# jjalcaraz-upct/network-slicing

Hardware: AMD Instinct MI355X
Metric: env-steps/sec (batched RanSlice.step, scenario_0) (higher is better)
Workload: dtype f64

## Files before the change

include/ranslice.h:

```cpp
#ifndef RANSLICE_H
#define RANSLICE_H

#include <stdint.h>

#ifdef __cplusplus
extern "C" {
#endif

#define RS_OK 0
#define RS_EINVAL (-1)
#define RS_EOVERFLOW (-2)
#define RS_EHIP (-3)
#define RS_ESTATE (-4)

#define RS_N_EMBB_VARS 10
#define RS_N_MMTC_VARS 3
#define RS_MAX_MCS 32
#define RS_MAX_SET 8
#define RS_N_TRACES 3

typedef struct rs_config {
    int32_t n_envs;
    int32_t n_prbs;
    int32_t n_embb;
    int32_t n_mmtc;
    int32_t slots_per_step;
    int32_t max_ue;
    int32_t max_bursts;
    int32_t max_mtc_queue;
    double slot_length;
    double penalty;
    double cbr_lambda, cbr_t_mean, cbr_bit_rate;
    double vbr_lambda, vbr_t_mean, vbr_p_size, vbr_b_size, vbr_b_rate;
    double sla_embb[6];
    double norm_embb[RS_N_EMBB_VARS];
    int32_t mtc_n_devices;
    int32_t mtc_n_rep, mtc_n_period;
    int32_t mtc_rep_set[RS_MAX_SET];
    int32_t mtc_period_set[RS_MAX_SET];
    double sla_mtc_delay;
    double norm_mmtc[RS_N_MMTC_VARS];
    double prop_A, prop_B;
    int32_t pf_granularity, pf_window, sym_per_prb;
    int32_t n_mcs;
    double mcs_rate[RS_MAX_MCS];
    double mcs_snr[RS_MAX_MCS];
    int32_t mcs_order[RS_MAX_MCS];
    int32_t mcs_mod[RS_MAX_MCS];
    double mi_x0[3], mi_k[3];
    int32_t l1_multiplex;
    int32_t reserved_;
} rs_config;

typedef struct rs_handle rs_handle;

typedef struct rs_alloc_rec {
    int32_t serial;
    int32_t type;
    int32_t e_snr;
    int32_t prbs;
    int64_t bits;
    double queue;
    double th;
    double p;
} rs_alloc_rec;

int rs_create(const rs_config* cfg, int device, rs_handle** out);

int rs_load_fading(rs_handle* h, int trace_id, const double* data, int rows, int cols);

int rs_reset(rs_handle* h, const uint64_t* seeds, float* obs);

int rs_step(rs_handle* h, const int32_t* actions, float* obs, double* reward, int32_t* labels,
            int32_t* violations);

int rs_step_resident(rs_handle* h);

int rs_random_actions(rs_handle* h, uint64_t seed, uint64_t step_index);

int rs_fetch(rs_handle* h, int32_t* actions, float* obs, double* reward, int32_t* labels,
             int32_t* violations);

int rs_get_info(rs_handle* h, double* info);

int rs_run_random(rs_handle* h, uint64_t seed, uint64_t step_index0, int n_steps, int use_graph);

int rs_set_alloc_trace(rs_handle* h, int enable);
int rs_get_alloc_trace(rs_handle* h, rs_alloc_rec* out);

int rs_get_counters(rs_handle* h, uint64_t counters[4]);

int rs_get_rx_stats(rs_handle* h, uint64_t out[3]);

int rs_kernel_time_ms(rs_handle* h, double* avg_ms, int64_t* launches);
int rs_kernel_time_stats_ms(rs_handle* h, double out[3], int64_t* launches);
int rs_set_kernel_timing(rs_handle* h, int enable);

int rs_set_group_size(rs_handle* h, int lanes);

int rs_set_schedule_hint(rs_handle* h, int mode);

int rs_get_section_profile(rs_handle* h, uint64_t out[16]);
int rs_get_task_profile(rs_handle* h, uint64_t* out);

int rs_synchronize(rs_handle* h);
int rs_device_count(void);
int rs_device_mem_info(int device, uint64_t* free_bytes, uint64_t* total_bytes);
int rs_n_vars(const rs_handle* h);
int rs_state_bytes(rs_handle* h, uint64_t* bytes);
int rs_save_state(rs_handle* h, void* blob, uint64_t bytes);
int rs_load_state(rs_handle* h, const void* blob, uint64_t bytes);
int rs_fork(rs_handle* dst, rs_handle* src, const int32_t* src_index);
int rs_set_lookahead(rs_handle* h, int max_branches);
int rs_step_clairvoyant(rs_handle* h, int32_t* actions_out, float* obs, double* reward, int32_t* labels,
                        int32_t* violations);
int rs_set_clairvoyant_fallback(rs_handle* h, int mode);
int rs_n_slices(const rs_handle* h);
#define RS_ACT_PRBS   0
#define RS_ACT_SHARES 1
#define RS_ACT_INDEX  2

typedef struct rs_device_view {
    int32_t device, n_envs, n_slices, n_vars;
    void*    stream;
    int32_t* in_prbs;  float* in_shares;  int64_t* in_index;
    int32_t* actions;  int32_t* resources;
    float*   obs;       float* obs_norm;
    double*  reward;    int32_t* labels;  int32_t* violations;  int32_t* total_violations;
    int64_t* rejected;
} rs_device_view;

int rs_get_device_view(rs_handle* h, rs_device_view* out);
int rs_step_device(rs_handle* h, int kind, const void* actions_device, void* caller_stream);
int rs_stream_join(rs_handle* h, void* caller_stream);
int rs_set_action_table(rs_handle* h, const int32_t* table , int32_t n_actions);
int rs_report_begin(rs_handle* h, int32_t steps);
int rs_report_extend(rs_handle* h, int32_t eval_steps);
int rs_report_fetch(rs_handle* h, int16_t* violation, double* reward, int16_t* resources, int32_t* n_recorded);
int rs_device_copy(rs_handle* h, void* dst, const void* src, uint64_t bytes, int to_device);
const char* rs_last_error(const rs_handle* h);
void rs_destroy(rs_handle* h);


#define KB_MAX_SLICES 8
#define KB_CAPACITY_MAX 65536

typedef struct kb_config {
    int32_t n_envs;
    int32_t n_slices;
    int32_t n_prbs;
    int32_t capacity;
    int32_t dims[KB_MAX_SLICES];
    double alfa;
    double acc_lo, acc_hi;
    double gamma, eta;
    int32_t shared_dictionary;
    int32_t first_env;
    int64_t pool_bytes;
} kb_config;

typedef struct kb_handle kb_handle;

int kb_create(const kb_config* cfg, int device, kb_handle** out);
void kb_destroy(kb_handle* k);
const char* kb_last_error(const kb_handle* k);
int kb_reset(kb_handle* k, const int32_t* initial_action, const int32_t* security_factor, const uint64_t* seeds);
int kb_update_control(kb_handle* k, const float* state, const int32_t* action, const int32_t* labels, int32_t* hits);
int kb_select_action(kb_handle* k, const float* state, int32_t* action, int32_t* adjusted);
int kb_step_resident(kb_handle* k, rs_handle* env);
int kb_run_resident(kb_handle* k, rs_handle* env, int n_steps, int use_graph);
int kb_predict(kb_handle* k, int e, int s, const double* x, int32_t* y_pred, double* f);
int kb_update(kb_handle* k, int e, int s, const double* x, int32_t y, int32_t* branch, double* delta);
int kb_get_kernel_row(kb_handle* k, int e, int s, int32_t* m, double* row);
int kb_get_learner(kb_handle* k, int e, int s, int32_t* m, double* landmarks, double* coeff, double* kinv);
int kb_get_control(kb_handle* k, int32_t* margins, int32_t* security, int32_t* action, int32_t* adjusted,
                   double* accuracies);
int kb_set_adjusted(kb_handle* k, const int32_t* adjusted);
#define KB_PROP_WIDTH 18
int kb_shared_scan(kb_handle* k, const float* state, const int32_t* action, const int32_t* labels, int32_t round,
                   int32_t budget, int32_t* hits, int32_t* counts, double* props);
// ... 100 lines not shown
```

network-slicing_amd/csrc/kb_api.hip:

```cpp
#pragma once
#include "kb_kbrl.hip"

struct kb_prune_state;
struct kb_ref_state;
struct kb_rebuild_state;
struct kb_bridge_state;
struct kb_fit_state;

struct kb_handle {
    kb_config cfg;
    int device = 0;
    hipStream_t stream = nullptr;
    hipEvent_t ev_order = nullptr;
    hipEvent_t ev_join = nullptr;
    hipStream_t side = nullptr;
    hipEvent_t ev_sfork = nullptr, ev_sjoin = nullptr;
    kb::KbDev D;
    kb::KbState K;
    std::vector<void*> allocs;
    std::vector<GuardedAlloc> guarded;
    std::vector<std::pair<void*, size_t>> regions;
    float* d_state = nullptr;
    float* d_prev_state = nullptr;
    int32_t* d_action = nullptr;
// ... 652 lines not shown
                hipLaunchKernelGGL(kb::select_bin_big_kernel, dim3(KB_BINBIG_GRID), dim3(64 * KB_BINBIG_WAVES), 0, k->stream, a);
                hipLaunchKernelGGL(kb::select_bin_kernel, dim3((unsigned)k->T), dim3(64), 0, k->stream, a, (int)KB_BIG_MAX);
            } else {
                hipLaunchKernelGGL(kb::select_bin_all_kernel, dim3(KB_BINBIG_GRID + (unsigned)((k->T + KB_BINBIG_WAVES - 1) / KB_BINBIG_WAVES)),
                                   dim3(64 * KB_BINBIG_WAVES), 0, k->stream, a);
            }
            hipLaunchKernelGGL(kb::big_list_kernel, dim3((unsigned)((k->T + 255) / 256)), dim3(256), 0, k->stream, k->D, k->K, a.big_par);
        } else {
            hipLaunchKernelGGL(kb::select_bin_kernel, dim3(slots), dim3(64), 0, k->stream, a, 0);
        }
        if (eb) HIPCHK(k, hipEventRecord(eb, k->stream));
        HIPCHK(k, k->spans.begin(k->stream, 6, &eg));
        hipLaunchKernelGGL(kb::select_gemm_kernel, dim3((slots + KB_SEL_WAVES - 1) / KB_SEL_WAVES), dim3(256), 0, k->stream, a);
        if (eg) HIPCHK(k, hipEventRecord(eg, k->stream));
    }
    if (e1) HIPCHK(k, hipEventRecord(e1, k->stream));
    hipLaunchKernelGGL(kb::adjust_kernel, dim3((unsigned)((k->cfg.n_envs + 255) / 256)), dim3(256), 0, k->stream, k->D,
                       k->K, d_action_out, a.big_par);
    if (a.big_par >= 0) k->big_par = 1 - k->big_par;
    return RS_OK;
}

static int kb_refuse_plus(kb_handle* k, const char* who) {
    if (k->alg != KB_ALG_PROJECTRON_PLUS || k->control_plus) return RS_OK;
    k->err = std::string(who) +
             ": the handle is in Projectron++ mode (kb_set_algorithm), which learns through kb_update / kb_fit only -- the control "
             "loop's update phase implements Projectron's rule (kb_set_algorithm(k, KB_ALG_PROJECTRON) switches back; "
             "kb_set_learning(k, 0) lets the resident loop select without learning)";
    return RS_ESTATE;
}

extern "C" int kb_update_control(kb_handle* k, const float* state, const int32_t* action, const int32_t* labels,
                                 int32_t* hits) {
    if (!k || !state || !action || !labels) return RS_EINVAL;
    if (!k->is_reset) {
        k->err = "kb_update_control: call kb_reset first";
        return RS_ESTATE;
    }
    if (int rc = kb_refuse_plus(k, "kb_update_control")) return rc;
    if (k->D.shared) {
        k->err = "kb_update_control: shared-dictionary handles learn through kb_shared_scan/apply/commit";
        return RS_ESTATE;
    }
    if (k->frozen) {
        k->err = "kb_update_control: an inference-only handle (kb_deploy) cannot learn: it holds no Kinv";
        return RS_ESTATE;
    }
    HIPCHK(k, hipSetDevice(k->device));
    const size_t T = (size_t)k->T, N = (size_t)k->cfg.n_envs;
    for (size_t i = 0; i < T; ++i)
        if (action[i] < 0 || action[i] > k->cfg.n_prbs || (labels[i] != 1 && labels[i] != -1)) {
            k->err = "kb_update_control: action out of [0, n_prbs] or label not +-1";
            return RS_EINVAL;
        }
    HIPCHK(k, hipMemcpyAsync(k->d_state, state, sizeof(float) * N * k->nv, hipMemcpyHostToDevice, k->stream));
    HIPCHK(k, hipMemcpyAsync(k->d_action, action, sizeof(int32_t) * T, hipMemcpyHostToDevice, k->stream));
    HIPCHK(k, hipMemcpyAsync(k->d_labels, labels, sizeof(int32_t) * T, hipMemcpyHostToDevice, k->stream));
    int rc = launch_update_control(k, k->d_state, k->d_action, k->d_labels);
    if (rc != RS_OK) return rc;
    HIPCHK(k, hipGetLastError());
    if (hits) HIPCHK(k, hipMemcpyAsync(hits, k->d_hits, sizeof(int32_t) * T, hipMemcpyDeviceToHost, k->stream));
    return kb_check(k);
}

extern "C" int kb_select_action(kb_handle* k, const float* state, int32_t* action, int32_t* adjusted) {
    if (!k || !state) return RS_EINVAL;
    if (!k->is_reset) {
        k->err = "kb_select_action: call kb_reset first";
        return RS_ESTATE;
    }
    HIPCHK(k, hipSetDevice(k->device));
    const size_t T = (size_t)k->T, N = (size_t)k->cfg.n_envs;
    HIPCHK(k, hipMemcpyAsync(k->d_state, state, sizeof(float) * N * k->nv, hipMemcpyHostToDevice, k->stream));
    int rc = launch_select(k, k->d_state, nullptr);
    if (rc != RS_OK) return rc;
    HIPCHK(k, hipGetLastError());
    if (action) HIPCHK(k, hipMemcpyAsync(action, k->K.action, sizeof(int32_t) * T, hipMemcpyDeviceToHost, k->stream));
    if (adjusted) HIPCHK(k, hipMemcpyAsync(adjusted, k->K.adjusted, sizeof(int32_t) * N, hipMemcpyDeviceToHost, k->stream));
    return kb_check(k);
}

extern "C" int kb_step_resident(kb_handle* k, rs_handle* env) {
    if (!k || !env) return RS_EINVAL;
    if (!k->is_reset || env->cfg.n_envs != k->cfg.n_envs || env->n_slices != k->cfg.n_slices || env->n_vars != k->nv ||
        env->device != k->device) {
        k->err = "kb_step_resident: agent and environment do not match (or kb_reset missing)";
        return RS_EINVAL;
    }
    if (k->D.shared) {
        k->err = "kb_step_resident: shared-dictionary handles step through kb_shared_step_resident";
        return RS_ESTATE;
    }
    if (k->learning)
        if (int rc = kb_refuse_plus(k, "kb_step_resident")) return rc;
    HIPCHK(k, hipSetDevice(k->device));
    if (env->hint_auto && !env->block_hint) {
        rs_set_schedule_hint(env, 1);
        env->hint_auto = true;
    }
    int rc = stream_after(k, &k->ev_order, env->stream, k->stream);
    if (rc != RS_OK) return rc;
    if (k->learning && (rc = launch_update_control(k, k->d_prev_state, env->d_actions, env->d_labels)) != RS_OK) return rc;
    rc = launch_select(k, env->d_obs, env->d_actions);
    if (rc != RS_OK) return rc;
    if (k->h_steps > 0) {
        kb::HistArgs ha;
        ha.D = k->D;
        ha.K = k->K;
        ha.reward = env->d_reward;
        ha.labels = env->d_labels;
        ha.violations = env->d_viol;
        ha.hits = k->d_hits;
        ha.h_reward = k->h_reward;
        ha.h_resources = k->h_resources;
        ha.h_hits = k->h_hits;
        ha.h_adjusted = k->h_adjusted;
        ha.h_sla = k->h_sla;
        ha.h_violation = k->h_violation;
        ha.cursor = k->h_cursor;
        ha.steps = k->h_steps;
        hipLaunchKernelGGL(kb::history_kernel, dim3((unsigned)((k->cfg.n_envs + 255) / 256)), dim3(256), 0, k->stream, ha);
        hipLaunchKernelGGL(kb::history_advance_kernel, dim3(1), dim3(1), 0, k->stream, k->h_cursor);
    }
    HIPCHK(k, hipMemcpyAsync(k->d_prev_state, env->d_obs, sizeof(float) * (size_t)k->cfg.n_envs * k->nv,
                             hipMemcpyDeviceToDevice, k->stream));
    if ((rc = stream_after(k, &k->ev_order, k->stream, env->stream)) != RS_OK) return rc;
    HIPCHK(k, hipGetLastError());
    return RS_OK;
}

static int enqueue_closed_step(kb_handle* k, rs_handle* env) {
    int rc = kb_step_resident(k, env);
    if (rc != RS_OK) return rc;
    rc = launch_step(env);
    if (rc != RS_OK) k->err = env->err;
    return rc;
}

extern "C" int kb_run_resident(kb_handle* k, rs_handle* env, int n_steps, int use_graph) {
    if (!k || !env || n_steps < 0) return RS_EINVAL;
    int done = 0, rc;
    if (k->learning && (rc = kb_refuse_plus(k, "kb_run_resident")) != RS_OK) return rc;
    static const bool no_graph = getenv("ROCP_TOOL_LIBRARIES") != nullptr &&
                                 !(dev_env("KBRL_GRAPH_UNDER_PROFILER") && atoi(dev_env("KBRL_GRAPH_UNDER_PROFILER")) != 0);
    if (no_graph) use_graph = 0;
    if (use_graph && !k->spans.on && !env->spans.on && !k->D.shared && n_steps >= 3) {
        if (!k->gexec || k->g_env != env || k->g_sig != env->launch_sig) {
            kb_drop_graph(k);
            if ((rc = enqueue_closed_step(k, env)) != RS_OK) return rc;
            done += 1;
        } else if (k->big_par != k->g_big_par || env->order_par != k->g_order_par) {
            if ((rc = enqueue_closed_step(k, env)) != RS_OK) return rc;
            done += 1;
            if (k->big_par != k->g_big_par || env->order_par != k->g_order_par) kb_drop_graph(k);
        }
        if (!k->gexec && n_steps - done >= 2) {
            const int32_t clock0 = env->clock;
            const uint64_t steps0 = env->steps;
            const bool ra = k->rounds_always, gf = k->gemm_fresh;
            k->g_big_par = k->big_par;
            k->g_order_par = env->order_par;
            k->rounds_always = true;
            HIPCHK(k, hipStreamBeginCapture(env->stream, hipStreamCaptureModeThreadLocal));
            const int rc1 = enqueue_closed_step(k, env);
            const int rc2 = rc1 == RS_OK ? enqueue_closed_step(k, env) : rc1;
            const hipError_t ec = hipStreamEndCapture(env->stream, &k->graph);
            env->clock = clock0;
            env->steps = steps0;
            env->order_par = k->g_order_par;
            k->big_par = k->g_big_par;
            k->rounds_always = ra;
            k->gemm_fresh = gf;
            if (rc2 != RS_OK || ec != hipSuccess) {
                kb_drop_graph(k);
                if (rc2 == RS_OK) k->err = std::string("hipStreamEndCapture: ") + hipGetErrorString(ec);
                return rc2 != RS_OK ? rc2 : RS_EHIP;
            }
            HIPCHK(k, hipGraphInstantiate(&k->gexec, k->graph, nullptr, nullptr, 0));
            k->g_env = env;
            k->g_sig = env->launch_sig;
        }
        bool launched = false;
        if (k->gexec && n_steps - done >= 2) {
            if ((rc = stream_after(k, &k->ev_order, k->stream, env->stream)) != RS_OK) return rc;
        }
        while (k->gexec && n_steps - done >= 2) {
            HIPCHK(k, hipGraphLaunch(k->gexec, env->stream));
            env->clock += 2 * env->cfg.slots_per_step;
            env->steps += 2;
            done += 2;
            launched = true;
        }
        if (launched) {
            if ((rc = stream_after(k, &k->ev_join, env->stream, k->stream)) != RS_OK) return rc;
        }
    }
    for (; done < n_steps; ++done)
        if ((rc = enqueue_closed_step(k, env)) != RS_OK) return rc;
    return RS_OK;
}

static int kb_one(kb_handle* k, int e, int s, const double* x, int y, bool update, double out[4]) {
    if (!k || !x || e < 0 || e >= k->cfg.n_envs || s < 0 || s >= k->cfg.n_slices) return RS_EINVAL;
    k->gemm_fresh = false;
    if (!k->is_reset) {
        k->err = "kb_predict/kb_update: call kb_reset first";
        return RS_ESTATE;
    }
    if (update && k->frozen) {
        k->err = "kb_update: an inference-only handle (kb_deploy) cannot learn: it holds no Kinv";
        return RS_ESTATE;
    }
    if (k->ref) {
        k->err = "kb_predict: a by-reference handle (kb_deploy_ref) shares read-only dictionaries: the cached kernel row would be written into a shared page";
        return RS_ESTATE;
    }
    HIPCHK(k, hipSetDevice(k->device));
    kb::OneArgs a;
    a.D = k->D;
    a.K = k->K;
    a.task = e * k->cfg.n_slices + s;
    a.y = y;
    memset(a.x, 0, sizeof a.x);
// ... 411 lines not shown
        k->gemm_fresh = false;
        launch_shared_scan(k, a);
        if (e1) local(hipEventRecord(e1, k->stream), "hipEventRecord");
        hipLaunchKernelGGL(kb::shared_collect_block_kernel, dim3((unsigned)S), dim3(KB_RANK_THREADS), 0, k->stream, k->D, d_state,
                           d_labels, k->d_cstar, (int)budget, k->d_block);
        if (rnd == 0 && hits_host) local(hipMemcpyAsync(hits_host, k->d_hits, sizeof(int32_t) * T, hipMemcpyDeviceToHost, k->stream), "copy of the hits");
        local(hipGetLastError(), "launch of the scan kernels");
        if (rnd == inject) local_err = "failure injected by KBRL_INJECT_FAIL_ROUND";
        if (!local_err.empty() && k->d_gather) {
            static const double mark[KB_MAX_SLICES] = {-1.0, -1.0, -1.0, -1.0, -1.0, -1.0, -1.0, -1.0};
            (void)hipMemcpyAsync(k->d_block, mark, sizeof(double) * S, hipMemcpyHostToDevice, k->stream);
        }
        if (!k->d_gather) {
            k->err = "kb_shared_step: " + local_err;
            if (k->comm) kb_comm_abort(k);
            return RS_EHIP;
        }
        if (k->comm) {
            const int nrc = rccl::AllGather(k->d_block, k->d_gather, blk, rccl::kDouble, k->comm, k->stream);
            if (nrc != 0) {
                k->err = std::string("ncclAllGather: ") + (rccl::GetErrorString ? rccl::GetErrorString(nrc) : "error");
                kb_comm_abort(k);
                return RS_EHIP;
            }
        } else {
            HIPCHK(k, hipMemcpyAsync(k->d_gather, k->d_block, sizeof(double) * blk, hipMemcpyDeviceToDevice, k->stream));
        }
        HIPCHK(k, hipMemsetAsync(k->d_total, 0, 2 * sizeof(int32_t), k->stream));
        hipLaunchKernelGGL(kb::shared_merge_kernel, dim3((unsigned)S), dim3(256), 0, k->stream, k->D, k->d_gather, W, me,
                           (int)budget, blk, k->d_mprops, k->d_mcounts, k->d_taken, k->d_total);
        launch_shared_apply(k, k->d_mprops, k->d_mcounts, (int)budget);
        hipLaunchKernelGGL(kb::shared_commit_kernel, dim3((unsigned)S), dim3(KB_RANK_THREADS), 0, k->stream, k->D, k->d_cstar, k->d_taken,
                           k->d_cursor);
        HIPCHK(k, hipGetLastError());
        if (rnd + 1 == max_rounds && !rounds_out && !k->comm && local_err.empty()) break;
        if (!k->h_total) HIPCHK(k, hipHostMalloc((void**)&k->h_total, 2 * sizeof(int32_t), hipHostMallocDefault));
        volatile int32_t* total = k->h_total;
        total[0] = total[1] = 0;
        HIPCHK(k, hipMemcpyAsync(k->h_total, k->d_total, 2 * sizeof(int32_t), hipMemcpyDeviceToHost, k->stream));
        const int wrc = shared_wait(k);
        if (wrc != RS_OK) return wrc;
        if (total[1] != 0 || !local_err.empty()) {
            k->err = !local_err.empty() ? "kb_shared_step: this rank failed in round " + std::to_string(rnd) + " (" + local_err +
                                              "); the other ranks were told through the exchange and leave the step with it"
                                        : "kb_shared_step: another rank of the shared-dictionary group reported a failure in round " +
                                              std::to_string(rnd) + "; all ranks leave the step together";
            return RS_EHIP;
        }
        if (total[0] == 0) break;
        rounds = rnd + 1;
    }
    if (rounds_out) *rounds_out = rounds;
    return RS_OK;
}

extern "C" int kb_shared_step(kb_handle* k, const float* state, const int32_t* action, const int32_t* labels,
                              int32_t budget, int32_t max_rounds, int32_t* hits, int32_t* rounds_out) {
    if (!k || !state || !action || !labels || budget <= 0 || max_rounds <= 0) return RS_EINVAL;
    if (!k->D.shared || !k->is_reset) {
        k->err = "kb_shared_step: handle is not a reset shared-dictionary agent";
        return RS_ESTATE;
    }
    if (budget > k->budget_cap) {
        k->err = "kb_shared_step: budget too large (<= 256)";
        return RS_EINVAL;
    }
    HIPCHK(k, hipSetDevice(k->device));
    const size_t T = (size_t)k->T, N = (size_t)k->cfg.n_envs;
    for (size_t i = 0; i < T; ++i)
        if (action[i] < 0 || action[i] > k->cfg.n_prbs || (labels[i] != 1 && labels[i] != -1)) {
            k->err = "kb_shared_step: action out of [0, n_prbs] or label not +-1";
            return RS_EINVAL;
        }
    HIPCHK(k, hipMemcpyAsync(k->d_state, state, sizeof(float) * N * k->nv, hipMemcpyHostToDevice, k->stream));
    HIPCHK(k, hipMemcpyAsync(k->d_action, action, sizeof(int32_t) * T, hipMemcpyHostToDevice, k->stream));
    HIPCHK(k, hipMemcpyAsync(k->d_labels, labels, sizeof(int32_t) * T, hipMemcpyHostToDevice, k->stream));
    int rc = shared_step_core(k, k->d_state, k->d_action, k->d_labels, budget, max_rounds, hits, rounds_out);
    if (rc != RS_OK) return rc;
    return kb_check(k);
}

extern "C" int kb_shared_step_resident(kb_handle* k, rs_handle* env, int32_t budget, int32_t max_rounds, int32_t* rounds_out) {
    if (!k || !env || budget <= 0 || max_rounds <= 0) return RS_EINVAL;
    if (!k->D.shared || !k->is_reset || env->cfg.n_envs != k->cfg.n_envs || env->n_slices != k->cfg.n_slices ||
        env->n_vars != k->nv || env->device != k->device || budget > k->budget_cap) {
        k->err = "kb_shared_step_resident: agent and environment do not match (or not a reset shared-dictionary agent, or budget > 256)";
        return RS_EINVAL;
    }
    HIPCHK(k, hipSetDevice(k->device));
    if (env->hint_auto && !env->block_hint) {
        rs_set_schedule_hint(env, 1);
        env->hint_auto = true;
    }
    int rc = stream_after(k, &k->ev_order, env->stream, k->stream);
    if (rc != RS_OK) return rc;
    rc = shared_step_core(k, k->d_prev_state, env->d_actions, env->d_labels, budget, max_rounds, nullptr, rounds_out);
    if (rc != RS_OK) return rc;
    rc = launch_select(k, env->d_obs, env->d_actions);
    if (rc != RS_OK) return rc;
    HIPCHK(k, hipMemcpyAsync(k->d_prev_state, env->d_obs, sizeof(float) * (size_t)k->cfg.n_envs * k->nv,
                             hipMemcpyDeviceToDevice, k->stream));
    if ((rc = stream_after(k, &k->ev_order, k->stream, env->stream)) != RS_OK) return rc;
    HIPCHK(k, hipGetLastError());
    k->gemm_fresh = true;
    return RS_OK;
}

extern "C" int kb_shared_merge(kb_handle* k, const double* gathered, int32_t world, int32_t me, int32_t budget, double* merged,
                               int32_t* counts, int32_t* taken, int32_t* total) {
    if (!k || !gathered || world < 1 || world > 64 || me < 0 || me >= world || budget <= 0 || budget > k->budget_cap)
        return RS_EINVAL;
    if (!k->D.shared) {
        k->err = "kb_shared_merge: handle is not a shared-dictionary agent";
        return RS_ESTATE;
    }
    HIPCHK(k, hipSetDevice(k->device));
    const size_t S = (size_t)k->cfg.n_slices, blk = S * (1 + (size_t)budget * KB_PROP_W);
    double* d_g = nullptr;
    HIPCHK(k, hipMalloc((void**)&d_g, sizeof(double) * blk * (size_t)world));
    int rc = RS_OK;
    hipError_t e = hipMemcpyAsync(d_g, gathered, sizeof(double) * blk * (size_t)world, hipMemcpyHostToDevice, k->stream);
    if (e == hipSuccess) e = hipMemsetAsync(k->d_total, 0, 2 * sizeof(int32_t), k->stream);
    if (e == hipSuccess) {
        hipLaunchKernelGGL(kb::shared_merge_kernel, dim3((unsigned)S), dim3(256), 0, k->stream, k->D, d_g, (int)world, (int)me,
                           (int)budget, blk, k->d_mprops, k->d_mcounts, k->d_taken, k->d_total);
        e = hipGetLastError();
    }
    if (e == hipSuccess && merged)
        e = hipMemcpyAsync(merged, k->d_mprops, sizeof(double) * S * budget * KB_PROP_W, hipMemcpyDeviceToHost, k->stream);
    if (e == hipSuccess && counts) e = hipMemcpyAsync(counts, k->d_mcounts, sizeof(int32_t) * S, hipMemcpyDeviceToHost, k->stream);
    if (e == hipSuccess && taken) e = hipMemcpyAsync(taken, k->d_taken, sizeof(int32_t) * S, hipMemcpyDeviceToHost, k->stream);
    if (e == hipSuccess && total) e = hipMemcpyAsync(total, k->d_total, sizeof(int32_t), hipMemcpyDeviceToHost, k->stream);
    if (e == hipSuccess) e = hipStreamSynchronize(k->stream);
    (void)hipFree(d_g);
    if (e != hipSuccess) {
        k->err = std::string("kb_shared_merge: ") + hipGetErrorString(e);
        rc = RS_EHIP;
    }
    return rc;
}

extern "C" int kb_history_begin(kb_handle* k, int32_t steps) {
    if (!k || steps <= 0) return RS_EINVAL;
    kb_drop_graph(k);
    HIPCHK(k, hipSetDevice(k->device));
    HIPCHK(k, hipStreamSynchronize(k->stream));
    kb_history_release(k);
    const size_t N = (size_t)k->cfg.n_envs, S = (size_t)k->cfg.n_slices, n = N * (size_t)steps;
    HIPCHK(k, hipMalloc((void**)&k->h_reward, sizeof(double) * n));
    HIPCHK(k, hipMalloc((void**)&k->h_resources, sizeof(int16_t) * n));
    HIPCHK(k, hipMalloc((void**)&k->h_hits, sizeof(int16_t) * n * S));
    HIPCHK(k, hipMalloc((void**)&k->h_adjusted, sizeof(int16_t) * n));
    HIPCHK(k, hipMalloc((void**)&k->h_sla, sizeof(int16_t) * n));
    HIPCHK(k, hipMalloc((void**)&k->h_violation, sizeof(int16_t) * n));
    HIPCHK(k, hipMalloc((void**)&k->h_cursor, sizeof(int32_t)));
    HIPCHK(k, hipMemsetAsync(k->h_reward, 0, sizeof(double) * n, k->stream));
    HIPCHK(k, hipMemsetAsync(k->h_resources, 0, sizeof(int16_t) * n, k->stream));
    HIPCHK(k, hipMemsetAsync(k->h_hits, 0, sizeof(int16_t) * n * S, k->stream));
    HIPCHK(k, hipMemsetAsync(k->h_adjusted, 0, sizeof(int16_t) * n, k->stream));
    HIPCHK(k, hipMemsetAsync(k->h_sla, 0, sizeof(int16_t) * n, k->stream));
    HIPCHK(k, hipMemsetAsync(k->h_violation, 0, sizeof(int16_t) * n, k->stream));
    HIPCHK(k, hipMemsetAsync(k->h_cursor, 0, sizeof(int32_t), k->stream));
    k->h_steps = steps;
    return RS_OK;
}

// ... 224 lines not shown
```

network-slicing_amd/csrc/rs_api.hip:

```cpp

#include <hip/hip_runtime.h>

#include <cmath>
#include <cstdio>
#include <cstdlib>
#include <cstring>
#include <string>
#include <vector>

#include "rs_host.h"

#ifdef RS_DEV
static inline const char* dev_env(const char* name) { return getenv(name); }
#else
static inline const char* dev_env(const char*) { return nullptr; }
#endif

#include "rs_embb.hip"
#include "rs_mmtc.hip"
#include "rs_order.hip"
#include "rs_mux.hip"

using namespace rs;

struct GuardedAlloc {
    void* base;
    size_t bytes;
};
static const size_t kGuard = 64 * 1024;
static bool guards_on() {
    static const bool on = dev_env("RANSLICE_GUARD") != nullptr;
    return on;
}
static hipError_t guarded_malloc(void** q, size_t bytes, std::vector<GuardedAlloc>* reg) {
    if (!guards_on()) return hipMalloc(q, bytes);
    void* b = nullptr;
    const size_t padded = (bytes + 255) / 256 * 256;
    hipError_t e = hipMalloc(&b, padded + 2 * kGuard);
    if (e != hipSuccess) return e;
    if (padded <= ((size_t)1 << 30)) {
        e = hipMemset(b, 0xA5, padded + 2 * kGuard);
    } else {
        e = hipMemset(b, 0xA5, kGuard);
        if (e == hipSuccess) e = hipMemset((char*)b + kGuard + padded, 0xA5, kGuard);
    }
    if (e != hipSuccess) return e;
    reg->push_back({b, padded});
    *q = (char*)b + kGuard;
    if (const char* v = dev_env("RANSLICE_GUARD"))
        if (v[0] == '2') fprintf(stderr, "RANSLICE_GUARD: buffer #%zu at %p, %zu bytes\n", reg->size() - 1, *q, bytes);
    return hipSuccess;
}
static void check_guards(const std::vector<GuardedAlloc>& reg, const char* who) {
    std::vector<unsigned char> buf(kGuard);
    for (size_t i = 0; i < reg.size(); ++i)
        for (int side = 0; side < 2; ++side) {
            const char* src = (const char*)reg[i].base + (side ? kGuard + reg[i].bytes : 0);
            if (hipMemcpy(buf.data(), src, kGuard, hipMemcpyDeviceToHost) != hipSuccess) continue;
            for (size_t k = 0; k < kGuard; ++k)
                if (buf[k] != 0xA5) {
                    fprintf(stderr, "RANSLICE_GUARD: %s buffer #%zu (%zu bytes): %s guard overwritten at offset %zu\n", who, i,
                            reg[i].bytes, side ? "upper" : "lower", k);
                    abort();
                }
        }
}

struct rs_handle {
    rs_config cfg;
    int device = 0;
    hipStream_t stream = nullptr;
    hipStream_t side = nullptr;
    hipEvent_t ev_fork = nullptr, ev_join = nullptr;
    int mixed = 0;
    int mixed_light = 256;
    int mixed_ue = 8;
    hipStream_t side2 = nullptr, side3 = nullptr;
    hipEvent_t ev_fork2 = nullptr, ev_join2 = nullptr, ev_join3 = nullptr;
    RsDev hdev;
    RsDev* ddev = nullptr;
    RsState st;
    RsState* d_st = nullptr;
    MtcState mst;
    std::vector<void*> allocs;
    std::vector<GuardedAlloc> guarded;
    std::vector<std::pair<void*, size_t>> regions;
    double* fad = nullptr;
    uint8_t* fad_valid = nullptr;
    double rx_band0 = 0.0;
    float* fad32 = nullptr;
    double* fps = nullptr;
    bool fad_loaded[RS_N_TRACES] = {false, false, false};
    std::vector<double> fad_host[RS_N_TRACES];
    std::vector<uint8_t> valid_host[RS_N_TRACES];
    int32_t* d_actions = nullptr;
    float* d_obs = nullptr;
    double* d_reward = nullptr;
    int32_t* d_labels = nullptr;
    int32_t* d_viol = nullptr;
    double* d_info = nullptr;
    uint64_t* d_counters = nullptr;
    uint64_t* d_counter_sum = nullptr;
    rs_alloc_rec* d_trace = nullptr;
    uint64_t* d_sections = nullptr;
    unsigned long long* d_pace = nullptr;
    int32_t* d_redo = nullptr;
    int32_t* d_order = nullptr;
    uint64_t* d_oslot = nullptr;
    int* d_ohist = nullptr;
    int order_par = 0;
    int order_mode = 6;
    int order_pair = 256;
    int block_hint = 0;
    int spread_mode = -1;
    int spread_max = 1024;
    int key_w[4] = {16, 16, 0, 0};
    int rot_mask = 0;
    int snake_mask = 0x2aaaaaaa;
    int snake = 1;
    bool hint_auto = true;
    int group = 16;
    bool trace_on = false;
    int n_slices = 0, n_vars = 0, n_tasks = 0;
    int n_ran = 0;
    bool mux = false;
    int64_t* d_run = nullptr;
    hipGraph_t graph = nullptr;
    hipGraphExec_t gexec = nullptr;
    int graph_par = 0, graph_sig = -1;
    uint64_t launch_sig = 0;
    int32_t clock = 0;
    uint64_t steps = 0;
    bool is_reset = false;
    uint64_t fad_hash = 0;
    bool tables_borrowed = false;
    int32_t* d_fork_idx = nullptr;
    int32_t* h_fork_idx = nullptr;
    hipEvent_t ev_fork_in = nullptr, ev_fork_out = nullptr;
    rs_handle* la = nullptr;
    int la_max = 0;
    int la_widest = 0;
    int32_t* d_la_err = nullptr;
    struct PolicyIo* pio = nullptr;
    EventSpans spans;
    std::string err;
};

static int auto_hint(const rs_handle* h);

static void drop_graph(rs_handle* h);

template <class T>
static int dalloc(rs_handle* h, T** p, size_t n) {
    void* q = nullptr;
    size_t bytes = sizeof(T) * (n ? n : 1);
    HIPCHK(h, guarded_malloc(&q, bytes, &h->guarded));
    HIPCHK(h, hipMemsetAsync(q, 0, bytes, h->stream));
    if (!guards_on()) h->allocs.push_back(q);
    h->regions.emplace_back(q, bytes);
    *p = (T*)q;
    return RS_OK;
}


static size_t mtc_mux_lds_bytes(int cap, int n_mmtc) {
    return ((size_t)2 * cap * n_mmtc + (size_t)n_mmtc * MTC_DEV_MAX) * sizeof(int32_t);
}

static int mtc_alloc(rs_handle* h, rs::MtcState* m, size_t n_tasks, const RsDev& d) {
    memset(m, 0, sizeof *m);
    m->n_tasks = n_tasks;
    m->cap = d.mtc_cap;
    if (n_tasks == 0) return RS_OK;
    if (d.mtc_n_dev > MTC_DEV_MAX || d.mtc_cap > MTC_CAP_MAX || d.mtc_n_rep <= 0 || d.mtc_n_rep > 8 ||
        d.mtc_n_period <= 0 || d.mtc_n_period > 8) {
        h->err = "rs_create: mMTC configuration out of range (<=1024 devices, queue capacity <=2048)";
        return RS_EINVAL;
    }
    if (d.mux) {
        const size_t lds = mtc_mux_lds_bytes(d.mtc_cap, d.n_mmtc);
        if (lds > 160 * 1024 - 4096) {
            h->err = "rs_create: l1_multiplex with this many mMTC RAN slices and this queue capacity needs more LDS than a CU has";
            return RS_EINVAL;
        }
        if (lds > 48 * 1024)
            HIPCHK(h, hipFuncSetAttribute((const void*)rs::mtc_mux_step_kernel, hipFuncAttributeMaxDynamicSharedMemorySize, (int)lds));
    }
    for (int i = 0; i < d.mtc_n_period; ++i)
        if (d.mtc_period_set[i] < d.slots) {
            h->err = "rs_create: mMTC periods shorter than one observation period are not supported";
            return RS_EINVAL;
        }
    int rc;
    if ((rc = dalloc(h, &m->n_users, n_tasks)) != RS_OK) return rc;
    if ((rc = dalloc(h, &m->s_start, n_tasks)) != RS_OK) return rc;
    if ((rc = dalloc(h, &m->s_rep, n_tasks)) != RS_OK) return rc;
    if ((rc = dalloc(h, &m->dev_next, n_tasks * MTC_DEV_MAX)) != RS_OK) return rc;
    if ((rc = dalloc(h, &m->dev_period, n_tasks * MTC_DEV_MAX)) != RS_OK) return rc;
    if ((rc = dalloc(h, &m->dev_rep, n_tasks * MTC_DEV_MAX)) != RS_OK) return rc;
    if ((rc = dalloc(h, &m->q_rep, n_tasks * (size_t)m->cap)) != RS_OK) return rc;
    if ((rc = dalloc(h, &m->q_start, n_tasks * (size_t)m->cap)) != RS_OK) return rc;
    return RS_OK;
}

static int mtc_reset(rs_handle* h, rs::MtcState* m) {
    if (m->n_tasks == 0) return RS_OK;
    hipLaunchKernelGGL(rs::mtc_reset_kernel, dim3((unsigned)m->n_tasks), dim3(256), 0, h->stream, h->ddev, *m,
                       h->st.seeds);
    return RS_OK;
}

static int mtc_step(rs_handle* h, rs::MtcState* m, hipStream_t stream) {
    if (m->n_tasks == 0) return RS_OK;
    rs::MtcArgs a;
    a.D = h->ddev;
    a.M = *m;
    a.actions = h->d_actions;
    a.run = h->d_run;
    a.obs = h->d_obs;
    a.labels = h->d_labels;
    a.violations = h->d_viol;
    a.info = h->d_info;
    a.err = h->st.err;
    size_t lds = (size_t)4 * 2 * m->cap * sizeof(int32_t);
    hipLaunchKernelGGL(rs::mtc_step_kernel, dim3((unsigned)((m->n_tasks + 3) / 4)), dim3(256), lds, stream, a);
    return RS_OK;
}


namespace rs {

__global__ void reset_kernel(const RsDev* D, RsState S, const uint64_t* seeds_in) {
    int i = blockIdx.x * blockDim.x + threadIdx.x;
    int n_tasks = D->n_envs * D->n_embb;
    if (i < n_tasks) {
        S.t_n_ue[i] = 0;
        S.t_cbr_at[i] = 1;
        S.t_vbr_at[i] = 1;
        S.t_ctr[i] = 0;
        S.t_serial[i] = 1;
        S.t_cost[i] = 0;
    }
    if (i < D->n_envs) {
        S.seeds[i] = seeds_in[i];
        S.err[i] = 0;
    }
}

__global__ void finalize_kernel(const RsDev* D, const int32_t* actions, const int32_t* viol, double* reward,
                                int64_t* run) {
    int r = blockIdx.x * blockDim.x + threadIdx.x;
    if (r >= D->n_envs) return;
    if (r == 0) {
        run[0] += D->slots;
        run[1] += 1;
    }
    int S = D->n_act;
    long tv = 0, ta = 0;
    for (int s = 0; s < S; ++s) {
        tv += viol[r * S + s];
        ta += actions[r * S + s];
    }
    double rew;
    if (tv > 0)
        rew = -1 * D->penalty * (double)tv;
    else
        rew = (double)(D->n_prbs - ta > 0 ? D->n_prbs - ta : 0);
    reward[r] = rew;
}

__global__ __launch_bounds__(256) void random_actions_kernel(const RsDev* D, int32_t* actions, uint64_t seed,
                                                           uint64_t step, const int64_t* run) {
    if (run) {
        step = (uint64_t)run[1];
        seed = (uint64_t)run[2];
    }
    const int lane = threadIdx.x & 63;
    const int r = blockIdx.x * 4 + (threadIdx.x >> 6);
    if (r >= D->n_envs) return;
    const int S = D->n_act;
    int my_bin[8];
    int cnt = 0;
    for (int p = lane; p < D->n_prbs; p += 64) {
        uint32_t a, b;
        rs_philox4x32_10((uint32_t)p, (uint32_t)r, (uint32_t)step,
                         (uint32_t)(step >> 32) ^ (uint32_t)((uint64_t)r >> 32) ^ 0x5bd1e995u, (uint32_t)seed,
                         (uint32_t)(seed >> 32), &a, &b);
        my_bin[cnt++ & 7] = (int)(((uint64_t)a * (uint64_t)(S + 1)) >> 32);
    }
    for (int s = 0; s < S; ++s) {
        int c = 0;
        for (int k = 0; k < cnt; ++k) c += my_bin[k] == s ? 1 : 0;
        for (int d = 32; d >= 1; d >>= 1) c += __shfl_xor(c, d);
        if (lane == 0) actions[r * S + s] = c;
    }
}

__global__ void set_run_kernel(int64_t* run, uint64_t seed, uint64_t step) {
    run[1] = (int64_t)step;
    run[2] = (int64_t)seed;
}

__global__ void counter_sum_kernel(const uint64_t* per_task, int n_tasks, uint64_t* out) {
    __shared__ unsigned long long acc[4];
    if (threadIdx.x < 4) acc[threadIdx.x] = 0ull;
    __syncthreads();
    unsigned long long loc[4] = {0ull, 0ull, 0ull, 0ull};
    for (int i = blockIdx.x * blockDim.x + threadIdx.x; i < n_tasks; i += gridDim.x * blockDim.x)
        for (int k = 0; k < 4; ++k) loc[k] += per_task[(size_t)i * 4 + k];
    for (int k = 0; k < 4; ++k) atomicAdd(&acc[k], loc[k]);
    __syncthreads();
    if (threadIdx.x < 4) atomicAdd((unsigned long long*)&out[threadIdx.x], acc[threadIdx.x]);
}

}


static void mcs_factors(double* A, double* B) {
    double Delta = 0.1;
    double a = 1.0 / Delta;
    double s01 = rs_sigmoid(0.1, 0.0, 1.0), s09 = rs_sigmoid(0.9, 0.0, 1.0);
    a = a * (rs_log(1.0 / s01 - 1.0) - rs_log(1.0 / s09 - 1.0));
    *A = a;
    *B = -rs_log(1.0 / s09 - 1.0);
}

static void mcs_lookup(const rs_config* c, double A, double B, int e_snr, int* mcs_out, int* rate_out) {
    double rx_prob = 1.0 - 0.1;
    int mcs;
    for (mcs = 0; mcs < c->n_mcs; ++mcs) {
        double x = A * ((double)e_snr - c->mcs_snr[mcs]) - B;
        if (rs_sigmoid(x, 0.0, 1.0) < rx_prob) {
            *mcs_out = mcs - 1 > 0 ? mcs - 1 : 0;
            *rate_out = (int)((double)c->sym_per_prb * (c->mcs_rate[mcs] * (double)c->mcs_order[mcs]));
            return;
        }
    }
    mcs = c->n_mcs - 1;
    *mcs_out = mcs;
    *rate_out = (int)((double)c->sym_per_prb * (c->mcs_rate[mcs] * (double)c->mcs_order[mcs]));
}

static void rx_fast_setup(RsDev& d, double* band0) {
    const double A = d.mcsA;
    double kmax = 0.0, kmin = 1e300;
    bool ok = std::isfinite(A) && A > 0.0 && std::isfinite(d.mcsB);
    for (int m = 0; m < 3; ++m) {
        const double k = d.mi_k[m];
        ok = ok && std::isfinite(k) && k > 0.0 && std::isfinite(d.mi_x0[m]);
        kmax = k > kmax ? k : kmax;
        kmin = k < kmin ? k : kmin;
        d.rx_c1[m] = (float)(-k * RS_INV_LN2);
    }
    ok = ok && A / kmax >= 1.0 && A / kmin <= 1.0e4;
    d.rx_invA = ok ? (float)(1.0 / A) : 0.0f;
    d.rx_B = (float)d.mcsB;
    d.rx_band = 0.0;
    *band0 = ok ? 6.0e-6 + 6.0e-6 * (kmax / A) : 0.0;
    d.rx_band1 = ok ? 4.0e-5 / A + 1.0e-6 : 0.0;
    if (dev_env("RANSLICE_RX_EXACT")) *band0 = 0.0;
    if (const char* e = dev_env("RANSLICE_RX_BAND_SCALE")) {
        const double f = atof(e);
// ... 117 lines not shown
        }
        d.slot_rc = rc;
        d.pf_div_fast = (same && !dev_env("RANSLICE_EXACT_DIV")) ? 1 : 0;
    }
    for (int m = 0; m < cfg->n_mcs; ++m) {
        d.mcs_ref[m] = cfg->mcs_snr[m];
        if (cfg->mcs_mod[m] < 0 || cfg->mcs_mod[m] > 2) {
            h->err = "rs_create: modulation index out of range";
            return RS_EINVAL;
        }
        d.mcs_mod[m] = cfg->mcs_mod[m];
    }
    for (int m = 0; m < 3; ++m) {
        d.mi_x0[m] = cfg->mi_x0[m];
        d.mi_k[m] = cfg->mi_k[m];
    }
    rx_fast_setup(d, &h->rx_band0);
    d.mtc_n_dev = cfg->mtc_n_devices;
    d.mtc_cap = cfg->max_mtc_queue > 0 ? cfg->max_mtc_queue : 1024;
    d.mtc_n_rep = cfg->mtc_n_rep;
    d.mtc_n_period = cfg->mtc_n_period;
    for (int i = 0; i < 8; ++i) {
        d.mtc_rep_set[i] = cfg->mtc_rep_set[i];
        d.mtc_period_set[i] = cfg->mtc_period_set[i];
    }
    d.sla_mtc_delay = cfg->sla_mtc_delay;
    for (int i = 0; i < 3; ++i) d.norm_mmtc[i] = cfg->norm_mmtc[i];

    int rc;
    const size_t T = (size_t)h->n_tasks, N = (size_t)cfg->n_envs;
    const size_t U = T * RS_GROUP;
    RsState& s = h->st;
#define DA(p, n)                                   \
    if ((rc = dalloc(h, &(p), (n))) != RS_OK) return rc
    DA(h->ddev, 1);
    DA(s.t_n_ue, T); DA(s.t_cbr_at, T); DA(s.t_vbr_at, T); DA(s.t_ctr, T); DA(s.t_serial, T); DA(s.t_cost, T);
    DA(s.u_queue, U); DA(s.u_th, U); DA(s.u_nominal, U);
    DA(s.u_hold_at, U); DA(s.u_e_snr, U); DA(s.u_findex, U); DA(s.u_bits, U); DA(s.u_prbs, U);
    DA(s.u_vbr_at, U); DA(s.u_ctr, U); DA(s.u_serial, U); DA(s.u_flags, U);
    DA(s.u_burst, U * RS_BURSTS);
    DA(s.seeds, N); DA(s.err, N);
    DA(h->d_actions, N * h->n_slices);
    DA(h->d_obs, N * h->n_vars);
    DA(h->d_reward, N);
    DA(h->d_labels, N * h->n_slices);
    DA(h->d_viol, N * h->n_slices);
    DA(h->d_info, N * h->n_ran * 10);
    DA(h->d_counters, (T ? T : 1) * 4);
    DA(h->d_counter_sum, 4);
    DA(h->d_sections, 16 + 4 * (T ? T : 1) + 16);
    DA(h->d_redo, T ? T : 1);
    DA(h->d_order, T ? T : 1);
    DA(h->d_oslot, T ? T : 1);
    DA(h->d_ohist, 2 * RS_ORDER_BINS);
    HIPCHK(h, hipMemset(h->d_ohist, 0, sizeof(int) * 2 * RS_ORDER_BINS));
    if (const char* e = dev_env("RANSLICE_ORDER")) h->order_mode = atoi(e);
    {
        int cus = 256;
        if (hipDeviceGetAttribute(&cus, hipDeviceAttributeMultiprocessorCount, h->device) != hipSuccess) cus = 256;
        (void)hipGetLastError();
        const long long resident_waves = (long long)cus * 4 * RS_OCC;
        h->order_pair = (long long)h->n_tasks / 4 > resident_waves + resident_waves / 4 ? 0 : 256;
    }
    if (const char* e = dev_env("RANSLICE_PAIR")) h->order_pair = atoi(e);
    h->group = h->n_tasks <= 6144 ? 32 : 16;
    if (const char* e = dev_env("RANSLICE_GROUP")) {
        const int g = atoi(e);
        if (g == 8 || g == 16 || g == 32) h->group = g;
    }
    {
        int cus = 0;
        if (hipDeviceGetAttribute(&cus, hipDeviceAttributeMultiprocessorCount, h->device) == hipSuccess && cus > 0) h->spread_max = cus * 4;
        (void)hipGetLastError();
        if (const char* e = dev_env("RANSLICE_SPREAD")) h->spread_mode = atoi(e);
        if (const char* e = dev_env("RANSLICE_SNAKE")) h->snake = atoi(e);
        if (const char* e = dev_env("RANSLICE_KEY_W")) (void)sscanf(e, "%d,%d,%d,%d", &h->key_w[0], &h->key_w[1], &h->key_w[2], &h->key_w[3]);
        if (const char* e = dev_env("RANSLICE_SNAKE_MASK")) h->snake_mask = (int)strtol(e, nullptr, 0);
        if (const char* e = dev_env("RANSLICE_SNAKE_ROT")) h->rot_mask = (int)strtol(e, nullptr, 0);
    }
    if (h->group == 16 && h->n_tasks >= 49152) h->mixed_light = 224;
    if (const char* e = dev_env("RANSLICE_MIXED")) h->mixed = atoi(e);
    if (const char* e = dev_env("RANSLICE_MIXED_UE")) h->mixed_ue = atoi(e);
    if (const char* e = dev_env("RANSLICE_MIXED_LIGHT")) h->mixed_light = atoi(e);
    if (h->mixed > 0 || h->mixed_light < 256) {
        HIPCHK(h, hipStreamCreateWithFlags(&h->side2, hipStreamNonBlocking));
        HIPCHK(h, hipEventCreateWithFlags(&h->ev_fork2, hipEventDisableTiming));
        HIPCHK(h, hipEventCreateWithFlags(&h->ev_join2, hipEventDisableTiming));
        HIPCHK(h, hipStreamCreateWithFlags(&h->side3, hipStreamNonBlocking));
        HIPCHK(h, hipEventCreateWithFlags(&h->ev_join3, hipEventDisableTiming));
    }
    h->block_hint = auto_hint(h);
    if (const char* e = dev_env("RANSLICE_HINT")) {
        h->hint_auto = atoi(e) < 0;
        if (!h->hint_auto) h->block_hint = atoi(e) ? 1 : 0;
    }
    DA(h->d_st, 1);
    DA(h->d_run, 4);
    DA(h->d_pace, 4);
    if ((rc = mtc_alloc(h, &h->mst, N * (size_t)cfg->n_mmtc, d)) != RS_OK) return rc;
#undef DA
    HIPCHK(h, hipMemcpyAsync(h->d_st, &h->st, sizeof(RsState), hipMemcpyHostToDevice, h->stream));
    HIPCHK(h, hipStreamSynchronize(h->stream));
    return RS_OK;
}

static void fork_release(rs_handle* h);
static void policy_io_release(rs_handle* h);
static int policy_io_on_reset(rs_handle* h);

extern "C" void rs_destroy(rs_handle* h) {
    if (!h) return;
    if (h->stream) (void)hipStreamSynchronize(h->stream);
    drop_graph(h);
    fork_release(h);
    policy_io_release(h);
    if (guards_on()) check_guards(h->guarded, "rs");
    for (auto& g : h->guarded) (void)hipFree(g.base);
    for (void* p : h->allocs) (void)hipFree(p);
    if (!h->tables_borrowed) {
        if (h->fad) (void)hipFree(h->fad);
        if (h->fad_valid) (void)hipFree(h->fad_valid);
        if (h->fad32) (void)hipFree(h->fad32);
        if (h->fps) (void)hipFree(h->fps);
    }
    if (h->d_trace) (void)hipFree(h->d_trace);
    h->spans.release();
    if (h->side) (void)hipStreamDestroy(h->side);
    if (h->side2) (void)hipStreamDestroy(h->side2);
    if (h->side3) (void)hipStreamDestroy(h->side3);
    if (h->ev_join3) (void)hipEventDestroy(h->ev_join3);
    if (h->ev_fork2) (void)hipEventDestroy(h->ev_fork2);
    if (h->ev_join2) (void)hipEventDestroy(h->ev_join2);
    if (h->ev_fork) (void)hipEventDestroy(h->ev_fork);
    if (h->ev_join) (void)hipEventDestroy(h->ev_join);
    if (h->stream) (void)hipStreamDestroy(h->stream);
    delete h;
}

extern "C" const char* rs_last_error(const rs_handle* h) { return h ? h->err.c_str() : "null handle"; }
extern "C" int rs_n_vars(const rs_handle* h) { return h ? h->n_vars : RS_EINVAL; }
extern "C" int rs_n_slices(const rs_handle* h) { return h ? h->n_slices : RS_EINVAL; }
extern "C" int rs_device_count(void) {
    int n = 0;
    return hipGetDeviceCount(&n) == hipSuccess ? n : RS_EHIP;
}

extern "C" int rs_device_mem_info(int device, uint64_t* free_bytes, uint64_t* total_bytes) {
    if (!free_bytes || !total_bytes) return RS_EINVAL;
    size_t f = 0, t = 0;
    if (hipSetDevice(device) != hipSuccess || hipMemGetInfo(&f, &t) != hipSuccess) return RS_EHIP;
    *free_bytes = (uint64_t)f;
    *total_bytes = (uint64_t)t;
    return RS_OK;
}


static uint64_t fading_hash(const rs_handle* h) {
    uint64_t x = kFnvOffsetBasis;
    auto mix = [&x](const void* p, size_t n) { x = fnv1a(p, n, x); };
    mix(&h->hdev.P, sizeof h->hdev.P);
    for (int f = 0; f < RS_N_TRACES; ++f) {
        mix(&h->hdev.T[f], sizeof h->hdev.T[f]);
        mix(h->fad_host[f].data(), sizeof(double) * h->fad_host[f].size());
        mix(h->valid_host[f].data(), h->valid_host[f].size());
    }
    return x;
}

static int upload_fading(rs_handle* h) {
    RsDev& d = h->hdev;
    size_t elems = 0, vbytes = 0;
    d.has_nan = 0;
    for (int f = 0; f < RS_N_TRACES; ++f) {
        d.fad_off[f] = (int64_t)elems;
        d.valid_off[f] = (int64_t)vbytes;
        elems += h->fad_host[f].size();
        vbytes += h->valid_host[f].size();
        bool any_valid = false;
        for (uint8_t v : h->valid_host[f]) {
            if (!v) d.has_nan = 1;
            any_valid = any_valid || v;
        }
        if (!any_valid) {
            h->err = "rs_load_fading: a trace has no NaN-free column";
            return RS_EINVAL;
        }
    }
    if (elems + (size_t)RS_MAX_PRBS >= (size_t)1 << 31) {
        h->err = "rs_load_fading: tables exceed 2^31 samples";
        return RS_EINVAL;
    }
    if (h->fad) (void)hipFree(h->fad);
    if (h->fad_valid) (void)hipFree(h->fad_valid);
    if (h->fad32) (void)hipFree(h->fad32);
    if (h->fps) (void)hipFree(h->fps);
    h->fad32 = nullptr;
    h->fps = nullptr;
    HIPCHK(h, hipMalloc((void**)&h->fad, sizeof(double) * (elems + 16)));
    HIPCHK(h, hipMalloc((void**)&h->fad_valid, vbytes + 16));
    if (const char* v = dev_env("RANSLICE_GUARD"))
        if (v[0] == '2') fprintf(stderr, "RANSLICE_GUARD: fading table at %p, %zu bytes\n", (void*)h->fad, sizeof(double) * (elems + 16));
    for (int f = 0; f < RS_N_TRACES; ++f) {
        HIPCHK(h, hipMemcpyAsync(h->fad + d.fad_off[f], h->fad_host[f].data(), sizeof(double) * h->fad_host[f].size(),
                                 hipMemcpyHostToDevice, h->stream));
        HIPCHK(h, hipMemcpyAsync(h->fad_valid + d.valid_off[f], h->valid_host[f].data(), h->valid_host[f].size(),
                                 hipMemcpyHostToDevice, h->stream));
    }
    {
        const int P = d.P;
        std::vector<float> t32(elems + 64, 0.0f);
        std::vector<double> ps((elems / (size_t)P) * (size_t)(P + 1) + 16, 0.0);
        double smax = 0.0;
        bool finite = true;
        for (int f = 0; f < RS_N_TRACES; ++f) {
            const std::vector<double>& tab = h->fad_host[f];
            const size_t cols = tab.size() / (size_t)P, c0 = (size_t)d.fad_off[f] / (size_t)P;
            d.col_off[f] = (int32_t)c0;
            for (size_t t = 0; t < cols; ++t) {
                long double acc = 0.0L;
                double* row = &ps[(c0 + t) * (size_t)(P + 1)];
                row[0] = 0.0;
                const bool ok = h->valid_host[f][t] != 0;
                for (int p = 0; p < P; ++p) {
                    const double v = tab[t * (size_t)P + p];
                    t32[(size_t)d.fad_off[f] + t * (size_t)P + p] = (float)v;
                    acc += (long double)v;
                    row[p + 1] = (double)acc;
                    if (ok) {
                        finite = finite && std::isfinite(v);
                        smax = std::fabs(v) > smax ? std::fabs(v) : smax;
                    }
                }
            }
        }
        const bool small = finite && smax <= 1.0e3;
        const bool ps_fits = ps.size() + (size_t)RS_MAX_PRBS < ((size_t)1 << 31);
        d.est_band = (small && ps_fits && !dev_env("RANSLICE_EST_EXACT")) ? 1.0e-9 : 0.0;
        double kmax = 0.0;
        for (int m = 0; m < 3; ++m) kmax = d.mi_k[m] > kmax ? d.mi_k[m] : kmax;
        d.rx_band = (small && h->rx_band0 > 0.0) ? h->rx_band0 + 0.5 * kmax * 5.97e-8 * smax : 0.0;
        if (const char* e = dev_env("RANSLICE_RX_BAND_SCALE")) {
            const double fsc = atof(e);
            if (fsc >= 1.0) d.rx_band *= fsc;
        }
        if (const char* e = dev_env("RANSLICE_EST_BAND")) {
            const double b = atof(e);
            if (d.est_band > 0.0 && b > 0.0 && b < 0.5) d.est_band = b;
        }
        HIPCHK(h, hipMalloc((void**)&h->fad32, sizeof(float) * t32.size()));
        HIPCHK(h, hipMalloc((void**)&h->fps, sizeof(double) * ps.size()));
        HIPCHK(h, hipMemcpy(h->fad32, t32.data(), sizeof(float) * t32.size(), hipMemcpyHostToDevice));
        HIPCHK(h, hipMemcpy(h->fps, ps.data(), sizeof(double) * ps.size(), hipMemcpyHostToDevice));
    }
    HIPCHK(h, hipMemcpyAsync(h->ddev, &d, sizeof d, hipMemcpyHostToDevice, h->stream));
    HIPCHK(h, hipStreamSynchronize(h->stream));
    h->fad_hash = fading_hash(h);
    for (int f = 0; f < RS_N_TRACES; ++f) {
        std::vector<double>().swap(h->fad_host[f]);
        std::vector<uint8_t>().swap(h->valid_host[f]);
    }
    return RS_OK;
}

extern "C" int rs_load_fading(rs_handle* h, int trace_id, const double* data, int rows, int cols) {
    if (!h) return RS_EINVAL;
    if (trace_id < 0 || trace_id >= RS_N_TRACES || !data || rows <= 0 || cols <= 0 || h->cfg.n_prbs > 2 * rows) {
        h->err = "rs_load_fading: bad arguments";
        return RS_EINVAL;
    }
    HIPCHK(h, hipSetDevice(h->device));
    drop_graph(h);
    if (h->tables_borrowed) {
        h->err = "rs_load_fading: a lookahead branch handle shares its tables";
        return RS_ESTATE;
    }
    if (h->la) {
        HIPCHK(h, hipStreamSynchronize(h->stream));
        rs_destroy(h->la);
        h->la = nullptr;
    }
    h->fad_hash = 0;
    const int P = h->cfg.n_prbs > rows ? h->cfg.n_prbs : rows;
    if (h->hdev.P != 0 && h->hdev.P != P) {
        h->err = "rs_load_fading: all traces must have the same number of rows";
        return RS_EINVAL;
    }
    h->hdev.P = P;
    h->hdev.T[trace_id] = cols;
    std::vector<double>& tab = h->fad_host[trace_id];
    std::vector<uint8_t>& val = h->valid_host[trace_id];
    tab.assign((size_t)P * cols, 0.0);
    val.assign((size_t)cols, 1);
    for (int t = 0; t < cols; ++t) {
        bool bad = false;
        for (int p = 0; p < P; ++p) {
            double v = data[(size_t)(p % rows) * cols + t];
            tab[(size_t)t * P + p] = v;
            bad = bad || (v != v);
        }
        val[t] = bad ? 0 : 1;
    }
    h->fad_loaded[trace_id] = true;
    if (h->fad_loaded[0] && h->fad_loaded[1] && h->fad_loaded[2]) return upload_fading(h);
    return RS_OK;
}


static bool fading_ready(const rs_handle* h) {
    return h->cfg.n_embb == 0 || (h->fad != nullptr && h->fad_loaded[0] && h->fad_loaded[1] && h->fad_loaded[2]);
}

extern "C" int rs_reset(rs_handle* h, const uint64_t* seeds, float* obs) {
    if (!h || !seeds) return RS_EINVAL;
    HIPCHK(h, hipSetDevice(h->device));
    if (!fading_ready(h)) {
        h->err = "rs_reset: fading traces not loaded";
        return RS_ESTATE;
    }
    const int N = h->cfg.n_envs;
    if (h->cfg.n_embb == 0) HIPCHK(h, hipMemcpyAsync(h->ddev, &h->hdev, sizeof(RsDev), hipMemcpyHostToDevice, h->stream));
    uint64_t* tmp = nullptr;
    HIPCHK(h, hipMalloc((void**)&tmp, sizeof(uint64_t) * N));
    HIPCHK(h, hipMemcpyAsync(tmp, seeds, sizeof(uint64_t) * N, hipMemcpyHostToDevice, h->stream));
    int n = h->n_tasks > N ? h->n_tasks : N;
    hipLaunchKernelGGL(reset_kernel, dim3((n + 255) / 256), dim3(256), 0, h->stream, h->ddev, h->st, tmp);
    if (h->cfg.n_mmtc > 0) mtc_reset(h, &h->mst);
    HIPCHK(h, hipMemsetAsync(h->d_counters, 0, sizeof(uint64_t) * 4 * (h->n_tasks ? h->n_tasks : 1), h->stream));
    HIPCHK(h, hipMemsetAsync(h->d_obs, 0, sizeof(float) * N * h->n_vars, h->stream));
    HIPCHK(h, hipMemsetAsync(h->d_run, 0, sizeof(int64_t) * 4, h->stream));
    if (policy_io_on_reset(h) != RS_OK) return RS_EHIP;
    HIPCHK(h, hipGetLastError());
    HIPCHK(h, hipStreamSynchronize(h->stream));
    (void)hipFree(tmp);
    h->clock = 0;
    h->steps = 0;
    h->is_reset = true;
    if (obs) memset(obs, 0, sizeof(float) * (size_t)N * h->n_vars);
    return RS_OK;
}

static StepArgs step_args(const rs_handle* h) {
    StepArgs a;
    memset(&a, 0, sizeof a);
    a.D = h->ddev;
    a.S = h->d_st;
    a.fad = h->fad;
    a.fad32 = h->fad32;
    a.fps = h->fps;
    a.fad_valid = h->fad_valid;
    a.actions = h->d_actions;
    a.run = h->d_run;
    a.obs = h->d_obs;
    a.labels = h->d_labels;
    a.violations = h->d_viol;
    a.info = h->d_info;
    a.counters = h->d_counters;
    a.trace = h->d_trace;
    return a;
}

static int launch_step(rs_handle* h) {
    if (!h->is_reset) {
        h->err = "rs_step: call rs_reset first";
        return RS_ESTATE;
    }
    if (h->clock > 2000000000 - h->cfg.slots_per_step) {
        h->err = "rs_step: slot clock would overflow; reset the environment";
        return RS_ESTATE;
    }
    if (h->mux) {
        if (h->n_tasks > 0) {
            StepArgs a = step_args(h);
            hipEvent_t e1;
            HIPCHK(h, h->spans.begin(h->stream, 0, &e1));
            if (h->trace_on) hipLaunchKernelGGL((embb_mux_step_kernel<true>), dim3((unsigned)h->cfg.n_envs), dim3(64), 0, h->stream, a);
            else hipLaunchKernelGGL((embb_mux_step_kernel<false>), dim3((unsigned)h->cfg.n_envs), dim3(64), 0, h->stream, a);
            if (e1) HIPCHK(h, hipEventRecord(e1, h->stream));
        }
        if (h->cfg.n_mmtc > 0) {
            rs::MtcArgs ma;
            ma.D = h->ddev;
            ma.M = h->mst;
            ma.actions = h->d_actions;
            ma.run = h->d_run;
            ma.obs = h->d_obs;
            ma.labels = h->d_labels;
            ma.violations = h->d_viol;
            ma.info = h->d_info;
            ma.err = h->st.err;
            const size_t lds = mtc_mux_lds_bytes(h->mst.cap, h->cfg.n_mmtc);
            hipLaunchKernelGGL(rs::mtc_mux_step_kernel, dim3((unsigned)h->cfg.n_envs), dim3(64), lds, h->stream, ma);
        }
        hipLaunchKernelGGL(finalize_kernel, dim3((h->cfg.n_envs + 255) / 256), dim3(256), 0, h->stream, h->ddev,
                           h->d_actions, h->d_viol, h->d_reward, h->d_run);
        HIPCHK(h, hipGetLastError());
        h->clock += h->cfg.slots_per_step;
        h->steps += 1;
        return RS_OK;
    }
    const bool forked = h->side && h->cfg.n_mmtc > 0 && h->n_tasks > 0 && h->mst.n_tasks > 0;
    if (forked) {
        HIPCHK(h, hipEventRecord(h->ev_fork, h->stream));
        HIPCHK(h, hipStreamWaitEvent(h->side, h->ev_fork, 0));
        mtc_step(h, &h->mst, h->side);
        HIPCHK(h, hipEventRecord(h->ev_join, h->side));
    }
    if (h->n_tasks > 0) {
        StepArgs a = step_args(h);
        a.sections = h->d_sections;
        a.redo = h->d_redo;
        a.pace = h->d_pace;
        a.order_cnt = -1;
        hipStream_t lstream = h->stream;
        auto launch = [&](int g) {
            if (a.order_cnt < 0) a.spread = (h->spread_mode == 1 || (h->spread_mode < 0 && h->n_tasks <= h->spread_max)) ? 1 : 0;
            const int per_block = a.spread ? 4 : 256 / g;
            const int n_mine = a.order_cnt >= 0 ? a.order_cnt : h->n_tasks;
            dim3 grid((n_mine + per_block - 1) / per_block), block(256);
            const bool tr = h->trace_on;
#define RS_LAUNCH_STEP(G_, TR_, BL_)                                                                              \
    do {                                                                                                          \
        if (h->hdev.pf_div_fast)                                                                                  \
            hipLaunchKernelGGL((embb_step_kernel<G_, TR_, BL_, true>), grid, block, 0, lstream, a);             \
        else                                                                                                      \
            hipLaunchKernelGGL((embb_step_kernel<G_, TR_, BL_, false>), grid, block, 0, lstream, a);            \
    } while (0)
            if (g == 8) {
                if (tr) RS_LAUNCH_STEP(8, true, true);
                else if (h->block_hint) RS_LAUNCH_STEP(8, false, true);
                else RS_LAUNCH_STEP(8, false, false);
            } else if (g == 16) {
                if (tr) RS_LAUNCH_STEP(16, true, true);
                else if (h->block_hint) RS_LAUNCH_STEP(16, false, true);
                else RS_LAUNCH_STEP(16, false, false);
            } else {
                if (tr) RS_LAUNCH_STEP(32, true, true);
                else RS_LAUNCH_STEP(32, false, true);
            }
#undef RS_LAUNCH_STEP
        };
        int seg_head = 0, seg_light = 0;
        if (h->order_mode > 0) {
            const int par = h->order_par;
            h->order_par ^= 1;
            const unsigned nb = (unsigned)((h->n_tasks + 255) / 256);
            const bool split = h->side2 != nullptr && (h->mixed > 0 || h->mixed_light < 256) && !h->trace_on && h->group == 16 && h->n_tasks >= 4096;
            if (split) {
                seg_head = h->mixed > 0 ? (h->n_tasks / h->mixed) & ~3 : 0;
                seg_light = h->mixed_light >= 256 ? h->n_tasks - seg_head : ((int)(((long long)h->n_tasks * h->mixed_light) >> 8)) & ~7;
                if (((h->n_tasks - seg_head - seg_light) & 3) != 0) seg_light += (h->n_tasks - seg_head - seg_light) & 3;
            }
            const int seg_mid = h->n_tasks - seg_head - seg_light;
            hipLaunchKernelGGL(order_key_kernel, dim3(nb), dim3(256), 0, h->stream, h->ddev, h->d_st, h->d_actions,
                               h->order_mode, h->d_ohist + par * RS_ORDER_BINS, h->d_oslot, make_int4(h->key_w[0], h->key_w[1], h->key_w[2], h->key_w[3]),
                               split ? h->mixed_ue : 0);
            hipLaunchKernelGGL(order_scatter_kernel, dim3(nb), dim3(256), 0, h->stream, h->ddev,
                               h->d_ohist + par * RS_ORDER_BINS, h->d_ohist + (1 - par) * RS_ORDER_BINS, h->d_oslot,
                               h->d_order, h->order_mode > 3 ? h->order_pair : 0, 64 / h->group,
                               h->snake == 1 ? h->spread_max : h->snake, h->snake_mask, h->rot_mask, seg_head, seg_head + seg_mid);
            a.order = h->d_order;
        }
        hipEvent_t e1;
        HIPCHK(h, h->spans.begin(h->stream, 0, &e1));
        if (a.order && seg_head + seg_light > 0) {
            const int seg_mid = h->n_tasks - seg_head - seg_light;
            HIPCHK(h, hipEventRecord(h->ev_fork2, h->stream));
            if (seg_head > 0) {
                HIPCHK(h, hipStreamWaitEvent(h->side2, h->ev_fork2, 0));
                lstream = h->side2;
                a.order_off = 0;
                a.order_cnt = seg_head;
                a.spread = 1;
                launch(16);
                HIPCHK(h, hipEventRecord(h->ev_join2, h->side2));
            }
            if (seg_mid > 0 && seg_light > 0) {
                HIPCHK(h, hipStreamWaitEvent(h->side3, h->ev_fork2, 0));
                lstream = h->side3;
                a.order_off = seg_head + seg_mid;
                a.order_cnt = seg_light;
                a.spread = 0;
                launch(8);
                HIPCHK(h, hipEventRecord(h->ev_join3, h->side3));
            }
            lstream = h->stream;
            a.spread = 0;
            if (seg_mid > 0) {
                a.order_off = seg_head;
                a.order_cnt = seg_mid;
                launch(16);
            } else {
                a.order_off = seg_head;
                a.order_cnt = seg_light;
                launch(8);
            }
            if (seg_head > 0) HIPCHK(h, hipStreamWaitEvent(h->stream, h->ev_join2, 0));
            if (seg_mid > 0 && seg_light > 0) HIPCHK(h, hipStreamWaitEvent(h->stream, h->ev_join3, 0));
            a.order_off = 0;
            a.order_cnt = -1;
        } else {
            launch(h->group);
        }
        if (e1) HIPCHK(h, hipEventRecord(e1, h->stream));
        a.order = nullptr;
        if (h->group < 32) {
            a.replay = 1;
            launch(32);
        }
    }
    if (forked) HIPCHK(h, hipStreamWaitEvent(h->stream, h->ev_join, 0));
    else if (h->cfg.n_mmtc > 0) mtc_step(h, &h->mst, h->stream);
    hipLaunchKernelGGL(finalize_kernel, dim3((h->cfg.n_envs + 255) / 256), dim3(256), 0, h->stream, h->ddev,
                       h->d_actions, h->d_viol, h->d_reward, h->d_run);
    HIPCHK(h, hipGetLastError());
    h->clock += h->cfg.slots_per_step;
    h->steps += 1;
    return RS_OK;
}

static int auto_hint(const rs_handle* h) {
    const int gran = h->cfg.pf_granularity > 0 ? h->cfg.pf_granularity : 1;
    return h->cfg.n_prbs / (h->n_slices + 1) >= RS_HINT_PAIRS * gran ? 1 : 0;
}

static int check_errors(rs_handle* h) {
    std::vector<int32_t> e((size_t)h->cfg.n_envs);
    HIPCHK(h, hipMemcpyAsync(e.data(), h->st.err, sizeof(int32_t) * e.size(), hipMemcpyDeviceToHost, h->stream));
    HIPCHK(h, hipStreamSynchronize(h->stream));
    for (size_t i = 0; i < e.size(); ++i)
        if (e[i]) {
            h->err = std::string("capacity exceeded in replica ") + std::to_string(i) + ":" +
                     ((e[i] & 1) ? " UEs per slice" : "") + ((e[i] & 2) ? " active VBR bursts per UE" : "") +
                     ((e[i] & 4) ? " backlogged mMTC devices" : "");
            return RS_EOVERFLOW;
        }
    return RS_OK;
}

extern "C" int rs_fetch(rs_handle* h, int32_t* actions, float* obs, double* reward, int32_t* labels,
                        int32_t* violations) {
    if (!h) return RS_EINVAL;
    HIPCHK(h, hipSetDevice(h->device));
    const size_t N = (size_t)h->cfg.n_envs, S = (size_t)h->n_slices;
    if (actions) HIPCHK(h, hipMemcpyAsync(actions, h->d_actions, sizeof(int32_t) * N * S, hipMemcpyDeviceToHost, h->stream));
    if (obs) HIPCHK(h, hipMemcpyAsync(obs, h->d_obs, sizeof(float) * N * h->n_vars, hipMemcpyDeviceToHost, h->stream));
    if (reward) HIPCHK(h, hipMemcpyAsync(reward, h->d_reward, sizeof(double) * N, hipMemcpyDeviceToHost, h->stream));
    if (labels) HIPCHK(h, hipMemcpyAsync(labels, h->d_labels, sizeof(int32_t) * N * S, hipMemcpyDeviceToHost, h->stream));
    if (violations) HIPCHK(h, hipMemcpyAsync(violations, h->d_viol, sizeof(int32_t) * N * S, hipMemcpyDeviceToHost, h->stream));
    return check_errors(h);
}

extern "C" int rs_step(rs_handle* h, const int32_t* actions, float* obs, double* reward, int32_t* labels,
                       int32_t* violations) {
    if (!h || !actions) return RS_EINVAL;
    HIPCHK(h, hipSetDevice(h->device));
    const size_t N = (size_t)h->cfg.n_envs, S = (size_t)h->n_slices;
    size_t wide = 0;
    const int wide_prbs = RS_HINT_PAIRS * (h->cfg.pf_granularity > 0 ? h->cfg.pf_granularity : 1);
    for (size_t r = 0; r < N; ++r) {
        long tot = 0;
        for (size_t s = 0; s < S; ++s) {
            if (actions[r * S + s] < 0) {
                h->err = "rs_step: negative action";
                return RS_EINVAL;
            }
            tot += actions[r * S + s];
            wide += actions[r * S + s] >= wide_prbs;
        }
        if (tot > h->cfg.n_prbs) {
            h->err = "rs_step: sum(action) > n_prbs in replica " + std::to_string(r);
            return RS_EINVAL;
        }
    }
    if (h->hint_auto) {
        const int want = wide * 16 >= N ? 1 : 0;
        if (want != h->block_hint) {
            h->block_hint = want;
            drop_graph(h);
        }
    }
    HIPCHK(h, hipMemcpyAsync(h->d_actions, actions, sizeof(int32_t) * N * S, hipMemcpyHostToDevice, h->stream));
    int rc = launch_step(h);
    if (rc != RS_OK) return rc;
    return rs_fetch(h, nullptr, obs, reward, labels, violations);
}

extern "C" int rs_step_resident(rs_handle* h) {
    if (!h) return RS_EINVAL;
    HIPCHK(h, hipSetDevice(h->device));
    return launch_step(h);
}

extern "C" int rs_random_actions(rs_handle* h, uint64_t seed, uint64_t step_index) {
    if (!h) return RS_EINVAL;
    HIPCHK(h, hipSetDevice(h->device));
    if (h->n_slices > 8) {
        h->err = "rs_random_actions: at most 8 slices";
        return RS_EINVAL;
    }
    if (h->cfg.n_prbs > 512) return RS_EINVAL;
    hipLaunchKernelGGL(random_actions_kernel, dim3((h->cfg.n_envs + 3) / 4), dim3(256), 0, h->stream, h->ddev,
                       h->d_actions, seed, step_index, (const int64_t*)nullptr);
    HIPCHK(h, hipGetLastError());
    return RS_OK;
}

static void drop_graph(rs_handle* h) {
    h->launch_sig += 1;
    if (h->gexec) (void)hipGraphExecDestroy(h->gexec);
    if (h->graph) (void)hipGraphDestroy(h->graph);
    h->gexec = nullptr;
    h->graph = nullptr;
}

static int enqueue_scripted_step(rs_handle* h) {
    hipLaunchKernelGGL(random_actions_kernel, dim3((h->cfg.n_envs + 3) / 4), dim3(256), 0, h->stream, h->ddev,
                       h->d_actions, (uint64_t)0, (uint64_t)0, (const int64_t*)h->d_run);
    return launch_step(h);
}

extern "C" int rs_run_random(rs_handle* h, uint64_t seed, uint64_t step_index0, int n_steps, int use_graph) {
    if (!h || n_steps < 0) return RS_EINVAL;
    HIPCHK(h, hipSetDevice(h->device));
    if (h->n_slices > 8 || h->cfg.n_prbs > 512) {
        h->err = "rs_run_random: at most 8 slices and 512 PRBs";
        return RS_EINVAL;
    }
    if (!h->is_reset) {
        h->err = "rs_run_random: call rs_reset first";
        return RS_ESTATE;
    }
    if ((int64_t)h->clock + (int64_t)n_steps * h->cfg.slots_per_step > 2000000000) {
        h->err = "rs_run_random: slot clock would overflow; reset the environment";
        return RS_ESTATE;
    }
    hipLaunchKernelGGL(set_run_kernel, dim3(1), dim3(1), 0, h->stream, h->d_run, seed, step_index0);
    int done = 0, rc;
    if (use_graph && !h->spans.on && n_steps >= 2) {
        if (h->gexec && h->graph_par != h->order_par) {
            if ((rc = enqueue_scripted_step(h)) != RS_OK) return rc;
            done += 1;
        }
        if (!h->gexec) {
            const int32_t clock0 = h->clock;
            const uint64_t steps0 = h->steps;
            h->graph_par = h->order_par;
            HIPCHK(h, hipStreamBeginCapture(h->stream, hipStreamCaptureModeThreadLocal));
            const int rc1 = enqueue_scripted_step(h);
            const int rc2 = rc1 == RS_OK ? enqueue_scripted_step(h) : rc1;
            const hipError_t ec = hipStreamEndCapture(h->stream, &h->graph);
            h->clock = clock0;
            h->steps = steps0;
            h->order_par = h->graph_par;
            if (rc2 != RS_OK || ec != hipSuccess) {
                drop_graph(h);
                if (rc2 == RS_OK) h->err = std::string("hipStreamEndCapture: ") + hipGetErrorString(ec);
                return rc2 != RS_OK ? rc2 : RS_EHIP;
            }
            HIPCHK(h, hipGraphInstantiate(&h->gexec, h->graph, nullptr, nullptr, 0));
        }
        while (n_steps - done >= 2) {
            HIPCHK(h, hipGraphLaunch(h->gexec, h->stream));
            h->clock += 2 * h->cfg.slots_per_step;
            h->steps += 2;
            done += 2;
        }
    }
    for (; done < n_steps; ++done)
        if ((rc = enqueue_scripted_step(h)) != RS_OK) return rc;
    return RS_OK;
}

extern "C" int rs_get_info(rs_handle* h, double* info) {
    if (!h || !info) return RS_EINVAL;
    HIPCHK(h, hipSetDevice(h->device));
    HIPCHK(h, hipMemcpyAsync(info, h->d_info, sizeof(double) * (size_t)h->cfg.n_envs * h->n_ran * 10,
                             hipMemcpyDeviceToHost, h->stream));
    HIPCHK(h, hipStreamSynchronize(h->stream));
    return RS_OK;
}

extern "C" int rs_set_alloc_trace(rs_handle* h, int enable) {
    if (!h) return RS_EINVAL;
    HIPCHK(h, hipSetDevice(h->device));
    if (enable && !h->d_trace) {
        size_t n = (size_t)h->n_tasks * h->cfg.slots_per_step * RS_GROUP;
        if (h->mux) n = (size_t)h->cfg.n_envs * h->cfg.slots_per_step * RS_MUX_UE;
        HIPCHK(h, hipMalloc((void**)&h->d_trace, sizeof(rs_alloc_rec) * (n ? n : 1)));
    }
    h->trace_on = enable != 0;
    drop_graph(h);
    return RS_OK;
}

extern "C" int rs_get_alloc_trace(rs_handle* h, rs_alloc_rec* out) {
    if (!h || !out || !h->d_trace) return RS_EINVAL;
    HIPCHK(h, hipSetDevice(h->device));
    size_t n = (size_t)h->n_tasks * h->cfg.slots_per_step * RS_GROUP;
    if (h->mux) n = (size_t)h->cfg.n_envs * h->cfg.slots_per_step * RS_MUX_UE;
    HIPCHK(h, hipMemcpyAsync(out, h->d_trace, sizeof(rs_alloc_rec) * n, hipMemcpyDeviceToHost, h->stream));
    HIPCHK(h, hipStreamSynchronize(h->stream));
    return RS_OK;
}

extern "C" int rs_get_counters(rs_handle* h, uint64_t counters[4]) {
    if (!h || !counters) return RS_EINVAL;
    HIPCHK(h, hipSetDevice(h->device));
    HIPCHK(h, hipMemsetAsync(h->d_counter_sum, 0, sizeof(uint64_t) * 4, h->stream));
    if (h->n_tasks > 0)
        hipLaunchKernelGGL(counter_sum_kernel, dim3(64), dim3(256), 0, h->stream, h->d_counters, h->n_tasks,
                           h->d_counter_sum);
    HIPCHK(h, hipMemcpyAsync(counters, h->d_counter_sum, sizeof(uint64_t) * 4, hipMemcpyDeviceToHost, h->stream));
    HIPCHK(h, hipStreamSynchronize(h->stream));
    counters[1] = h->steps * (uint64_t)h->cfg.n_envs;
    return RS_OK;
}

extern "C" int rs_get_rx_stats(rs_handle* h, uint64_t out[3]) {
    if (!h || !out) return RS_EINVAL;
    uint64_t c[4];
    const int rc = rs_get_counters(h, c);
    if (rc != RS_OK) return rc;
    HIPCHK(h, hipMemcpyAsync(c, h->d_counter_sum, sizeof(uint64_t) * 4, hipMemcpyDeviceToHost, h->stream));
    HIPCHK(h, hipStreamSynchronize(h->stream));
    out[0] = c[1] >> 32;
    out[1] = c[1] & 0xffffffffull;
    out[2] = h->hdev.rx_band > 0.0 ? 1u : 0u;
    return RS_OK;
}

extern "C" int rs_set_schedule_hint(rs_handle* h, int mode) {
    if (!h) return RS_EINVAL;
    h->hint_auto = mode < 0;
    h->block_hint = mode < 0 ? auto_hint(h) : (mode ? 1 : 0);
    drop_graph(h);
    return RS_OK;
}

extern "C" int rs_set_group_size(rs_handle* h, int lanes) {
    if (!h || (lanes != 8 && lanes != 16 && lanes != 32)) return RS_EINVAL;
    h->group = lanes;
    drop_graph(h);
    return RS_OK;
}

extern "C" int rs_get_section_profile(rs_handle* h, uint64_t out[16]) {
    if (!h || !out) return RS_EINVAL;
    HIPCHK(h, hipSetDevice(h->device));
    HIPCHK(h, hipMemcpyAsync(out, h->d_sections, sizeof(uint64_t) * 16, hipMemcpyDeviceToHost, h->stream));
    HIPCHK(h, hipStreamSynchronize(h->stream));
    return RS_OK;
}

extern "C" int rs_get_task_profile(rs_handle* h, uint64_t* out) {
    if (!h || !out) return RS_EINVAL;
    HIPCHK(h, hipSetDevice(h->device));
    HIPCHK(h, hipMemcpyAsync(out, h->d_sections + 16, sizeof(uint64_t) * (4 * (size_t)h->n_tasks + 16),
                             hipMemcpyDeviceToHost, h->stream));
    HIPCHK(h, hipStreamSynchronize(h->stream));
    return RS_OK;
}

extern "C" int rs_set_kernel_timing(rs_handle* h, int enable) {
    if (!h) return RS_EINVAL;
    h->spans.on = enable != 0;
    h->spans.reset();
    return RS_OK;
}

extern "C" int rs_kernel_time_stats_ms(rs_handle* h, double out[3], int64_t* launches) {
    if (!h || !out) return RS_EINVAL;
    HIPCHK(h, hipSetDevice(h->device));
    HIPCHK(h, hipStreamSynchronize(h->stream));
    double tot = 0.0, mn = 0.0, mx = 0.0;
    int64_t n = 0;
    HIPCHK(h, h->spans.drain([&](int, double ms) {
        tot += ms;
        mn = (n == 0 || ms < mn) ? ms : mn;
        mx = ms > mx ? ms : mx;
        n += 1;
    }));
    out[0] = n ? tot / (double)n : 0.0;
    out[1] = mn;
    out[2] = mx;
    if (launches) *launches = n;
    return RS_OK;
}

extern "C" int rs_kernel_time_ms(rs_handle* h, double* avg_ms, int64_t* launches) {
    if (!h || !avg_ms) return RS_EINVAL;
    double st[3];
    const int rc = rs_kernel_time_stats_ms(h, st, launches);
    if (rc == RS_OK) *avg_ms = st[0];
    return rc;
}

extern "C" int rs_synchronize(rs_handle* h) {
    if (!h) return RS_EINVAL;
    HIPCHK(h, hipSetDevice(h->device));
    HIPCHK(h, hipStreamSynchronize(h->stream));
    return RS_OK;
}

struct rs_state_header {
    uint64_t magic, n_regions, total_bytes, cfg_hash;
    int64_t clock, steps;
    int32_t order_par, graph_par, block_hint, hint_auto, is_reset, pad;
};
static int sync_streams(rs_handle* h) {
    HIPCHK(h, hipStreamSynchronize(h->stream));
    for (hipStream_t s : {h->side, h->side2, h->side3})
        if (s) HIPCHK(h, hipStreamSynchronize(s));
    return RS_OK;
}
static const uint64_t kRsStateMagic = 0x52534c4943453034ull;
static uint64_t rs_cfg_hash(const rs_handle* h) {
    uint64_t x = fnv1a(&h->cfg, sizeof h->cfg);
    for (auto& r : h->regions) x = fnv1a_step(x, (uint64_t)r.second);
    return x;
}
extern "C" int rs_state_bytes(rs_handle* h, uint64_t* bytes) {
    if (!h || !bytes) return RS_EINVAL;
    uint64_t t = sizeof(rs_state_header);
    for (auto& r : h->regions) t += r.second;
    *bytes = t;
    return RS_OK;
}
extern "C" int rs_save_state(rs_handle* h, void* blob, uint64_t bytes) {
    uint64_t need = 0;
    if (!h || !blob || rs_state_bytes(h, &need) != RS_OK) return RS_EINVAL;
    if (bytes < need) {
        h->err = "rs_save_state: buffer smaller than rs_state_bytes";
        return RS_EINVAL;
    }
    HIPCHK(h, hipSetDevice(h->device));
    if (sync_streams(h) != RS_OK) return RS_EHIP;
    rs_state_header hd = {kRsStateMagic, (uint64_t)h->regions.size(), need, rs_cfg_hash(h), (int64_t)h->clock, (int64_t)h->steps,
                          h->order_par, h->graph_par, h->block_hint, h->hint_auto ? 1 : 0, h->is_reset ? 1 : 0, 0};
    memcpy(blob, &hd, sizeof hd);
    char* o = (char*)blob + sizeof hd;
    for (auto& r : h->regions) {
        HIPCHK(h, hipMemcpy(o, r.first, r.second, hipMemcpyDeviceToHost));
        o += r.second;
    }
    return RS_OK;
}
extern "C" int rs_load_state(rs_handle* h, const void* blob, uint64_t bytes) {
    uint64_t need = 0;
    if (!h || !blob || rs_state_bytes(h, &need) != RS_OK) return RS_EINVAL;
    rs_state_header hd;
    if (bytes < sizeof hd) return RS_EINVAL;
    memcpy(&hd, blob, sizeof hd);
    if (hd.magic != kRsStateMagic || hd.n_regions != h->regions.size() || hd.total_bytes != need || bytes < need ||
        hd.cfg_hash != rs_cfg_hash(h)) {
        h->err = "rs_load_state: the blob was not saved by a handle of this configuration";
        return RS_EINVAL;
    }
    HIPCHK(h, hipSetDevice(h->device));
    if (sync_streams(h) != RS_OK) return RS_EHIP;
    drop_graph(h);
    const char* o = (const char*)blob + sizeof hd;
    for (auto& r : h->regions) {
        if (r.first != (void*)h->ddev && r.first != (void*)h->d_st)
            HIPCHK(h, hipMemcpy(r.first, o, r.second, hipMemcpyHostToDevice));
        o += r.second;
    }
    h->clock = (int32_t)hd.clock;
    h->steps = (uint64_t)hd.steps;
    h->order_par = hd.order_par;
    h->graph_par = hd.graph_par;
    h->graph_sig = -1;
    h->block_hint = hd.block_hint;
    h->hint_auto = hd.hint_auto != 0;
    h->is_reset = hd.is_reset != 0;
    return RS_OK;
}
#include "rs_fork.hip"
#include "rs_policy_io.hip"
#include "kb_api.hip"
#include "kb_fork.hip"
#include "kb_prune.hip"
#include "kb_shared_prune.hip"
#include "kb_ref.hip"
#include "kb_agents.hip"
#include "kb_rebuild.hip"
#include "kb_bridge.hip"
#include "kb_fit.hip"
#include "kb_fit_wide.hip"
#include "kb_fit_steps.hip"
#include "kb_control_plus.hip"
#include "kb_control_plus_batch.hip"
#include "kb_control_plus_wide.hip"
#include "kb_fit_steps_batch.hip"
#include "kb_shared_plus.hip"
#include "kb_shared_plus_batch.hip"
#ifdef RS_DEV
#include "rs_probe.hip"
#include "kb_probe.hip"
#endif
```

network-slicing_amd/csrc/rs_fork.hip:

```cpp

#define RS_FORK_MAX 48

namespace rs {

struct ForkTable {
    const char* src[RS_FORK_MAX];
    char* dst[RS_FORK_MAX];
    uint32_t bpr[RS_FORK_MAX];
    int32_t n;
};

struct ForkArgs {
    ForkTable T;
    const int32_t* index;
    int32_t n_dst;
    const int64_t* run_src;
    int64_t* run_dst;
    int32_t C, c0, cnt, s, n_act, n_prbs;
    const int32_t* acts_src;
    int32_t* acts_dst;
};

__global__ __launch_bounds__(256) void fork_gather_kernel(ForkArgs a) {
    const int lane = threadIdx.x & 63;
// ... 92 lines not shown
        {a.u_bits, b.u_bits, 4 * U}, {a.u_prbs, b.u_prbs, 4 * U}, {a.u_vbr_at, b.u_vbr_at, 4 * U},
        {a.u_ctr, b.u_ctr, 4 * U}, {a.u_serial, b.u_serial, 4 * U}, {a.u_flags, b.u_flags, 4 * U},
        {a.u_burst, b.u_burst, 2 * U * RS_BURSTS},
        {a.seeds, b.seeds, 8}, {a.err, b.err, 4},
        {ma.n_users, mb.n_users, 4 * M}, {ma.s_start, mb.s_start, 8 * M}, {ma.s_rep, mb.s_rep, 8 * M},
        {ma.dev_next, mb.dev_next, 4 * MD}, {ma.dev_period, mb.dev_period, 4 * MD}, {ma.dev_rep, mb.dev_rep, 4 * MD},
        {ma.q_rep, mb.q_rep, 4 * MQ}, {ma.q_start, mb.q_start, 4 * MQ},
        {src->d_obs, dst->d_obs, 4 * (size_t)src->n_vars}, {src->d_reward, dst->d_reward, 8},
        {src->d_labels, dst->d_labels, 4 * (size_t)src->n_slices}, {src->d_viol, dst->d_viol, 4 * (size_t)src->n_slices},
        {src->d_info, dst->d_info, 80 * (size_t)src->n_ran},
        {src->d_actions, dst->d_actions, with_actions ? 4 * (size_t)src->n_slices : 0},
    };
    const void* skipped[] = {a.t_cost, src->d_counters, src->ddev, src->d_st, src->d_run, src->d_counter_sum, src->d_sections,
                             src->d_redo, src->d_order, src->d_oslot, src->d_ohist, src->d_pace};
    const size_t n_src = (size_t)src->cfg.n_envs, n_dst = (size_t)dst->cfg.n_envs;
    auto region_bytes = [](const rs_handle* h, const void* p) -> size_t {
        for (auto& r : h->regions)
            if (r.first == p) return r.second;
        return 0;
    };
    for (auto& r : src->regions) {
        bool known = false;
        for (const Ent& e : copied) known = known || e.s == r.first;
        for (const void* p : skipped) known = known || p == r.first;
        if (!known) {
            src->err = "rs_fork: a state region of the handle is not classified for forking";
            return RS_ESTATE;
        }
    }
    T->n = 0;
    for (const Ent& e : copied) {
        if (e.bpr == 0 || !e.s) continue;
        if (T->n == RS_FORK_MAX || (e.bpr & 3) != 0 || e.bpr > 0xffffffffull || region_bytes(src, e.s) < e.bpr * n_src ||
            region_bytes(dst, e.d) < e.bpr * n_dst) {
            src->err = "rs_fork: internal region layout mismatch";
            return RS_ESTATE;
        }
        T->src[T->n] = (const char*)e.s;
        T->dst[T->n] = (char*)e.d;
        T->bpr[T->n] = (uint32_t)e.bpr;
        T->n++;
    }
    return RS_OK;
}

static uint64_t fork_cfg_hash(const rs_handle* h) {
    rs_config c = h->cfg;
    c.n_envs = 0;
    return fnv1a(&c, sizeof c);
}

static int fork_check(rs_handle* dst, rs_handle* src, const char* who) {
    if (fork_cfg_hash(dst) != fork_cfg_hash(src)) {
        dst->err = std::string(who) + ": the handles' configurations differ (beyond n_envs)";
        return RS_EINVAL;
    }
    if (!src->is_reset) {
        dst->err = std::string(who) + ": the source was never reset";
        return RS_ESTATE;
    }
    if (dst->device != src->device) {
        dst->err = std::string(who) + ": the handles live on different devices";
        return RS_ESTATE;
    }
    if (!fading_ready(src) || !fading_ready(dst) || dst->fad_hash != src->fad_hash) {
        dst->err = std::string(who) + ": the handles' fading tables are not identical";
        return RS_ESTATE;
    }
    return RS_OK;
}

static int fork_adopt(rs_handle* dst, const rs_handle* src) {
    if (dst->cfg.n_embb == 0)
        HIPCHK(dst, hipMemcpyAsync(dst->ddev, &dst->hdev, sizeof(RsDev), hipMemcpyHostToDevice, dst->stream));
    HIPCHK(dst, hipMemsetAsync(dst->d_counters, 0, sizeof(uint64_t) * 4 * (dst->n_tasks ? dst->n_tasks : 1), dst->stream));
    dst->clock = src->clock;
    dst->steps = src->steps;
    dst->is_reset = true;
    return RS_OK;
}

extern "C" int rs_fork(rs_handle* dst, rs_handle* src, const int32_t* src_index) {
    if (!dst || !src || !src_index) return RS_EINVAL;
    if (dst == src) {
        dst->err = "rs_fork: source and destination must be different handles";
        return RS_EINVAL;
    }
    int rc = fork_check(dst, src, "rs_fork");
    if (rc != RS_OK) return rc;
    const int n_dst = dst->cfg.n_envs;
    for (int j = 0; j < n_dst; ++j)
        if (src_index[j] < 0 || src_index[j] >= src->cfg.n_envs) {
            dst->err = "rs_fork: source index " + std::to_string(src_index[j]) + " of destination replica " + std::to_string(j) +
                       " out of range";
            return RS_EINVAL;
        }
    rs::ForkArgs a;
    memset(&a, 0, sizeof a);
    if ((rc = fork_table(dst, src, true, &a.T)) != RS_OK) {
        dst->err = src->err;
        return rc;
    }
    HIPCHK(dst, hipSetDevice(dst->device));
    drop_graph(dst);
    if ((rc = ensure_event(dst, &dst->ev_fork_in)) != RS_OK || (rc = ensure_event(dst, &dst->ev_fork_out)) != RS_OK) return rc;
    if (!dst->d_fork_idx) HIPCHK(dst, hipMalloc((void**)&dst->d_fork_idx, sizeof(int32_t) * n_dst));
    if (!dst->h_fork_idx) HIPCHK(dst, hipHostMalloc((void**)&dst->h_fork_idx, sizeof(int32_t) * n_dst, hipHostMallocDefault));
    else HIPCHK(dst, hipEventSynchronize(dst->ev_fork_out));
    memcpy(dst->h_fork_idx, src_index, sizeof(int32_t) * n_dst);
    if ((rc = stream_after(dst, &dst->ev_fork_in, src->stream, dst->stream)) != RS_OK) return rc;
    HIPCHK(dst, hipMemcpyAsync(dst->d_fork_idx, dst->h_fork_idx, sizeof(int32_t) * n_dst, hipMemcpyHostToDevice,
                               dst->stream));
    a.index = dst->d_fork_idx;
    a.n_dst = n_dst;
    a.run_src = src->d_run;
    a.run_dst = dst->d_run;
    hipLaunchKernelGGL(rs::fork_gather_kernel, dim3((unsigned)((n_dst + 3) / 4)), dim3(256), 0, dst->stream, a);
    HIPCHK(dst, hipGetLastError());
    if ((rc = fork_adopt(dst, src)) != RS_OK) return rc;
    return stream_after(dst, &dst->ev_fork_out, dst->stream, src->stream);
}

static void fork_release(rs_handle* h) {
    if (h->la) {
        rs_destroy(h->la);
        h->la = nullptr;
    }
    if (h->d_la_err) (void)hipFree(h->d_la_err);
    if (h->d_fork_idx) (void)hipFree(h->d_fork_idx);
    if (h->h_fork_idx) (void)hipHostFree(h->h_fork_idx);
    h->h_fork_idx = nullptr;
    h->d_la_err = nullptr;
    h->d_fork_idx = nullptr;
    if (h->ev_fork_in) (void)hipEventDestroy(h->ev_fork_in);
    if (h->ev_fork_out) (void)hipEventDestroy(h->ev_fork_out);
    h->ev_fork_in = h->ev_fork_out = nullptr;
}


extern "C" int rs_set_lookahead(rs_handle* h, int max_branches) {
    if (!h) return RS_EINVAL;
    if (max_branches < 0 || (max_branches > 0 && max_branches < h->cfg.n_prbs + 1)) {
        h->err = "rs_set_lookahead: max_branches must be 0 or at least n_prbs + 1";
        return RS_EINVAL;
    }
    HIPCHK(h, hipSetDevice(h->device));
    if (h->la) {
        HIPCHK(h, hipStreamSynchronize(h->stream));
        rs_destroy(h->la);
        h->la = nullptr;
    }
    h->la_max = max_branches;
    return RS_OK;
}

extern "C" int rs_set_clairvoyant_fallback(rs_handle* h, int mode) {
    if (!h || mode < 0 || mode > 1) return RS_EINVAL;
    h->la_widest = mode;
    return RS_OK;
}

static int ensure_branches(rs_handle* h) {
    if (h->la) return RS_OK;
    const long long C = h->cfg.n_prbs + 1;
    long long reps = 0x7fffffffll;
    if (h->cfg.n_embb > 0) reps = std::min(reps, 0x7fffffffll / ((long long)RS_BURSTS * RS_GROUP * h->cfg.n_embb) - 1);
    if (h->cfg.n_mmtc > 0)
        reps = std::min(reps, 0x7fffffffll / ((long long)h->cfg.n_mmtc * std::max<long long>(MTC_DEV_MAX, h->mst.cap)) - 1);
    const long long chunk = std::min<long long>(std::min<long long>(h->la_max, reps) / C, h->cfg.n_envs);
    if (chunk < 1) {
        h->err = "rs_step_clairvoyant: one replica's candidates exceed the largest branch handle";
        return RS_EINVAL;
    }
    rs_config c = h->cfg;
    c.n_envs = (int32_t)(chunk * C);
    rs_handle* b = nullptr;
    int rc = rs_create(&c, h->device, &b);
    if (rc != RS_OK) {
        h->err = std::string("rs_step_clairvoyant: creating the branch handle: ") + (b ? b->err : "");
        rs_destroy(b);
        return rc;
    }
    b->fad = h->fad;
    b->fad_valid = h->fad_valid;
    b->fad32 = h->fad32;
    b->fps = h->fps;
    b->tables_borrowed = true;
    for (int f = 0; f < RS_N_TRACES; ++f) b->fad_loaded[f] = h->fad_loaded[f];
    b->fad_hash = h->fad_hash;
    b->hdev = h->hdev;
    b->hdev.n_envs = c.n_envs;
    b->hint_auto = false;
    b->block_hint = 1;
    if (hipMemcpyAsync(b->ddev, &b->hdev, sizeof(RsDev), hipMemcpyHostToDevice, b->stream) != hipSuccess ||
        hipStreamSynchronize(b->stream) != hipSuccess || ensure_event(b, &b->ev_fork_in) != RS_OK ||
        ensure_event(b, &b->ev_fork_out) != RS_OK) {
        h->err = "rs_step_clairvoyant: setting up the branch handle failed";
        rs_destroy(b);
        return RS_EHIP;
    }
    if (!h->d_la_err) HIPCHK(h, hipMalloc((void**)&h->d_la_err, sizeof(int32_t) * h->cfg.n_envs));
    h->la = b;
    return RS_OK;
}

extern "C" int rs_step_clairvoyant(rs_handle* h, int32_t* actions_out, float* obs, double* reward, int32_t* labels,
                                   int32_t* violations) {
    if (!h) return RS_EINVAL;
    HIPCHK(h, hipSetDevice(h->device));
    if (!h->is_reset) {
        h->err = "rs_step_clairvoyant: call rs_reset first";
        return RS_ESTATE;
    }
    if (h->la_max <= 0) {
        h->err = "rs_step_clairvoyant: no lookahead capacity (rs_set_lookahead)";
        return RS_ESTATE;
    }
    if (h->clock > 2000000000 - h->cfg.slots_per_step) {
        h->err = "rs_step_clairvoyant: slot clock would overflow; reset the environment";
        return RS_ESTATE;
    }
    int rc = ensure_branches(h);
    if (rc != RS_OK) return rc;
    rs_handle* B = h->la;
    rs::ForkArgs a;
    memset(&a, 0, sizeof a);
    if ((rc = fork_table(B, h, false, &a.T)) != RS_OK) return rc;
    const int N = h->cfg.n_envs, S = h->n_slices, C = h->cfg.n_prbs + 1;
    const int chunk = B->cfg.n_envs / C;
    a.index = nullptr;
    a.n_dst = B->cfg.n_envs;
    a.run_src = h->d_run;
    a.run_dst = B->d_run;
    a.C = C;
    a.n_act = S;
    a.n_prbs = h->cfg.n_prbs;
    a.acts_src = h->d_actions;
    a.acts_dst = B->d_actions;
    if ((rc = stream_after(h, &B->ev_fork_in, h->stream, B->stream)) != RS_OK) return rc;
    HIPCHK(h, hipMemsetAsync(h->d_la_err, 0, sizeof(int32_t) * N, B->stream));
    for (int s = 0; s < S; ++s)
        for (int c0 = 0; c0 < N; c0 += chunk) {
            a.c0 = c0;
            a.cnt = std::min(chunk, N - c0);
            a.s = s;
            hipLaunchKernelGGL(rs::fork_gather_kernel, dim3((unsigned)((a.n_dst + 3) / 4)), dim3(256), 0, B->stream, a);
            HIPCHK(h, hipGetLastError());
            B->clock = h->clock;
            B->steps = h->steps;
            B->is_reset = true;
            if ((rc = launch_step(B)) != RS_OK) {
                h->err = "rs_step_clairvoyant: branch step: " + B->err;
                return rc;
            }
            hipLaunchKernelGGL(rs::clairvoyant_select_kernel, dim3((unsigned)((a.cnt + 3) / 4)), dim3(256), 0, B->stream,
                               (const int32_t*)B->d_viol, (const int32_t*)B->st.err, C, c0, a.cnt, s, S, h->cfg.n_prbs,
                               h->la_widest, h->d_actions, h->d_la_err);
            HIPCHK(h, hipGetLastError());
        }
    if ((rc = stream_after(h, &B->ev_fork_out, B->stream, h->stream)) != RS_OK) return rc;
    if ((rc = launch_step(h)) != RS_OK) return rc;
    if ((rc = rs_fetch(h, actions_out, obs, reward, labels, violations)) != RS_OK) return rc;
    std::vector<int32_t> e((size_t)N);
    HIPCHK(h, hipMemcpyAsync(e.data(), h->d_la_err, sizeof(int32_t) * N, hipMemcpyDeviceToHost, h->stream));
    HIPCHK(h, hipStreamSynchronize(h->stream));
    for (int i = 0; i < N; ++i)
        if (e[i]) {
            h->err = "capacity exceeded in a lookahead branch of replica " + std::to_string(i) + ":" +
                     ((e[i] & 1) ? " UEs per slice" : "") + ((e[i] & 2) ? " active VBR bursts per UE" : "") +
                     ((e[i] & 4) ? " backlogged mMTC devices" : "");
            return RS_EOVERFLOW;
        }
    return RS_OK;
}
```

network-slicing_amd/csrc/rs_order.hip:

```cpp
#pragma once
#include <hip/hip_runtime.h>
#include <stdint.h>

#include "rs_device.h"

namespace rs {

#define RS_ORDER_BINS 2048

__device__ __forceinline__ int order_key(int mode, int n_ue, int n_prb, int cost) {
    int key;
    mode = mode > 3 ? mode - 3 : mode;
    if (mode == 4) key = ((n_ue * n_prb) >> 2) + 2 * cost;
    else if (mode == 5) key = cost;
    else if (mode == 2) key = n_ue * 64 + (n_prb >> 2);
    else if (mode == 3) key = n_ue * n_prb + cost;
    else key = n_ue * n_prb;
    key = key < 0 ? 0 : key;
    return key < RS_ORDER_BINS ? key : RS_ORDER_BINS - 1;
}

__global__ __launch_bounds__(256) void order_key_kernel(const RsDev* __restrict__ D, const RsState* __restrict__ Sp,
                                                        const int32_t* __restrict__ actions, int mode, int* hist,
                                                        uint64_t* slot, int4 kw, int split_ue) {
    __shared__ int cnt[RS_ORDER_BINS];
    for (int k = threadIdx.x; k < RS_ORDER_BINS; k += 256) cnt[k] = 0;
    __syncthreads();
    const int n_tasks = D->n_envs * D->n_embb;
    const int task = (int)(blockIdx.x * blockDim.x + threadIdx.x);
    int bin = 0, local = 0;
    if (task < n_tasks) {
        const int rep = task / D->n_embb, sl = task - rep * D->n_embb;
        const int n_prb = actions[rep * D->n_slices + sl];
        int key;
        if (kw.w > 0 || kw.x != 16 || kw.y != 16 || kw.z != 0) {
            const int n_ue = Sp->t_n_ue[task];
            int need_rb = 0;
            if (kw.w > 0) {
                for (int u = 0; u < n_ue && u < RS_GROUP; ++u) {
                    const double q = Sp->u_queue[(size_t)task * RS_GROUP + u];
                    int li = Sp->u_e_snr[(size_t)task * RS_GROUP + u] - D->lut_lo;
                    li = li < 0 ? 0 : (li >= D->lut_n ? D->lut_n - 1 : li);
                    const int rate = D->lut_rate[li] > 0 ? D->lut_rate[li] : 1;
                    const double rb = q / (double)rate;
                    need_rb += rb < 100000.0 ? (int)rb : 100000;
                }
            }
            int drain = n_prb > 0 ? need_rb / n_prb : 0;
            drain = drain < 50 ? drain : 50;
            key = (kw.x * (n_ue * n_prb) + kw.y * Sp->t_cost[task] + kw.z * n_ue + kw.w * drain * (n_ue + 1)) >> 4;
            key = key < 0 ? 0 : (key < RS_ORDER_BINS ? key : RS_ORDER_BINS - 1);
        } else {
            key = order_key(mode, Sp->t_n_ue[task], n_prb, Sp->t_cost[task]);
        }
        if (split_ue > 0) key = (Sp->t_n_ue[task] >= split_ue ? RS_ORDER_BINS / 2 : 0) + ((key >> 1) < RS_ORDER_BINS / 2 ? (key >> 1) : RS_ORDER_BINS / 2 - 1);
        bin = RS_ORDER_BINS - 1 - key;
        local = atomicAdd(&cnt[bin], 1);
    }
    __syncthreads();
    if (task < n_tasks && local == 0) cnt[bin] = atomicAdd(&hist[bin], cnt[bin]);
    __syncthreads();
    if (task < n_tasks) slot[task] = (uint64_t)bin | ((uint64_t)(cnt[bin] + local) << 11);
}

__global__ __launch_bounds__(256) void order_scatter_kernel(const RsDev* __restrict__ D, const int* __restrict__ hist,
                                                            int* hist_next, const uint64_t* __restrict__ slot,
                                                            int32_t* order, int pair, int tpw, int snake, int snake_mask, int rot_mask,
                                                            int seg_lo, int seg_hi) {
    __shared__ int start[RS_ORDER_BINS];
    __shared__ int part[256];
    constexpr int PER = RS_ORDER_BINS / 256;
    int loc[PER];
    int s = 0;
#pragma unroll
    for (int k = 0; k < PER; ++k) {
        loc[k] = s;
        s += hist[threadIdx.x * PER + k];
    }
    part[threadIdx.x] = s;
    __syncthreads();
    int incl = s;
    for (int d = 1; d < 256; d <<= 1) {
        const int o = (int)threadIdx.x >= d ? part[threadIdx.x - d] : 0;
        __syncthreads();
        incl += o;
        part[threadIdx.x] = incl;
        __syncthreads();
    }
    const int excl = incl - s;
#pragma unroll
    for (int k = 0; k < PER; ++k) start[threadIdx.x * PER + k] = excl + loc[k];
    __syncthreads();
    if (blockIdx.x == 0)
        for (int k = threadIdx.x; k < RS_ORDER_BINS; k += 256) hist_next[k] = 0;
    const int n_all = D->n_envs * D->n_embb;
    const int task = (int)(blockIdx.x * blockDim.x + threadIdx.x);
    if (task >= n_all) return;
    const uint64_t v = slot[task];
    int p = start[(int)(v & (RS_ORDER_BINS - 1))] + (int)(v >> 11);
    if (p < seg_lo || p >= seg_hi) {
        order[p] = task;
        return;
    }
    const int n_tasks = seg_hi - seg_lo;
    p -= seg_lo;
    if (pair > 0 && tpw > 1 && n_tasks % tpw == 0) {
        const int W = n_tasks / tpw;
        const int Hw = (int)(((long long)W * pair) >> 8);
        if (p < Hw) p = tpw * p;
        else if (p >= n_tasks - (tpw - 1) * Hw) {
            const int q = n_tasks - 1 - p;
            p = tpw * (q / (tpw - 1)) + 1 + q % (tpw - 1);
        } else {
            p = tpw * Hw + (p - Hw);
        }
    }
    if (snake > 0 && tpw > 0) {
        int Wv = p / tpw;
        const int in = p - Wv * tpw, k = Wv / snake;
        if (((snake_mask >> (k & 31)) & 1) != 0 && (k + 1) * snake <= n_tasks / tpw) Wv = k * snake + (snake - 1 - (Wv - k * snake));
        if (((rot_mask >> (k & 31)) & 1) != 0 && (k + 1) * snake <= n_tasks / tpw) Wv = k * snake + (Wv - k * snake + snake / 2) % snake;
        p = Wv * tpw + in;
    }
    order[seg_lo + p] = task;
}

}
```

network-slicing_amd/csrc/rs_policy_io.hip:

```cpp

namespace rs {

struct FrontArgs {
    const RsDev* D;
    int32_t kind;
    const void* in;
    const int32_t* table;
    int32_t n_table;
    int32_t* actions;
    int32_t* resources;
    unsigned long long* rejected;
    int32_t* cursor;
    int32_t hist_steps;
};

__global__ __launch_bounds__(256) void policy_front_kernel(FrontArgs a) {
    const int r = blockIdx.x * blockDim.x + threadIdx.x;
    const int N = a.D->n_envs, S = a.D->n_act, n_prbs = a.D->n_prbs;
    if (r == 0 && a.cursor && *a.cursor <= a.hist_steps) *a.cursor += 1;
    if (r >= N) return;
    int32_t row[8];
    bool ok = true;
    if (a.kind == RS_ACT_PRBS) {
        const int32_t* in = (const int32_t*)a.in + (size_t)r * S;
// ... 99 lines not shown
    int32_t* total_viol = nullptr;
    unsigned long long* rejected = nullptr;
    int32_t* cursor = nullptr;
    int32_t* table = nullptr;
    int32_t n_table = 0;
    int32_t hist_steps = 0;
    int16_t* h_viol = nullptr;
    double* h_reward = nullptr;
    int16_t* h_res = nullptr;
    hipEvent_t ev_in = nullptr, ev_out = nullptr;
    std::vector<void*> allocs;
};

template <class T>
static int pio_alloc(rs_handle* h, T** p, size_t n) {
    void* q = nullptr;
    const size_t bytes = sizeof(T) * (n ? n : 1);
    HIPCHK(h, guarded_malloc(&q, bytes, &h->guarded));
    HIPCHK(h, hipMemsetAsync(q, 0, bytes, h->stream));
    if (!guards_on()) h->pio->allocs.push_back(q);
    *p = (T*)q;
    return RS_OK;
}

static int pio_create(rs_handle* h) {
    PolicyIo* p = h->pio;
    const size_t N = (size_t)h->cfg.n_envs, S = (size_t)h->n_slices;
    int rc;
    if ((rc = pio_alloc(h, &p->in_prbs, N * S)) != RS_OK) return rc;
    if ((rc = pio_alloc(h, &p->in_shares, N * (S + 1))) != RS_OK) return rc;
    if ((rc = pio_alloc(h, &p->in_index, N)) != RS_OK) return rc;
    if ((rc = pio_alloc(h, &p->resources, N)) != RS_OK) return rc;
    if ((rc = pio_alloc(h, &p->obs_norm, N * h->n_vars)) != RS_OK) return rc;
    if ((rc = pio_alloc(h, &p->total_viol, N)) != RS_OK) return rc;
    if ((rc = pio_alloc(h, &p->rejected, 1)) != RS_OK) return rc;
    if ((rc = pio_alloc(h, &p->cursor, 1)) != RS_OK) return rc;
    HIPCHK(h, hipEventCreateWithFlags(&p->ev_in, hipEventDisableTiming));
    HIPCHK(h, hipEventCreateWithFlags(&p->ev_out, hipEventDisableTiming));
    return RS_OK;
}

static void policy_io_release(rs_handle* h);

static int pio_ensure(rs_handle* h) {
    if (h->pio) return RS_OK;
    HIPCHK(h, hipSetDevice(h->device));
    h->pio = new PolicyIo();
    const int rc = pio_create(h);
    if (rc != RS_OK) policy_io_release(h);
    return rc;
}

static void pio_free_history(PolicyIo* p) {
    if (p->h_viol) (void)hipFree(p->h_viol);
    if (p->h_reward) (void)hipFree(p->h_reward);
    if (p->h_res) (void)hipFree(p->h_res);
    p->h_viol = p->h_res = nullptr;
    p->h_reward = nullptr;
    p->hist_steps = 0;
}

static void policy_io_release(rs_handle* h) {
    PolicyIo* p = h->pio;
    if (!p) return;
    pio_free_history(p);
    if (p->table) (void)hipFree(p->table);
    for (void* q : p->allocs) (void)hipFree(q);
    if (p->ev_in) (void)hipEventDestroy(p->ev_in);
    if (p->ev_out) (void)hipEventDestroy(p->ev_out);
    delete p;
    h->pio = nullptr;
}

static int policy_io_on_reset(rs_handle* h) {
    PolicyIo* p = h->pio;
    if (!p) return RS_OK;
    HIPCHK(h, hipMemsetAsync(p->rejected, 0, sizeof(unsigned long long), h->stream));
    HIPCHK(h, hipMemsetAsync(p->cursor, 0, sizeof(int32_t), h->stream));
    return RS_OK;
}

extern "C" int rs_get_device_view(rs_handle* h, rs_device_view* out) {
    if (!h || !out) return RS_EINVAL;
    int rc = pio_ensure(h);
    if (rc != RS_OK) return rc;
    const PolicyIo* p = h->pio;
    memset(out, 0, sizeof *out);
    out->device = h->device;
    out->n_envs = h->cfg.n_envs;
    out->n_slices = h->n_slices;
    out->n_vars = h->n_vars;
    out->stream = (void*)h->stream;
    out->in_prbs = p->in_prbs;
    out->in_shares = p->in_shares;
    out->in_index = p->in_index;
    out->actions = h->d_actions;
    out->resources = p->resources;
    out->obs = h->d_obs;
    out->obs_norm = p->obs_norm;
    out->reward = h->d_reward;
    out->labels = h->d_labels;
    out->violations = h->d_viol;
    out->total_violations = p->total_viol;
    out->rejected = (int64_t*)p->rejected;
    return RS_OK;
}

extern "C" int rs_step_device(rs_handle* h, int kind, const void* actions_device, void* caller_stream) {
    if (!h || !actions_device) return RS_EINVAL;
    if (kind != RS_ACT_PRBS && kind != RS_ACT_SHARES && kind != RS_ACT_INDEX) {
        h->err = "rs_step_device: unknown action kind";
        return RS_EINVAL;
    }
    if (h->n_slices > 8) {
        h->err = "rs_step_device: at most 8 action entries per replica";
        return RS_EINVAL;
    }
    if (!h->is_reset) {
        h->err = "rs_step_device: call rs_reset first";
        return RS_ESTATE;
    }
    int rc = pio_ensure(h);
    if (rc != RS_OK) return rc;
    PolicyIo* p = h->pio;
    if (kind == RS_ACT_INDEX && !p->table) {
        h->err = "rs_step_device: RS_ACT_INDEX needs an action table (rs_set_action_table)";
        return RS_ESTATE;
    }
    HIPCHK(h, hipSetDevice(h->device));
    if (h->hint_auto) {
        const int want = auto_hint(h);
        if (want != h->block_hint) {
            h->block_hint = want;
            drop_graph(h);
        }
    }
    hipStream_t cs = (hipStream_t)caller_stream;
    const bool foreign = cs != h->stream;
    if (foreign && (rc = stream_after(h, &p->ev_in, cs, h->stream)) != RS_OK) return rc;
    const unsigned nb = (unsigned)((h->cfg.n_envs + 255) / 256);
    rs::FrontArgs f;
    f.D = h->ddev;
    f.kind = kind;
    f.in = actions_device;
    f.table = p->table;
    f.n_table = p->n_table;
    f.actions = h->d_actions;
    f.resources = p->resources;
    f.rejected = p->rejected;
    f.cursor = p->cursor;
    f.hist_steps = p->hist_steps;
    hipLaunchKernelGGL(rs::policy_front_kernel, dim3(nb), dim3(256), 0, h->stream, f);
    if ((rc = launch_step(h)) != RS_OK) return rc;
    rs::BackArgs b;
    b.D = h->ddev;
    b.obs = h->d_obs;
    b.obs_norm = p->obs_norm;
    b.viol = h->d_viol;
    b.reward = h->d_reward;
    b.resources = p->resources;
    b.total_viol = p->total_viol;
    b.cursor = p->cursor;
    b.hist_steps = p->hist_steps;
    b.h_viol = p->h_viol;
    b.h_reward = p->h_reward;
    b.h_res = p->h_res;
    const size_t quads = ((size_t)h->cfg.n_envs * h->n_vars + 3) / 4;
    size_t blocks = (quads + 255) / 256;
    if (blocks < nb) blocks = nb;
    if (blocks > 2048) blocks = 2048;
    hipLaunchKernelGGL(rs::policy_back_kernel, dim3((unsigned)blocks), dim3(256), 0, h->stream, b);
    HIPCHK(h, hipGetLastError());
    return foreign ? stream_after(h, &p->ev_out, h->stream, cs) : RS_OK;
}

extern "C" int rs_stream_join(rs_handle* h, void* caller_stream) {
    if (!h) return RS_EINVAL;
    hipStream_t cs = (hipStream_t)caller_stream;
    if (cs == h->stream) return RS_OK;
    int rc = pio_ensure(h);
    if (rc != RS_OK) return rc;
    HIPCHK(h, hipSetDevice(h->device));
    return stream_after(h, &h->pio->ev_out, h->stream, cs);
}

extern "C" int rs_set_action_table(rs_handle* h, const int32_t* table, int32_t n_actions) {
    if (!h || !table || n_actions <= 0) return RS_EINVAL;
    int rc = pio_ensure(h);
    if (rc != RS_OK) return rc;
    PolicyIo* p = h->pio;
    HIPCHK(h, hipSetDevice(h->device));
    HIPCHK(h, hipStreamSynchronize(h->stream));
    if (p->table) (void)hipFree(p->table);
    p->table = nullptr;
    p->n_table = 0;
    const size_t bytes = sizeof(int32_t) * (size_t)n_actions * h->n_slices;
    HIPCHK(h, hipMalloc((void**)&p->table, bytes));
    HIPCHK(h, hipMemcpy(p->table, table, bytes, hipMemcpyHostToDevice));
    p->n_table = n_actions;
    return RS_OK;
}

static int pio_new_history(rs_handle* h, int32_t steps, int16_t** v, double** rw, int16_t** rs_) {
    const size_t n = (size_t)h->cfg.n_envs * (size_t)steps;
    HIPCHK(h, hipMalloc((void**)v, sizeof(int16_t) * (n ? n : 1)));
    HIPCHK(h, hipMalloc((void**)rw, sizeof(double) * (n ? n : 1)));
    HIPCHK(h, hipMalloc((void**)rs_, sizeof(int16_t) * (n ? n : 1)));
    if (n) {
        HIPCHK(h, hipMemsetAsync(*v, 0, sizeof(int16_t) * n, h->stream));
        HIPCHK(h, hipMemsetAsync(*rw, 0, sizeof(double) * n, h->stream));
        HIPCHK(h, hipMemsetAsync(*rs_, 0, sizeof(int16_t) * n, h->stream));
    }
    return RS_OK;
}

extern "C" int rs_report_begin(rs_handle* h, int32_t steps) {
    if (!h || steps < 0) return RS_EINVAL;
    int rc = pio_ensure(h);
    if (rc != RS_OK) return rc;
    PolicyIo* p = h->pio;
    HIPCHK(h, hipSetDevice(h->device));
    HIPCHK(h, hipStreamSynchronize(h->stream));
    pio_free_history(p);
    if ((rc = pio_new_history(h, steps, &p->h_viol, &p->h_reward, &p->h_res)) != RS_OK) return rc;
    p->hist_steps = steps;
    HIPCHK(h, hipMemsetAsync(p->cursor, 0, sizeof(int32_t), h->stream));
    return RS_OK;
}

extern "C" int rs_report_extend(rs_handle* h, int32_t eval_steps) {
    if (!h || eval_steps < 0) return RS_EINVAL;
    PolicyIo* p = h->pio;
    if (!p || !p->h_viol) {
        h->err = "rs_report_extend: no report history (rs_report_begin)";
        return RS_ESTATE;
    }
    HIPCHK(h, hipSetDevice(h->device));
    const int32_t old = p->hist_steps, now = old + eval_steps;
    const size_t N = (size_t)h->cfg.n_envs;
    int16_t *v = nullptr, *r = nullptr;
    double* w = nullptr;
    int rc = pio_new_history(h, now, &v, &w, &r);
    if (rc != RS_OK) return rc;
    if (old > 0) {
        HIPCHK(h, hipMemcpy2DAsync(v, sizeof(int16_t) * now, p->h_viol, sizeof(int16_t) * old, sizeof(int16_t) * old, N, hipMemcpyDeviceToDevice, h->stream));
        HIPCHK(h, hipMemcpy2DAsync(w, sizeof(double) * now, p->h_reward, sizeof(double) * old, sizeof(double) * old, N, hipMemcpyDeviceToDevice, h->stream));
        HIPCHK(h, hipMemcpy2DAsync(r, sizeof(int16_t) * now, p->h_res, sizeof(int16_t) * old, sizeof(int16_t) * old, N, hipMemcpyDeviceToDevice, h->stream));
    }
    HIPCHK(h, hipMemcpyAsync(p->cursor, &old, sizeof(int32_t), hipMemcpyHostToDevice, h->stream));
    HIPCHK(h, hipStreamSynchronize(h->stream));
    pio_free_history(p);
    p->h_viol = v;
    p->h_reward = w;
    p->h_res = r;
    p->hist_steps = now;
    return RS_OK;
}

extern "C" int rs_report_fetch(rs_handle* h, int16_t* violation, double* reward, int16_t* resources, int32_t* n_recorded) {
    if (!h) return RS_EINVAL;
    PolicyIo* p = h->pio;
    if (!p || !p->h_viol) {
        h->err = "rs_report_fetch: no report history (rs_report_begin)";
        return RS_ESTATE;
    }
    HIPCHK(h, hipSetDevice(h->device));
    const size_t n = (size_t)h->cfg.n_envs * (size_t)p->hist_steps;
    int32_t cur = 0;
    if (violation && n) HIPCHK(h, hipMemcpyAsync(violation, p->h_viol, sizeof(int16_t) * n, hipMemcpyDeviceToHost, h->stream));
    if (reward && n) HIPCHK(h, hipMemcpyAsync(reward, p->h_reward, sizeof(double) * n, hipMemcpyDeviceToHost, h->stream));
    if (resources && n) HIPCHK(h, hipMemcpyAsync(resources, p->h_res, sizeof(int16_t) * n, hipMemcpyDeviceToHost, h->stream));
    HIPCHK(h, hipMemcpyAsync(&cur, p->cursor, sizeof(int32_t), hipMemcpyDeviceToHost, h->stream));
    HIPCHK(h, hipStreamSynchronize(h->stream));
    if (n_recorded) *n_recorded = cur < p->hist_steps ? cur : p->hist_steps;
    return RS_OK;
}

extern "C" int rs_device_copy(rs_handle* h, void* dst, const void* src, uint64_t bytes, int to_device) {
    if (!h || (bytes && (!dst || !src))) return RS_EINVAL;
    HIPCHK(h, hipSetDevice(h->device));
    if (bytes == 0) return RS_OK;
    HIPCHK(h, hipMemcpyAsync(dst, src, (size_t)bytes, to_device ? hipMemcpyHostToDevice : hipMemcpyDeviceToHost, h->stream));
    if (!to_device) HIPCHK(h, hipStreamSynchronize(h->stream));
    return RS_OK;
}
```

network-slicing_amd/ranslice/_lib.py:

```python
import ctypes as C
import os

from .config import RsConfig, KbConfig

_HERE = os.path.dirname(os.path.abspath(__file__))
LIB_PATH = os.environ.get('RANSLICE_LIB', os.path.join(os.path.dirname(_HERE), 'csrc', 'build', 'libranslice.so'))
DEV_LIB_PATH = os.path.join(os.path.dirname(LIB_PATH), 'libranslice_dev.so')

RS_OK, RS_EINVAL, RS_EOVERFLOW, RS_EHIP, RS_ESTATE = 0, -1, -2, -3, -4

KB_EXPORTS = (
    'kb_create', 'kb_destroy', 'kb_last_error', 'kb_reset', 'kb_update_control', 'kb_select_action',
    'kb_step_resident', 'kb_run_resident', 'kb_predict', 'kb_update', 'kb_get_learner', 'kb_get_control', 'kb_set_adjusted',
    'kb_comm_info', 'kb_get_stats', 'kb_get_sizes', 'kb_get_pool', 'kb_state_bytes', 'kb_save_state', 'kb_load_state', 'kb_get_flags', 'kb_get_repair_work', 'kb_get_kernel_row', 'kb_shared_scan', 'kb_shared_apply', 'kb_shared_commit', 'kb_comm_unique_id', 'kb_comm_init', 'kb_shared_step', 'kb_shared_step_resident', 'kb_shared_merge', 'kb_history_begin', 'kb_history_fetch', 'kb_kernel_time_ms', 'kb_phase_times_ms', 'kb_repair_times_ms', 'kb_kernel_times_ms', 'kb_set_kernel_timing', 'kb_synchronize',
    'kb_fork', 'kb_deploy', 'kb_set_learning',
    'kb_prune', 'kb_get_pruned', 'kb_prune_time_ms', 'kb_get_prune_work',
    'kb_shared_prune',
    'kb_deploy_ref',
    'kb_export_bytes', 'kb_export_agents', 'kb_agents_info', 'kb_import_agents', 'kb_agents_kernel_times',
    'kb_fork_rebuild', 'kb_get_rebuild', 'kb_rebuild_time_ms',
    'kb_unshare', 'kb_share', 'kb_bridge_time_ms',
    'kb_fit', 'kb_score', 'kb_fit_time_ms',
    'kb_set_algorithm', 'kb_get_algorithm',
    'kb_set_fit_wide', 'kb_get_fit_wide', 'kb_fit_wide_info',
    'kb_set_fit_wide_plus', 'kb_get_fit_wide_plus',
    'kb_fit_steps',
    'kb_set_control_plus', 'kb_get_control_plus',
    'kb_set_control_plus_batch', 'kb_get_control_plus_batch', 'kb_control_plus_batch_info',
    'kb_set_control_plus_wide', 'kb_get_control_plus_wide', 'kb_control_plus_wide_info',
    'kb_set_fit_steps_batch', 'kb_get_fit_steps_batch', 'kb_fit_steps_batch_info',
    'kb_set_shared_plus', 'kb_get_shared_plus',
    'kb_set_shared_plus_batch', 'kb_get_shared_plus_batch', 'kb_shared_plus_batch_info',
)

EXPORTS = (
    'rs_create', 'rs_load_fading', 'rs_reset', 'rs_step', 'rs_step_resident', 'rs_random_actions', 'rs_fetch',
    'rs_get_info', 'rs_set_alloc_trace', 'rs_get_alloc_trace', 'rs_get_counters', 'rs_get_rx_stats', 'rs_set_group_size', 'rs_set_schedule_hint', 'rs_get_section_profile', 'rs_get_task_profile', 'rs_run_random', 'rs_kernel_time_ms', 'rs_kernel_time_stats_ms',
    'rs_set_kernel_timing', 'rs_synchronize', 'rs_state_bytes', 'rs_save_state', 'rs_load_state', 'rs_device_count', 'rs_device_mem_info', 'rs_n_vars', 'rs_n_slices', 'rs_last_error', 'rs_destroy',
    'rs_fork', 'rs_set_lookahead', 'rs_step_clairvoyant', 'rs_set_clairvoyant_fallback',
    'rs_get_device_view', 'rs_step_device', 'rs_stream_join', 'rs_set_action_table', 'rs_report_begin', 'rs_report_extend',
    'rs_report_fetch', 'rs_device_copy',
) + KB_EXPORTS

RS_ACT_PRBS, RS_ACT_SHARES, RS_ACT_INDEX = 0, 1, 2


class RsDeviceView(C.Structure):
    _fields_ = [('device', C.c_int32), ('n_envs', C.c_int32), ('n_slices', C.c_int32), ('n_vars', C.c_int32),
                ('stream', C.c_void_p),
                ('in_prbs', C.c_void_p), ('in_shares', C.c_void_p), ('in_index', C.c_void_p),
                ('actions', C.c_void_p), ('resources', C.c_void_p),
                ('obs', C.c_void_p), ('obs_norm', C.c_void_p),
                ('reward', C.c_void_p), ('labels', C.c_void_p), ('violations', C.c_void_p), ('total_violations', C.c_void_p),
                ('rejected', C.c_void_p)]


class RanSliceError(RuntimeError):
    def __init__(self, code, msg):
        super().__init__('libranslice error %d: %s' % (code, msg))
        self.code = code


_libs = {}


def device_count():
    n = load().rs_device_count()
    if n < 0:
        raise RanSliceError(n, 'hipGetDeviceCount failed')
    return n


def device_mem_info(device=0):
    f, t = C.c_uint64(), C.c_uint64()
    rc = load().rs_device_mem_info(int(device), C.byref(f), C.byref(t))
    if rc < 0:
        raise RanSliceError(rc, 'hipMemGetInfo failed')
    return int(f.value), int(t.value)


def default_pool_bytes(device=0, headroom=24 << 30, floor=8 << 30):
    free, _ = device_mem_info(device)
    return max(int(floor), int(free) - int(headroom))


def load(dev=None):
    if dev is None:
        dev = os.environ.get('RANSLICE_DEV_BUILD') == '1'
    path = DEV_LIB_PATH if dev else LIB_PATH
    if path in _libs:
        return _libs[path]
    if not os.path.exists(path):
        raise ImportError('%s not found: build it with `make -C network-slicing_amd/csrc` '
                          '(hipcc, gfx950). There is no CPU fallback.' % path)
    os.environ.setdefault('GPU_MAX_HW_QUEUES', '24')
    L = C.CDLL(path)
    vp, ip, dp = C.c_void_p, C.POINTER(C.c_int32), C.POINTER(C.c_double)
    fp, up = C.POINTER(C.c_float), C.POINTER(C.c_uint64)
    L.rs_create.argtypes = [C.POINTER(RsConfig), C.c_int, C.POINTER(vp)]
    L.rs_load_fading.argtypes = [vp, C.c_int, dp, C.c_int, C.c_int]
    L.rs_reset.argtypes = [vp, up, fp]
    L.rs_step.argtypes = [vp, ip, fp, dp, ip, ip]
    L.rs_step_resident.argtypes = [vp]
    L.rs_random_actions.argtypes = [vp, C.c_uint64, C.c_uint64]
    L.rs_run_random.argtypes = [vp, C.c_uint64, C.c_uint64, C.c_int, C.c_int]
    L.rs_fetch.argtypes = [vp, ip, fp, dp, ip, ip]
    L.rs_get_info.argtypes = [vp, dp]
    L.rs_set_alloc_trace.argtypes = [vp, C.c_int]
    L.rs_get_alloc_trace.argtypes = [vp, vp]
    L.rs_get_counters.argtypes = [vp, up]
    L.rs_get_rx_stats.argtypes = [vp, up]
    L.rs_get_section_profile.argtypes = [vp, up]
    L.rs_get_task_profile.argtypes = [vp, up]
    L.rs_set_group_size.argtypes = [vp, C.c_int]
    L.rs_set_schedule_hint.argtypes = [vp, C.c_int]
    L.rs_kernel_time_ms.argtypes = [vp, dp, C.POINTER(C.c_int64)]
    L.rs_kernel_time_stats_ms.argtypes = [vp, dp, C.POINTER(C.c_int64)]
    L.rs_set_kernel_timing.argtypes = [vp, C.c_int]
    L.rs_synchronize.argtypes = [vp]
    L.rs_n_vars.argtypes = [vp]
    L.rs_n_slices.argtypes = [vp]
    L.rs_last_error.argtypes = [vp]
    L.rs_last_error.restype = C.c_char_p
    L.rs_destroy.argtypes = [vp]
    L.rs_destroy.restype = None
    L.rs_fork.argtypes = [vp, vp, ip]
    L.rs_set_lookahead.argtypes = [vp, C.c_int]
    L.rs_set_clairvoyant_fallback.argtypes = [vp, C.c_int]
    L.rs_step_clairvoyant.argtypes = [vp, ip, fp, dp, ip, ip]
    L.rs_get_device_view.argtypes = [vp, C.POINTER(RsDeviceView)]
    L.rs_step_device.argtypes = [vp, C.c_int, vp, vp]
    L.rs_stream_join.argtypes = [vp, vp]
    L.rs_set_action_table.argtypes = [vp, ip, C.c_int32]
    L.rs_report_begin.argtypes = [vp, C.c_int32]
    L.rs_report_extend.argtypes = [vp, C.c_int32]
    L.rs_report_fetch.argtypes = [vp, C.POINTER(C.c_int16), dp, C.POINTER(C.c_int16), ip]
    L.rs_device_copy.argtypes = [vp, vp, vp, C.c_uint64, C.c_int]
    i64p = C.POINTER(C.c_int64)
    L.kb_create.argtypes = [C.POINTER(KbConfig), C.c_int, C.POINTER(vp)]
    L.kb_destroy.argtypes = [vp]
    L.kb_destroy.restype = None
    L.kb_last_error.argtypes = [vp]
    L.kb_last_error.restype = C.c_char_p
    L.kb_reset.argtypes = [vp, ip, ip, up]
    L.kb_update_control.argtypes = [vp, fp, ip, ip, ip]
    L.kb_select_action.argtypes = [vp, fp, ip, ip]
    L.kb_step_resident.argtypes = [vp, vp]
    L.kb_run_resident.argtypes = [vp, vp, C.c_int, C.c_int]
    L.kb_predict.argtypes = [vp, C.c_int, C.c_int, dp, ip, dp]
    L.kb_update.argtypes = [vp, C.c_int, C.c_int, dp, C.c_int32, ip, dp]
    L.kb_get_learner.argtypes = [vp, C.c_int, C.c_int, ip, dp, dp, dp]
    L.kb_get_control.argtypes = [vp, ip, ip, ip, ip, dp]
    L.kb_set_adjusted.argtypes = [vp, ip]
    L.kb_get_stats.argtypes = [vp, up]
    L.kb_get_sizes.argtypes = [vp, ip]
    L.kb_get_pool.argtypes = [vp, up, up, ip, ip]
    L.kb_get_repair_work.argtypes = [vp, up]
    for _n in ('rs', 'kb'):
        getattr(L, _n + '_state_bytes').argtypes = [vp, up]
        getattr(L, _n + '_save_state').argtypes = [vp, vp, C.c_uint64]
        getattr(L, _n + '_load_state').argtypes = [vp, vp, C.c_uint64]
    L.kb_get_flags.argtypes = [vp, ip]
    L.kb_get_kernel_row.argtypes = [vp, C.c_int, C.c_int, ip, dp]
    L.kb_shared_scan.argtypes = [vp, fp, ip, ip, C.c_int32, C.c_int32, ip, ip, dp]
    L.kb_shared_apply.argtypes = [vp, ip, dp, C.c_int32]
    L.kb_shared_commit.argtypes = [vp, ip]
    sp = C.POINTER(C.c_int16)
    L.kb_history_begin.argtypes = [vp, C.c_int32]
    L.kb_history_fetch.argtypes = [vp, dp, sp, sp, sp, sp, sp, ip]
    L.kb_comm_unique_id.argtypes = [vp]
    L.kb_comm_init.argtypes = [vp, vp, C.c_int, C.c_int]
    L.kb_comm_info.argtypes = [vp, C.POINTER(C.c_int), C.POINTER(C.c_int)]
    L.kb_shared_step.argtypes = [vp, fp, ip, ip, C.c_int32, C.c_int32, ip, ip]
    L.kb_shared_step_resident.argtypes = [vp, vp, C.c_int32, C.c_int32, ip]
    L.kb_shared_merge.argtypes = [vp, dp, C.c_int32, C.c_int32, C.c_int32, dp, ip, ip, ip]
    L.rs_device_count.argtypes = []
    L.rs_device_mem_info.argtypes = [C.c_int, up, up]
    L.kb_kernel_time_ms.argtypes = [vp, dp, i64p]
    L.kb_phase_times_ms.argtypes = [vp, dp, i64p]
    L.kb_repair_times_ms.argtypes = [vp, dp, i64p]
    L.kb_kernel_times_ms.argtypes = [vp, dp, i64p]
    L.kb_set_kernel_timing.argtypes = [vp, C.c_int]
    L.kb_synchronize.argtypes = [vp]
    L.kb_fork.argtypes = [vp, vp, ip]
    L.kb_deploy.argtypes = [vp, ip, C.c_int32, C.POINTER(vp)]
    L.kb_deploy_ref.argtypes = [vp, ip, C.c_int32, C.POINTER(vp)]
    L.kb_set_learning.argtypes = [vp, C.c_int]
    L.kb_export_bytes.argtypes = [vp, ip, C.c_int32, up]
    L.kb_export_agents.argtypes = [vp, ip, C.c_int32, vp, C.c_uint64]
    L.kb_agents_info.argtypes = [vp, C.c_uint64, C.POINTER(KbConfig), ip]
    L.kb_import_agents.argtypes = [vp, C.c_uint64, C.c_int, C.POINTER(vp)]
    L.kb_agents_kernel_times.argtypes = [dp, up]
    L.kb_fork_rebuild.argtypes = [vp, vp, ip]
    L.kb_get_rebuild.argtypes = [vp, dp, up]
    L.kb_rebuild_time_ms.argtypes = [vp, dp]
    L.kb_unshare.argtypes = [vp, vp, ip]
    L.kb_share.argtypes = [vp, vp, C.c_int32, ip]
    L.kb_bridge_time_ms.argtypes = [vp, dp, up]
# ... 41 lines not shown
```

network-slicing_amd/ranslice/vec_env.py:

```python
import ctypes as C

import numpy as np

from . import _lib
from .config import RsAllocRec, make_config, n_vars
from .device_io import DeviceArray, describe
from .fading import synth_fading
from .sharding import replica_seeds

_dp = C.POINTER(C.c_double)
_ip = C.POINTER(C.c_int32)
_fp = C.POINTER(C.c_float)
_up = C.POINTER(C.c_uint64)


def default_fading(n_cols=10000, seed=20240):
    return [synth_fading(t, n_cols, seed=seed) for t in range(3)]


class VecRanSlice:
    def __init__(self, n_envs=1, scenario=0, seed=0, device=0, fading=None, cfg=None, **cfg_kw):
        self.L = _lib.load()
        self.cfg = cfg if cfg is not None else make_config(scenario, n_envs=n_envs, **cfg_kw)
        self.cfg.n_envs = n_envs
# ... 93 lines not shown
        self._check(self.L.rs_get_device_view(self.h, C.byref(v)))
        N, S, V = self.n_envs, self.n_slices, self.n_variables
        spec = dict(in_prbs=((N, S), np.int32), in_shares=((N, S + 1), np.float32), in_index=((N,), np.int64),
                    actions=((N, S), np.int32), resources=((N,), np.int32), obs=((N, V), np.float32),
                    obs_norm=((N, V), np.float32), reward=((N,), np.float64), labels=((N, S), np.int32),
                    violations=((N, S), np.int32), total_violations=((N,), np.int32), rejected=((1,), np.int64))
        out = {k: DeviceArray(getattr(v, k), shape, dt, owner=self) for k, (shape, dt) in spec.items()}
        out['stream'] = int(v.stream or 0)
        return out

    def _action_kind(self, shape, dtype):
        N, S = self.n_envs, self.n_slices
        if dtype == np.int32 and shape in ((N, S), (N * S,)):
            return _lib.RS_ACT_PRBS
        if dtype == np.float32 and shape in ((N, S + 1), (N * (S + 1),)):
            return _lib.RS_ACT_SHARES
        if dtype == np.int64 and shape in ((N,), (N, 1)):
            return _lib.RS_ACT_INDEX
        raise ValueError('step_device: %s %s fits no action kind (int32 [%d, %d] PRBs, float32 [%d, %d] shares, int64 [%d] '
                         'table rows)' % (dtype, shape, N, S, N, S + 1, N))

    def step_device(self, actions, kind=None, stream=0):
        ptr, shape, dtype = describe(actions)
        if shape is not None and dtype is not None:
            fits = self._action_kind(shape, dtype)
            if kind is None:
                kind = fits
            elif int(kind) != fits:
                raise ValueError('step_device: %s %s is not the layout of action kind %d' % (dtype, shape, int(kind)))
        elif kind is None:
            raise ValueError('step_device: a bare pointer needs an explicit kind')
        self._check(self.L.rs_step_device(self.h, int(kind), C.c_void_p(ptr), C.c_void_p(int(stream) or None)))

    def stream_join(self, stream=0):
        self._check(self.L.rs_stream_join(self.h, C.c_void_p(int(stream) or None)))

    def set_action_table(self, table):
        table = np.ascontiguousarray(table, dtype=np.int32)
        if table.ndim != 2 or table.shape[1] != self.n_slices or table.shape[0] == 0:
            raise ValueError('set_action_table: expected [n_actions, %d], got %s' % (self.n_slices, table.shape))
        self._check(self.L.rs_set_action_table(self.h, table.ctypes.data_as(_ip), table.shape[0]))

    def rejected_rows(self):
        return int(self.device_view()['rejected'].get()[0])

    def fork_from(self, src, index):
        index = np.ascontiguousarray(index, dtype=np.int32)
        if index.shape != (self.n_envs,):
            raise ValueError('fork_from: index must have n_envs = %d entries' % self.n_envs)
        self._check(self.L.rs_fork(self.h, src.h, index.ctypes.data_as(_ip)))

    def set_lookahead(self, max_branches=None):
        if max_branches is None:
            n = C.c_uint64()
            self._check(self.L.rs_state_bytes(self.h, C.byref(n)))
            per_replica = max(1, n.value // self.n_envs)
            free, _ = _lib.device_mem_info(self.device)
            cand = self.n_prbs + 1
            max_branches = int(min(self.n_envs * cand, max(cand, (free // 4) // per_replica)))
        self._check(self.L.rs_set_lookahead(self.h, int(max_branches)))
        self._lookahead = int(max_branches)

    def set_clairvoyant_fallback(self, mode):
        mode = {'cheapest': 0, 'widest': 1}.get(mode, mode)
        self._check(self.L.rs_set_clairvoyant_fallback(self.h, int(mode)))

    def step_clairvoyant(self):
        if not getattr(self, '_lookahead', 0):
            self.set_lookahead()
        actions = np.zeros((self.n_envs, self.n_slices), dtype=np.int32)
        self._check(self.L.rs_step_clairvoyant(self.h, actions.ctypes.data_as(_ip), self._obs.ctypes.data_as(_fp),
                                               self._reward.ctypes.data_as(_dp), self._labels.ctypes.data_as(_ip),
                                               self._viol.ctypes.data_as(_ip)))
        return actions, self._obs.copy(), self._reward.copy(), self._labels.copy(), self._viol.copy()

    def l1_info(self):
        info = np.zeros((self.n_envs, self.n_ran, 10), dtype=np.float64)
        self._check(self.L.rs_get_info(self.h, info.ctypes.data_as(_dp)))
        return info

    def set_group_size(self, lanes):
        self._check(self.L.rs_set_group_size(self.h, int(lanes)))

    def set_schedule_hint(self, mode):
        self._check(self.L.rs_set_schedule_hint(self.h, int(mode)))

    def set_alloc_trace(self, enable=True):
        self._check(self.L.rs_set_alloc_trace(self.h, int(bool(enable))))

    def alloc_trace(self):
        shape = ((self.n_envs, self.cfg.slots_per_step, 64) if self.multiplexed
                 else (self.n_envs, self.cfg.n_embb, self.cfg.slots_per_step, 32))
        tr = np.zeros(shape, dtype=np.dtype(RsAllocRec))
        self._check(self.L.rs_get_alloc_trace(self.h, tr.ctypes.data_as(C.c_void_p)))
        return tr

    def counters(self):
        c = (C.c_uint64 * 4)()
        self._check(self.L.rs_get_counters(self.h, c))
        return [int(x) for x in c]

    def rx_stats(self):
        c = (C.c_uint64 * 3)()
        self._check(self.L.rs_get_rx_stats(self.h, c))
        return int(c[0]), int(c[1]), bool(c[2])

    def set_kernel_timing(self, enable=True):
        self._check(self.L.rs_set_kernel_timing(self.h, int(bool(enable))))

    def kernel_time_stats_ms(self):
        st = (C.c_double * 3)()
        n = C.c_int64()
        self._check(self.L.rs_kernel_time_stats_ms(self.h, st, C.byref(n)))
        return (st[0], st[1], st[2]), n.value

    def kernel_time_ms(self):
        ms = C.c_double()
        n = C.c_int64()
        self._check(self.L.rs_kernel_time_ms(self.h, C.byref(ms), C.byref(n)))
        return ms.value, n.value
```

Baseline: 4.904 million.

## Split replicas into independent stream lanes for concurrent step pipelines

Adds a lane mode that partitions environment replicas across several streams. Each lane runs its own ordering, step and finalize kernels over a replica range, with private run counters, pace and histogram buffers. The aim is to overlap small per-step launches and fill the GPU when task counts are moderate. Lanes are closed, streams rejoined and the global order rebuilt before any other API touches state. This adds synchronization complexity and risks divergence in shared counters and ordering.

```diff
diff --git a/include/ranslice.h b/include/ranslice.h
--- a/include/ranslice.h
+++ b/include/ranslice.h
@@ -96,6 +96,9 @@
 int rs_kernel_time_stats_ms(rs_handle* h, double out[3], int64_t* launches);
 int rs_set_kernel_timing(rs_handle* h, int enable);
 
+int rs_set_lanes(rs_handle* h, int n);
+int rs_get_lane_info(rs_handle* h, double out[4]);
+
 int rs_set_group_size(rs_handle* h, int lanes);
 
 int rs_set_schedule_hint(rs_handle* h, int mode);
diff --git a/network-slicing_amd/csrc/kb_api.hip b/network-slicing_amd/csrc/kb_api.hip
--- a/network-slicing_amd/csrc/kb_api.hip
+++ b/network-slicing_amd/csrc/kb_api.hip
@@ -758,6 +758,7 @@
 
 extern "C" int kb_step_resident(kb_handle* k, rs_handle* env) {
     if (!k || !env) return RS_EINVAL;
+    if (lanes_close(env) != RS_OK) return RS_EHIP;
     if (!k->is_reset || env->cfg.n_envs != k->cfg.n_envs || env->n_slices != k->cfg.n_slices || env->n_vars != k->nv ||
         env->device != k->device) {
         k->err = "kb_step_resident: agent and environment do not match (or kb_reset missing)";
@@ -815,6 +816,7 @@
 
 extern "C" int kb_run_resident(kb_handle* k, rs_handle* env, int n_steps, int use_graph) {
     if (!k || !env || n_steps < 0) return RS_EINVAL;
+    if (lanes_close(env) != RS_OK) return RS_EHIP;
     int done = 0, rc;
     if (k->learning && (rc = kb_refuse_plus(k, "kb_run_resident")) != RS_OK) return rc;
     static const bool no_graph = getenv("ROCP_TOOL_LIBRARIES") != nullptr &&
@@ -1392,6 +1394,7 @@
 
 extern "C" int kb_shared_step_resident(kb_handle* k, rs_handle* env, int32_t budget, int32_t max_rounds, int32_t* rounds_out) {
     if (!k || !env || budget <= 0 || max_rounds <= 0) return RS_EINVAL;
+    if (lanes_close(env) != RS_OK) return RS_EHIP;
     if (!k->D.shared || !k->is_reset || env->cfg.n_envs != k->cfg.n_envs || env->n_slices != k->cfg.n_slices ||
         env->n_vars != k->nv || env->device != k->device || budget > k->budget_cap) {
         k->err = "kb_shared_step_resident: agent and environment do not match (or not a reset shared-dictionary agent, or budget > 256)";
diff --git a/network-slicing_amd/csrc/rs_api.hip b/network-slicing_amd/csrc/rs_api.hip
--- a/network-slicing_amd/csrc/rs_api.hip
+++ b/network-slicing_amd/csrc/rs_api.hip
@@ -1,6 +1,7 @@
 
 #include <hip/hip_runtime.h>
 
+#include <algorithm>
 #include <cmath>
 #include <cstdio>
 #include <cstdlib>
@@ -143,6 +144,22 @@
     int32_t* d_la_err = nullptr;
     struct PolicyIo* pio = nullptr;
     EventSpans spans;
+    struct Lane {
+        hipStream_t stream = nullptr;
+        bool own_stream = false;
+        int rep0 = 0, n_rep = 0;
+        int64_t* run = nullptr;
+        int* hist = nullptr;
+        unsigned long long* pace = nullptr;
+        void* mem = nullptr;
+        hipEvent_t ev_open = nullptr, ev_done = nullptr;
+    };
+    std::vector<Lane> lanes;
+    int lanes_req = 0;
+    int lanes_open = 0;
+    uint64_t lane_steps = 0;
+    hipEvent_t ev_ref = nullptr;
+    double lane_info[4] = {1.0, 0.0, 0.0, 0.0};
     std::string err;
 };
 
@@ -248,10 +265,11 @@
 }
 
 __global__ void finalize_kernel(const RsDev* D, const int32_t* actions, const int32_t* viol, double* reward,
-                                int64_t* run) {
+                                int64_t* run, int rep0, int n_rep) {
     int r = blockIdx.x * blockDim.x + threadIdx.x;
-    if (r >= D->n_envs) return;
-    if (r == 0) {
+    if (r >= n_rep) return;
+    r += rep0;
+    if (r == rep0) {
         run[0] += D->slots;
         run[1] += 1;
     }
@@ -270,14 +288,14 @@
 }
 
 __global__ __launch_bounds__(256) void random_actions_kernel(const RsDev* D, int32_t* actions, uint64_t seed,
-                                                           uint64_t step, const int64_t* run) {
+                                                           uint64_t step, const int64_t* run, int rep0, int n_rep) {
     if (run) {
         step = (uint64_t)run[1];
         seed = (uint64_t)run[2];
     }
     const int lane = threadIdx.x & 63;
-    const int r = blockIdx.x * 4 + (threadIdx.x >> 6);
-    if (r >= D->n_envs) return;
+    const int r = rep0 + blockIdx.x * 4 + (threadIdx.x >> 6);
+    if (r >= rep0 + n_rep) return;
     const int S = D->n_act;
     int my_bin[8];
     int cnt = 0;
@@ -561,6 +579,7 @@
     if (const char* e = dev_env("RANSLICE_MIXED")) h->mixed = atoi(e);
     if (const char* e = dev_env("RANSLICE_MIXED_UE")) h->mixed_ue = atoi(e);
     if (const char* e = dev_env("RANSLICE_MIXED_LIGHT")) h->mixed_light = atoi(e);
+    if (const char* e = dev_env("RANSLICE_LANES")) h->lanes_req = atoi(e) > 0 ? atoi(e) : 0;
     if (h->mixed > 0 || h->mixed_light < 256) {
         HIPCHK(h, hipStreamCreateWithFlags(&h->side2, hipStreamNonBlocking));
         HIPCHK(h, hipEventCreateWithFlags(&h->ev_fork2, hipEventDisableTiming));
@@ -584,13 +603,17 @@
 }
 
 static void fork_release(rs_handle* h);
+static int lanes_close(rs_handle* h);
+static void lanes_release(rs_handle* h);
 static void policy_io_release(rs_handle* h);
 static int policy_io_on_reset(rs_handle* h);
 
 extern "C" void rs_destroy(rs_handle* h) {
     if (!h) return;
+    (void)lanes_close(h);
     if (h->stream) (void)hipStreamSynchronize(h->stream);
     drop_graph(h);
+    lanes_release(h);
     fork_release(h);
     policy_io_release(h);
     if (guards_on()) check_guards(h->guarded, "rs");
@@ -743,6 +766,7 @@
 
 extern "C" int rs_load_fading(rs_handle* h, int trace_id, const double* data, int rows, int cols) {
     if (!h) return RS_EINVAL;
+    if (lanes_close(h) != RS_OK) return RS_EHIP;
     if (trace_id < 0 || trace_id >= RS_N_TRACES || !data || rows <= 0 || cols <= 0 || h->cfg.n_prbs > 2 * rows) {
         h->err = "rs_load_fading: bad arguments";
         return RS_EINVAL;
@@ -791,6 +815,7 @@
 
 extern "C" int rs_reset(rs_handle* h, const uint64_t* seeds, float* obs) {
     if (!h || !seeds) return RS_EINVAL;
+    if (lanes_close(h) != RS_OK) return RS_EHIP;
     HIPCHK(h, hipSetDevice(h->device));
     if (!fading_ready(h)) {
         h->err = "rs_reset: fading traces not loaded";
@@ -838,7 +863,35 @@
     return a;
 }
 
-static int launch_step(rs_handle* h) {
+static void launch_embb(const rs_handle* h, StepArgs& a, int g, hipStream_t lstream) {
+    if (a.order_cnt < 0) a.spread = (h->spread_mode == 1 || (h->spread_mode < 0 && h->n_tasks <= h->spread_max)) ? 1 : 0;
+    const int per_block = a.spread ? 4 : 256 / g;
+    const int n_mine = a.order_cnt >= 0 ? a.order_cnt : h->n_tasks;
+    dim3 grid((n_mine + per_block - 1) / per_block), block(256);
+    const bool tr = h->trace_on;
+#define RS_LAUNCH_STEP(G_, TR_, BL_)                                                                              \
+    do {                                                                                                          \
+        if (h->hdev.pf_div_fast)                                                                                  \
+            hipLaunchKernelGGL((embb_step_kernel<G_, TR_, BL_, true>), grid, block, 0, lstream, a);             \
+        else                                                                                                      \
+            hipLaunchKernelGGL((embb_step_kernel<G_, TR_, BL_, false>), grid, block, 0, lstream, a);            \
+    } while (0)
+    if (g == 8) {
+        if (tr) RS_LAUNCH_STEP(8, true, true);
+        else if (h->block_hint) RS_LAUNCH_STEP(8, false, true);
+        else RS_LAUNCH_STEP(8, false, false);
+    } else if (g == 16) {
+        if (tr) RS_LAUNCH_STEP(16, true, true);
+        else if (h->block_hint) RS_LAUNCH_STEP(16, false, true);
+        else RS_LAUNCH_STEP(16, false, false);
+    } else {
+        if (tr) RS_LAUNCH_STEP(32, true, true);
+        else RS_LAUNCH_STEP(32, false, true);
+    }
+#undef RS_LAUNCH_STEP
+}
+
+static int step_ready(rs_handle* h) {
     if (!h->is_reset) {
         h->err = "rs_step: call rs_reset first";
         return RS_ESTATE;
@@ -847,6 +900,12 @@
         h->err = "rs_step: slot clock would overflow; reset the environment";
         return RS_ESTATE;
     }
+    return RS_OK;
+}
+
+static int launch_step(rs_handle* h) {
+    const int ready = step_ready(h);
+    if (ready != RS_OK) return ready;
     if (h->mux) {
         if (h->n_tasks > 0) {
             StepArgs a = step_args(h);
@@ -871,7 +930,7 @@
             hipLaunchKernelGGL(rs::mtc_mux_step_kernel, dim3((unsigned)h->cfg.n_envs), dim3(64), lds, h->stream, ma);
         }
         hipLaunchKernelGGL(finalize_kernel, dim3((h->cfg.n_envs + 255) / 256), dim3(256), 0, h->stream, h->ddev,
-                           h->d_actions, h->d_viol, h->d_reward, h->d_run);
+                           h->d_actions, h->d_viol, h->d_reward, h->d_run, 0, h->cfg.n_envs);
         HIPCHK(h, hipGetLastError());
         h->clock += h->cfg.slots_per_step;
         h->steps += 1;
@@ -891,33 +950,7 @@
         a.pace = h->d_pace;
         a.order_cnt = -1;
         hipStream_t lstream = h->stream;
-        auto launch = [&](int g) {
-            if (a.order_cnt < 0) a.spread = (h->spread_mode == 1 || (h->spread_mode < 0 && h->n_tasks <= h->spread_max)) ? 1 : 0;
-            const int per_block = a.spread ? 4 : 256 / g;
-            const int n_mine = a.order_cnt >= 0 ? a.order_cnt : h->n_tasks;
-            dim3 grid((n_mine + per_block - 1) / per_block), block(256);
-            const bool tr = h->trace_on;
-#define RS_LAUNCH_STEP(G_, TR_, BL_)                                                                              \
-    do {                                                                                                          \
-        if (h->hdev.pf_div_fast)                                                                                  \
-            hipLaunchKernelGGL((embb_step_kernel<G_, TR_, BL_, true>), grid, block, 0, lstream, a);             \
-        else                                                                                                      \
-            hipLaunchKernelGGL((embb_step_kernel<G_, TR_, BL_, false>), grid, block, 0, lstream, a);            \
-    } while (0)
-            if (g == 8) {
-                if (tr) RS_LAUNCH_STEP(8, true, true);
-                else if (h->block_hint) RS_LAUNCH_STEP(8, false, true);
-                else RS_LAUNCH_STEP(8, false, false);
-            } else if (g == 16) {
-                if (tr) RS_LAUNCH_STEP(16, true, true);
-                else if (h->block_hint) RS_LAUNCH_STEP(16, false, true);
-                else RS_LAUNCH_STEP(16, false, false);
-            } else {
-                if (tr) RS_LAUNCH_STEP(32, true, true);
-                else RS_LAUNCH_STEP(32, false, true);
-            }
-#undef RS_LAUNCH_STEP
-        };
+        auto launch = [&](int g) { launch_embb(h, a, g, lstream); };
         int seg_head = 0, seg_light = 0;
         if (h->order_mode > 0) {
             const int par = h->order_par;
@@ -932,11 +965,11 @@
             const int seg_mid = h->n_tasks - seg_head - seg_light;
             hipLaunchKernelGGL(order_key_kernel, dim3(nb), dim3(256), 0, h->stream, h->ddev, h->d_st, h->d_actions,
                                h->order_mode, h->d_ohist + par * RS_ORDER_BINS, h->d_oslot, make_int4(h->key_w[0], h->key_w[1], h->key_w[2], h->key_w[3]),
-                               split ? h->mixed_ue : 0);
+                               split ? h->mixed_ue : 0, 0, h->n_tasks, 0);
             hipLaunchKernelGGL(order_scatter_kernel, dim3(nb), dim3(256), 0, h->stream, h->ddev,
                                h->d_ohist + par * RS_ORDER_BINS, h->d_ohist + (1 - par) * RS_ORDER_BINS, h->d_oslot,
                                h->d_order, h->order_mode > 3 ? h->order_pair : 0, 64 / h->group,
-                               h->snake == 1 ? h->spread_max : h->snake, h->snake_mask, h->rot_mask, seg_head, seg_head + seg_mid);
+                               h->snake == 1 ? h->spread_max : h->snake, h->snake_mask, h->rot_mask, seg_head, seg_head + seg_mid, 0, h->n_tasks);
             a.order = h->d_order;
         }
         hipEvent_t e1;
@@ -990,7 +1023,7 @@
     if (forked) HIPCHK(h, hipStreamWaitEvent(h->stream, h->ev_join, 0));
     else if (h->cfg.n_mmtc > 0) mtc_step(h, &h->mst, h->stream);
     hipLaunchKernelGGL(finalize_kernel, dim3((h->cfg.n_envs + 255) / 256), dim3(256), 0, h->stream, h->ddev,
-                       h->d_actions, h->d_viol, h->d_reward, h->d_run);
+                       h->d_actions, h->d_viol, h->d_reward, h->d_run, 0, h->cfg.n_envs);
     HIPCHK(h, hipGetLastError());
     h->clock += h->cfg.slots_per_step;
     h->steps += 1;
@@ -1000,6 +1033,170 @@
 static int auto_hint(const rs_handle* h) {
     const int gran = h->cfg.pf_granularity > 0 ? h->cfg.pf_granularity : 1;
     return h->cfg.n_prbs / (h->n_slices + 1) >= RS_HINT_PAIRS * gran ? 1 : 0;
+}
+
+static const int kLanesAuto = 2;
+static const int kLanesMax = 8;
+
+static int lanes_wanted(const rs_handle* h) {
+    const bool legal = !h->mux && h->cfg.n_mmtc == 0 && !h->trace_on && h->n_tasks > 0 && h->order_mode > 0 && h->mixed == 0 &&
+                       h->mixed_light >= 256;
+    if (!legal || h->lanes_req == 1) return 1;
+    int want = h->lanes_req;
+    if (want == 0) want = (h->group == 16 && h->n_tasks < 49152 && h->n_tasks >= 4 * h->spread_max) ? kLanesAuto : 1;
+    if (want > h->cfg.n_envs) want = h->cfg.n_envs;
+    return want < kLanesMax ? want : kLanesMax;
+}
+
+static int lanes_ensure(rs_handle* h, int L) {
+    while ((int)h->lanes.size() < L) {
+        const int l = (int)h->lanes.size();
+        rs_handle::Lane ln;
+        if (l == 0) {
+            ln.stream = h->stream;
+            ln.run = h->d_run;
+            ln.hist = h->d_ohist;
+            ln.pace = h->d_pace;
+        } else {
+            hipStream_t idle[3] = {h->side, h->side2, h->side3};
+            for (int k = 0, seen = 0; k < 3 && !ln.stream; ++k)
+                if (idle[k] && ++seen == l) ln.stream = idle[k];
+            if (!ln.stream) {
+                HIPCHK(h, hipStreamCreateWithFlags(&ln.stream, hipStreamNonBlocking));
+                ln.own_stream = true;
+            }
+            const size_t bytes = sizeof(int64_t) * 4 + sizeof(unsigned long long) * 4 + sizeof(int) * 2 * RS_ORDER_BINS;
+            const hipError_t e = hipMalloc(&ln.mem, bytes);
+            if (e != hipSuccess) {
+                if (ln.own_stream) (void)hipStreamDestroy(ln.stream);
+                h->err = std::string("hipMalloc (lane): ") + hipGetErrorString(e);
+                return RS_EHIP;
+            }
+            ln.run = (int64_t*)ln.mem;
+            ln.pace = (unsigned long long*)(ln.run + 4);
+            ln.hist = (int*)(ln.pace + 4);
+        }
+        h->lanes.push_back(ln);
+    }
+    return RS_OK;
+}
+
+static void lanes_release(rs_handle* h) {
+    for (auto& ln : h->lanes) {
+        if (ln.ev_open) (void)hipEventDestroy(ln.ev_open);
+        if (ln.ev_done) (void)hipEventDestroy(ln.ev_done);
+        if (ln.own_stream) (void)hipStreamDestroy(ln.stream);
+        if (ln.mem) (void)hipFree(ln.mem);
+    }
+    h->lanes.clear();
+    if (h->ev_ref) (void)hipEventDestroy(h->ev_ref);
+    h->ev_ref = nullptr;
+}
+
+static int lanes_open(rs_handle* h) {
+    if (h->lanes_open) return RS_OK;
+    const int L = lanes_wanted(h);
+    if (L < 2) return RS_OK;
+    int rc = lanes_ensure(h, L);
+    if (rc != RS_OK) return rc;
+    const int N = h->cfg.n_envs;
+    for (int l = 0, r = 0; l < L; ++l) {
+        rs_handle::Lane& ln = h->lanes[l];
+        ln.rep0 = r;
+        ln.n_rep = N / L + (l < N % L ? 1 : 0);
+        r += ln.n_rep;
+        if (l == 0) continue;
+        HIPCHK(h, hipMemcpyAsync(ln.run, h->d_run, sizeof(int64_t) * 4, hipMemcpyDeviceToDevice, h->stream));
+        HIPCHK(h, hipMemcpyAsync(ln.pace, h->d_pace, sizeof(unsigned long long) * 4, hipMemcpyDeviceToDevice, h->stream));
+        HIPCHK(h, hipMemsetAsync(ln.hist, 0, sizeof(int) * 2 * RS_ORDER_BINS, h->stream));
+    }
+    for (int l = 1; l < L; ++l)
+        if ((rc = stream_after(h, &h->lanes[l].ev_open, h->stream, h->lanes[l].stream)) != RS_OK) return rc;
+    h->lanes_open = L;
+    h->lane_steps = 0;
+    return RS_OK;
+}
+
+static int lanes_close(rs_handle* h) {
+    if (!h || !h->lanes_open) return RS_OK;
+    HIPCHK(h, hipSetDevice(h->device));
+    const int L = h->lanes_open;
+    h->lanes_open = 0;
+    for (int l = 1; l < L; ++l) {
+        const int rc = stream_after(h, &h->lanes[l].ev_done, h->lanes[l].stream, h->stream);
+        if (rc != RS_OK) return rc;
+    }
+    if (h->lane_steps > 0) {
+        const int par = h->order_par ^ 1;
+        const unsigned nb = (unsigned)((h->n_tasks + 255) / 256);
+        HIPCHK(h, hipMemsetAsync(h->d_ohist + par * RS_ORDER_BINS, 0, sizeof(int) * RS_ORDER_BINS, h->stream));
+        hipLaunchKernelGGL(order_key_kernel, dim3(nb), dim3(256), 0, h->stream, h->ddev, h->d_st, h->d_actions, h->order_mode,
+                           h->d_ohist + par * RS_ORDER_BINS, h->d_oslot, make_int4(h->key_w[0], h->key_w[1], h->key_w[2], h->key_w[3]),
+                           0, 0, h->n_tasks, 1);
+        hipLaunchKernelGGL(order_scatter_kernel, dim3(nb), dim3(256), 0, h->stream, h->ddev, h->d_ohist + par * RS_ORDER_BINS,
+                           h->d_ohist + (1 - par) * RS_ORDER_BINS, h->d_oslot, h->d_order, h->order_mode > 3 ? h->order_pair : 0,
+                           64 / h->group, h->snake == 1 ? h->spread_max : h->snake, h->snake_mask, h->rot_mask, 0, h->n_tasks, 0,
+                           h->n_tasks);
+        HIPCHK(h, hipGetLastError());
+    }
+    return RS_OK;
+}
+
+static int lanes_actions(rs_handle* h, uint64_t seed, uint64_t step_index, bool scripted) {
+    const int rc = lanes_open(h);
+    if (rc != RS_OK) return rc;
+    const int L = h->lanes_open ? h->lanes_open : 1;
+    for (int l = 0; l < L; ++l) {
+        const int rep0 = h->lanes_open ? h->lanes[l].rep0 : 0, n_rep = h->lanes_open ? h->lanes[l].n_rep : h->cfg.n_envs;
+        const int64_t* run = !scripted ? nullptr : (h->lanes_open ? h->lanes[l].run : h->d_run);
+        hipLaunchKernelGGL(random_actions_kernel, dim3((n_rep + 3) / 4), dim3(256), 0, h->lanes_open ? h->lanes[l].stream : h->stream,
+                           h->ddev, h->d_actions, seed, step_index, run, rep0, n_rep);
+    }
+    HIPCHK(h, hipGetLastError());
+    return RS_OK;
+}
+
+static int lanes_step(rs_handle* h) {
+    if (!h->lanes_open) return launch_step(h);
+    const int ready = step_ready(h);
+    if (ready != RS_OK) return ready;
+    const int L = h->lanes_open, par = h->order_par;
+    h->order_par ^= 1;
+    for (int l = 0; l < L; ++l) {
+        const rs_handle::Lane& ln = h->lanes[l];
+        const int task0 = ln.rep0 * h->cfg.n_embb, cnt = ln.n_rep * h->cfg.n_embb;
+        const unsigned nb = (unsigned)((cnt + 255) / 256);
+        hipLaunchKernelGGL(order_key_kernel, dim3(nb), dim3(256), 0, ln.stream, h->ddev, h->d_st, h->d_actions, h->order_mode,
+                           ln.hist + par * RS_ORDER_BINS, h->d_oslot, make_int4(h->key_w[0], h->key_w[1], h->key_w[2], h->key_w[3]), 0,
+                           task0, cnt, 0);
+        hipLaunchKernelGGL(order_scatter_kernel, dim3(nb), dim3(256), 0, ln.stream, h->ddev, ln.hist + par * RS_ORDER_BINS,
+                           ln.hist + (1 - par) * RS_ORDER_BINS, h->d_oslot, h->d_order, h->order_mode > 3 ? h->order_pair : 0,
+                           64 / h->group, h->snake == 1 ? h->spread_max : h->snake, h->snake_mask, h->rot_mask, 0, cnt, task0, cnt);
+        StepArgs a = step_args(h);
+        a.run = ln.run;
+        a.sections = h->d_sections;
+        a.redo = h->d_redo;
+        a.pace = ln.pace;
+        a.order = h->d_order;
+        a.order_off = task0;
+        a.order_cnt = cnt;
+        a.spread = (h->spread_mode == 1 || (h->spread_mode < 0 && h->n_tasks <= h->spread_max)) ? 1 : 0;
+        hipEvent_t e1;
+        HIPCHK(h, h->spans.begin(ln.stream, l | (L << 8), &e1));
+        launch_embb(h, a, h->group, ln.stream);
+        if (e1) HIPCHK(h, hipEventRecord(e1, ln.stream));
+        if (h->group < 32) {
+            a.replay = 1;
+            launch_embb(h, a, 32, ln.stream);
+        }
+        hipLaunchKernelGGL(finalize_kernel, dim3((ln.n_rep + 255) / 256), dim3(256), 0, ln.stream, h->ddev, h->d_actions, h->d_viol,
+                           h->d_reward, ln.run, ln.rep0, ln.n_rep);
+    }
+    HIPCHK(h, hipGetLastError());
+    h->clock += h->cfg.slots_per_step;
+    h->steps += 1;
+    h->lane_steps += 1;
+    return RS_OK;
 }
 
 static int check_errors(rs_handle* h) {
@@ -1019,6 +1216,7 @@
 extern "C" int rs_fetch(rs_handle* h, int32_t* actions, float* obs, double* reward, int32_t* labels,
                         int32_t* violations) {
     if (!h) return RS_EINVAL;
+    if (lanes_close(h) != RS_OK) return RS_EHIP;
     HIPCHK(h, hipSetDevice(h->device));
     const size_t N = (size_t)h->cfg.n_envs, S = (size_t)h->n_slices;
     if (actions) HIPCHK(h, hipMemcpyAsync(actions, h->d_actions, sizeof(int32_t) * N * S, hipMemcpyDeviceToHost, h->stream));
@@ -1032,6 +1230,7 @@
 extern "C" int rs_step(rs_handle* h, const int32_t* actions, float* obs, double* reward, int32_t* labels,
                        int32_t* violations) {
     if (!h || !actions) return RS_EINVAL;
+    if (lanes_close(h) != RS_OK) return RS_EHIP;
     HIPCHK(h, hipSetDevice(h->device));
     const size_t N = (size_t)h->cfg.n_envs, S = (size_t)h->n_slices;
     size_t wide = 0;
@@ -1067,7 +1266,7 @@
 extern "C" int rs_step_resident(rs_handle* h) {
     if (!h) return RS_EINVAL;
     HIPCHK(h, hipSetDevice(h->device));
-    return launch_step(h);
+    return lanes_step(h);
 }
 
 extern "C" int rs_random_actions(rs_handle* h, uint64_t seed, uint64_t step_index) {
@@ -1078,10 +1277,7 @@
         return RS_EINVAL;
     }
     if (h->cfg.n_prbs > 512) return RS_EINVAL;
-    hipLaunchKernelGGL(random_actions_kernel, dim3((h->cfg.n_envs + 3) / 4), dim3(256), 0, h->stream, h->ddev,
-                       h->d_actions, seed, step_index, (const int64_t*)nullptr);
-    HIPCHK(h, hipGetLastError());
-    return RS_OK;
+    return lanes_actions(h, seed, step_index, false);
 }
 
 static void drop_graph(rs_handle* h) {
@@ -1092,9 +1288,13 @@
     h->graph = nullptr;
 }
 
-static int enqueue_scripted_step(rs_handle* h) {
+static int enqueue_scripted_step(rs_handle* h, bool laned) {
+    if (laned) {
+        const int rc = lanes_actions(h, 0, 0, true);
+        return rc != RS_OK ? rc : lanes_step(h);
+    }
     hipLaunchKernelGGL(random_actions_kernel, dim3((h->cfg.n_envs + 3) / 4), dim3(256), 0, h->stream, h->ddev,
-                       h->d_actions, (uint64_t)0, (uint64_t)0, (const int64_t*)h->d_run);
+                       h->d_actions, (uint64_t)0, (uint64_t)0, (const int64_t*)h->d_run, 0, h->cfg.n_envs);
     return launch_step(h);
 }
 
@@ -1113,11 +1313,12 @@
         h->err = "rs_run_random: slot clock would overflow; reset the environment";
         return RS_ESTATE;
     }
+    int done = 0, rc;
+    if ((rc = lanes_close(h)) != RS_OK) return rc;
     hipLaunchKernelGGL(set_run_kernel, dim3(1), dim3(1), 0, h->stream, h->d_run, seed, step_index0);
-    int done = 0, rc;
     if (use_graph && !h->spans.on && n_steps >= 2) {
         if (h->gexec && h->graph_par != h->order_par) {
-            if ((rc = enqueue_scripted_step(h)) != RS_OK) return rc;
+            if ((rc = enqueue_scripted_step(h, false)) != RS_OK) return rc;
             done += 1;
         }
         if (!h->gexec) {
@@ -1125,8 +1326,8 @@
             const uint64_t steps0 = h->steps;
             h->graph_par = h->order_par;
             HIPCHK(h, hipStreamBeginCapture(h->stream, hipStreamCaptureModeThreadLocal));
-            const int rc1 = enqueue_scripted_step(h);
-            const int rc2 = rc1 == RS_OK ? enqueue_scripted_step(h) : rc1;
+            const int rc1 = enqueue_scripted_step(h, false);
+            const int rc2 = rc1 == RS_OK ? enqueue_scripted_step(h, false) : rc1;
             const hipError_t ec = hipStreamEndCapture(h->stream, &h->graph);
             h->clock = clock0;
             h->steps = steps0;
@@ -1145,13 +1346,14 @@
             done += 2;
         }
     }
-    for (; done < n_steps; ++done)
-        if ((rc = enqueue_scripted_step(h)) != RS_OK) return rc;
+    for (const bool laned = done == 0; done < n_steps; ++done)
+        if ((rc = enqueue_scripted_step(h, laned)) != RS_OK) return rc;
     return RS_OK;
 }
 
 extern "C" int rs_get_info(rs_handle* h, double* info) {
     if (!h || !info) return RS_EINVAL;
+    if (lanes_close(h) != RS_OK) return RS_EHIP;
     HIPCHK(h, hipSetDevice(h->device));
     HIPCHK(h, hipMemcpyAsync(info, h->d_info, sizeof(double) * (size_t)h->cfg.n_envs * h->n_ran * 10,
                              hipMemcpyDeviceToHost, h->stream));
@@ -1161,6 +1363,7 @@
 
 extern "C" int rs_set_alloc_trace(rs_handle* h, int enable) {
     if (!h) return RS_EINVAL;
+    if (lanes_close(h) != RS_OK) return RS_EHIP;
     HIPCHK(h, hipSetDevice(h->device));
     if (enable && !h->d_trace) {
         size_t n = (size_t)h->n_tasks * h->cfg.slots_per_step * RS_GROUP;
@@ -1174,6 +1377,7 @@
 
 extern "C" int rs_get_alloc_trace(rs_handle* h, rs_alloc_rec* out) {
     if (!h || !out || !h->d_trace) return RS_EINVAL;
+    if (lanes_close(h) != RS_OK) return RS_EHIP;
     HIPCHK(h, hipSetDevice(h->device));
     size_t n = (size_t)h->n_tasks * h->cfg.slots_per_step * RS_GROUP;
     if (h->mux) n = (size_t)h->cfg.n_envs * h->cfg.slots_per_step * RS_MUX_UE;
@@ -1184,6 +1388,7 @@
 
 extern "C" int rs_get_counters(rs_handle* h, uint64_t counters[4]) {
     if (!h || !counters) return RS_EINVAL;
+    if (lanes_close(h) != RS_OK) return RS_EHIP;
     HIPCHK(h, hipSetDevice(h->device));
     HIPCHK(h, hipMemsetAsync(h->d_counter_sum, 0, sizeof(uint64_t) * 4, h->stream));
     if (h->n_tasks > 0)
@@ -1197,6 +1402,7 @@
 
 extern "C" int rs_get_rx_stats(rs_handle* h, uint64_t out[3]) {
     if (!h || !out) return RS_EINVAL;
+    if (lanes_close(h) != RS_OK) return RS_EHIP;
     uint64_t c[4];
     const int rc = rs_get_counters(h, c);
     if (rc != RS_OK) return rc;
@@ -1210,6 +1416,7 @@
 
 extern "C" int rs_set_schedule_hint(rs_handle* h, int mode) {
     if (!h) return RS_EINVAL;
+    if (lanes_close(h) != RS_OK) return RS_EHIP;
     h->hint_auto = mode < 0;
     h->block_hint = mode < 0 ? auto_hint(h) : (mode ? 1 : 0);
     drop_graph(h);
@@ -1218,6 +1425,7 @@
 
 extern "C" int rs_set_group_size(rs_handle* h, int lanes) {
     if (!h || (lanes != 8 && lanes != 16 && lanes != 32)) return RS_EINVAL;
+    if (lanes_close(h) != RS_OK) return RS_EHIP;
     h->group = lanes;
     drop_graph(h);
     return RS_OK;
@@ -1225,6 +1433,7 @@
 
 extern "C" int rs_get_section_profile(rs_handle* h, uint64_t out[16]) {
     if (!h || !out) return RS_EINVAL;
+    if (lanes_close(h) != RS_OK) return RS_EHIP;
     HIPCHK(h, hipSetDevice(h->device));
     HIPCHK(h, hipMemcpyAsync(out, h->d_sections, sizeof(uint64_t) * 16, hipMemcpyDeviceToHost, h->stream));
     HIPCHK(h, hipStreamSynchronize(h->stream));
@@ -1233,6 +1442,7 @@
 
 extern "C" int rs_get_task_profile(rs_handle* h, uint64_t* out) {
     if (!h || !out) return RS_EINVAL;
+    if (lanes_close(h) != RS_OK) return RS_EHIP;
     HIPCHK(h, hipSetDevice(h->device));
     HIPCHK(h, hipMemcpyAsync(out, h->d_sections + 16, sizeof(uint64_t) * (4 * (size_t)h->n_tasks + 16),
                              hipMemcpyDeviceToHost, h->stream));
@@ -1242,22 +1452,63 @@
 
 extern "C" int rs_set_kernel_timing(rs_handle* h, int enable) {
     if (!h) return RS_EINVAL;
+    if (lanes_close(h) != RS_OK) return RS_EHIP;
     h->spans.on = enable != 0;
     h->spans.reset();
+    if (enable) {
+        HIPCHK(h, hipSetDevice(h->device));
+        if (!h->ev_ref) HIPCHK(h, hipEventCreate(&h->ev_ref));
+        HIPCHK(h, hipEventRecord(h->ev_ref, h->stream));
+    }
+    return RS_OK;
+}
+
+static int lane_window(rs_handle* h, double out[4]) {
+    std::vector<std::pair<double, double>> iv;
+    double sum = 0.0;
+    int64_t steps = 0;
+    for (size_t i = 0; i < h->spans.used && h->ev_ref; ++i) {
+        const EventSpans::Span& sp = h->spans.spans[i];
+        float t0 = 0.f, t1 = 0.f;
+        HIPCHK(h, hipEventElapsedTime(&t0, h->ev_ref, sp.e0));
+        HIPCHK(h, hipEventElapsedTime(&t1, h->ev_ref, sp.e1));
+        iv.emplace_back((double)t0, (double)t1);
+        sum += (double)t1 - (double)t0;
+        const int L = sp.kind >> 8, l = sp.kind & 255;
+        steps += (L == 0 || l == L - 1) ? 1 : 0;
+    }
+    std::sort(iv.begin(), iv.end());
+    double uni = 0.0, hi = 0.0;
+    for (size_t i = 0; i < iv.size(); ++i) {
+        const double lo = (i == 0 || iv[i].first > hi) ? iv[i].first : hi;
+        if (iv[i].second > lo) uni += iv[i].second - lo;
+        hi = (i == 0 || iv[i].second > hi) ? iv[i].second : hi;
+    }
+    if (uni > sum) uni = sum;
+    out[0] = (double)lanes_wanted(h);
+    out[1] = steps ? sum / (double)steps : 0.0;
+    out[2] = steps ? uni / (double)steps : 0.0;
+    out[3] = sum > 0.0 ? 1.0 - uni / sum : 0.0;
+    if (out[3] < 0.0) out[3] = 0.0;
     return RS_OK;
 }
 
 extern "C" int rs_kernel_time_stats_ms(rs_handle* h, double out[3], int64_t* launches) {
     if (!h || !out) return RS_EINVAL;
+    if (lanes_close(h) != RS_OK) return RS_EHIP;
     HIPCHK(h, hipSetDevice(h->device));
     HIPCHK(h, hipStreamSynchronize(h->stream));
-    double tot = 0.0, mn = 0.0, mx = 0.0;
+    if (h->spans.used > 0 && lane_window(h, h->lane_info) != RS_OK) return RS_EHIP;
+    double tot = 0.0, mn = 0.0, mx = 0.0, step_ms = 0.0;
     int64_t n = 0;
-    HIPCHK(h, h->spans.drain([&](int, double ms) {
-        tot += ms;
-        mn = (n == 0 || ms < mn) ? ms : mn;
-        mx = ms > mx ? ms : mx;
+    HIPCHK(h, h->spans.drain([&](int kind, double ms) {
+        step_ms += ms;
+        if ((kind >> 8) != 0 && (kind & 255) != (kind >> 8) - 1) return;
+        tot += step_ms;
+        mn = (n == 0 || step_ms < mn) ? step_ms : mn;
+        mx = step_ms > mx ? step_ms : mx;
         n += 1;
+        step_ms = 0.0;
     }));
     out[0] = n ? tot / (double)n : 0.0;
     out[1] = mn;
@@ -1266,8 +1517,33 @@
     return RS_OK;
 }
 
+extern "C" int rs_get_lane_info(rs_handle* h, double out[4]) {
+    if (!h || !out) return RS_EINVAL;
+    if (lanes_close(h) != RS_OK) return RS_EHIP;
+    HIPCHK(h, hipSetDevice(h->device));
+    if (h->spans.used > 0) {
+        HIPCHK(h, hipStreamSynchronize(h->stream));
+        if (lane_window(h, h->lane_info) != RS_OK) return RS_EHIP;
+    }
+    memcpy(out, h->lane_info, sizeof(double) * 4);
+    out[0] = (double)lanes_wanted(h);
+    return RS_OK;
+}
+
+extern "C" int rs_set_lanes(rs_handle* h, int n) {
+    if (!h || n < 0) return RS_EINVAL;
+    if (lanes_close(h) != RS_OK) return RS_EHIP;
+    if (n >= 2 && (h->mux || h->cfg.n_mmtc > 0)) {
+        h->err = "rs_set_lanes: no lanes for multiplexed handles or handles with mMTC slices";
+        return RS_EINVAL;
+    }
+    h->lanes_req = n;
+    return RS_OK;
+}
+
 extern "C" int rs_kernel_time_ms(rs_handle* h, double* avg_ms, int64_t* launches) {
     if (!h || !avg_ms) return RS_EINVAL;
+    if (lanes_close(h) != RS_OK) return RS_EHIP;
     double st[3];
     const int rc = rs_kernel_time_stats_ms(h, st, launches);
     if (rc == RS_OK) *avg_ms = st[0];
@@ -1276,6 +1552,7 @@
 
 extern "C" int rs_synchronize(rs_handle* h) {
     if (!h) return RS_EINVAL;
+    if (lanes_close(h) != RS_OK) return RS_EHIP;
     HIPCHK(h, hipSetDevice(h->device));
     HIPCHK(h, hipStreamSynchronize(h->stream));
     return RS_OK;
@@ -1300,12 +1577,14 @@
 }
 extern "C" int rs_state_bytes(rs_handle* h, uint64_t* bytes) {
     if (!h || !bytes) return RS_EINVAL;
+    if (lanes_close(h) != RS_OK) return RS_EHIP;
     uint64_t t = sizeof(rs_state_header);
     for (auto& r : h->regions) t += r.second;
     *bytes = t;
     return RS_OK;
 }
 extern "C" int rs_save_state(rs_handle* h, void* blob, uint64_t bytes) {
+    if (lanes_close(h) != RS_OK) return RS_EHIP;
     uint64_t need = 0;
     if (!h || !blob || rs_state_bytes(h, &need) != RS_OK) return RS_EINVAL;
     if (bytes < need) {
@@ -1325,6 +1604,7 @@
     return RS_OK;
 }
 extern "C" int rs_load_state(rs_handle* h, const void* blob, uint64_t bytes) {
+    if (lanes_close(h) != RS_OK) return RS_EHIP;
     uint64_t need = 0;
     if (!h || !blob || rs_state_bytes(h, &need) != RS_OK) return RS_EINVAL;
     rs_state_header hd;
diff --git a/network-slicing_amd/csrc/rs_fork.hip b/network-slicing_amd/csrc/rs_fork.hip
--- a/network-slicing_amd/csrc/rs_fork.hip
+++ b/network-slicing_amd/csrc/rs_fork.hip
@@ -198,6 +198,8 @@
 
 extern "C" int rs_fork(rs_handle* dst, rs_handle* src, const int32_t* src_index) {
     if (!dst || !src || !src_index) return RS_EINVAL;
+    if (lanes_close(dst) != RS_OK) return RS_EHIP;
+    if (lanes_close(src) != RS_OK) return RS_EHIP;
     if (dst == src) {
         dst->err = "rs_fork: source and destination must be different handles";
         return RS_EINVAL;
@@ -256,6 +258,7 @@
 
 extern "C" int rs_set_lookahead(rs_handle* h, int max_branches) {
     if (!h) return RS_EINVAL;
+    if (lanes_close(h) != RS_OK) return RS_EHIP;
     if (max_branches < 0 || (max_branches > 0 && max_branches < h->cfg.n_prbs + 1)) {
         h->err = "rs_set_lookahead: max_branches must be 0 or at least n_prbs + 1";
         return RS_EINVAL;
@@ -272,6 +275,7 @@
 
 extern "C" int rs_set_clairvoyant_fallback(rs_handle* h, int mode) {
     if (!h || mode < 0 || mode > 1) return RS_EINVAL;
+    if (lanes_close(h) != RS_OK) return RS_EHIP;
     h->la_widest = mode;
     return RS_OK;
 }
@@ -323,6 +327,7 @@
 extern "C" int rs_step_clairvoyant(rs_handle* h, int32_t* actions_out, float* obs, double* reward, int32_t* labels,
                                    int32_t* violations) {
     if (!h) return RS_EINVAL;
+    if (lanes_close(h) != RS_OK) return RS_EHIP;
     HIPCHK(h, hipSetDevice(h->device));
     if (!h->is_reset) {
         h->err = "rs_step_clairvoyant: call rs_reset first";
diff --git a/network-slicing_amd/csrc/rs_order.hip b/network-slicing_amd/csrc/rs_order.hip
--- a/network-slicing_amd/csrc/rs_order.hip
+++ b/network-slicing_amd/csrc/rs_order.hip
@@ -22,14 +22,17 @@
 
 __global__ __launch_bounds__(256) void order_key_kernel(const RsDev* __restrict__ D, const RsState* __restrict__ Sp,
                                                         const int32_t* __restrict__ actions, int mode, int* hist,
-                                                        uint64_t* slot, int4 kw, int split_ue) {
+                                                        uint64_t* slot, int4 kw, int split_ue, int task0, int task_cnt, int rebin) {
     __shared__ int cnt[RS_ORDER_BINS];
     for (int k = threadIdx.x; k < RS_ORDER_BINS; k += 256) cnt[k] = 0;
     __syncthreads();
-    const int n_tasks = D->n_envs * D->n_embb;
-    const int task = (int)(blockIdx.x * blockDim.x + threadIdx.x);
+    const int n_tasks = task0 + task_cnt;
+    const int task = task0 + (int)(blockIdx.x * blockDim.x + threadIdx.x);
     int bin = 0, local = 0;
-    if (task < n_tasks) {
+    if (task < n_tasks && rebin) {
+        bin = (int)(slot[task] & (RS_ORDER_BINS - 1));
+        local = atomicAdd(&cnt[bin], 1);
+    } else if (task < n_tasks) {
         const int rep = task / D->n_embb, sl = task - rep * D->n_embb;
         const int n_prb = actions[rep * D->n_slices + sl];
         int key;
@@ -66,7 +69,7 @@
 __global__ __launch_bounds__(256) void order_scatter_kernel(const RsDev* __restrict__ D, const int* __restrict__ hist,
                                                             int* hist_next, const uint64_t* __restrict__ slot,
                                                             int32_t* order, int pair, int tpw, int snake, int snake_mask, int rot_mask,
-                                                            int seg_lo, int seg_hi) {
+                                                            int seg_lo, int seg_hi, int task0, int task_cnt) {
     __shared__ int start[RS_ORDER_BINS];
     __shared__ int part[256];
     constexpr int PER = RS_ORDER_BINS / 256;
@@ -93,9 +96,9 @@
     __syncthreads();
     if (blockIdx.x == 0)
         for (int k = threadIdx.x; k < RS_ORDER_BINS; k += 256) hist_next[k] = 0;
-    const int n_all = D->n_envs * D->n_embb;
-    const int task = (int)(blockIdx.x * blockDim.x + threadIdx.x);
-    if (task >= n_all) return;
+    const int task = task0 + (int)(blockIdx.x * blockDim.x + threadIdx.x);
+    if (task >= task0 + task_cnt) return;
+    order += task0;
     const uint64_t v = slot[task];
     int p = start[(int)(v & (RS_ORDER_BINS - 1))] + (int)(v >> 11);
     if (p < seg_lo || p >= seg_hi) {
diff --git a/network-slicing_amd/csrc/rs_policy_io.hip b/network-slicing_amd/csrc/rs_policy_io.hip
--- a/network-slicing_amd/csrc/rs_policy_io.hip
+++ b/network-slicing_amd/csrc/rs_policy_io.hip
@@ -205,6 +205,7 @@
 
 extern "C" int rs_get_device_view(rs_handle* h, rs_device_view* out) {
     if (!h || !out) return RS_EINVAL;
+    if (lanes_close(h) != RS_OK) return RS_EHIP;
     int rc = pio_ensure(h);
     if (rc != RS_OK) return rc;
     const PolicyIo* p = h->pio;
@@ -231,6 +232,7 @@
 
 extern "C" int rs_step_device(rs_handle* h, int kind, const void* actions_device, void* caller_stream) {
     if (!h || !actions_device) return RS_EINVAL;
+    if (lanes_close(h) != RS_OK) return RS_EHIP;
     if (kind != RS_ACT_PRBS && kind != RS_ACT_SHARES && kind != RS_ACT_INDEX) {
         h->err = "rs_step_device: unknown action kind";
         return RS_EINVAL;
@@ -299,6 +301,7 @@
 
 extern "C" int rs_stream_join(rs_handle* h, void* caller_stream) {
     if (!h) return RS_EINVAL;
+    if (lanes_close(h) != RS_OK) return RS_EHIP;
     hipStream_t cs = (hipStream_t)caller_stream;
     if (cs == h->stream) return RS_OK;
     int rc = pio_ensure(h);
@@ -309,6 +312,7 @@
 
 extern "C" int rs_set_action_table(rs_handle* h, const int32_t* table, int32_t n_actions) {
     if (!h || !table || n_actions <= 0) return RS_EINVAL;
+    if (lanes_close(h) != RS_OK) return RS_EHIP;
     int rc = pio_ensure(h);
     if (rc != RS_OK) return rc;
     PolicyIo* p = h->pio;
@@ -339,6 +343,7 @@
 
 extern "C" int rs_report_begin(rs_handle* h, int32_t steps) {
     if (!h || steps < 0) return RS_EINVAL;
+    if (lanes_close(h) != RS_OK) return RS_EHIP;
     int rc = pio_ensure(h);
     if (rc != RS_OK) return rc;
     PolicyIo* p = h->pio;
@@ -353,6 +358,7 @@
 
 extern "C" int rs_report_extend(rs_handle* h, int32_t eval_steps) {
     if (!h || eval_steps < 0) return RS_EINVAL;
+    if (lanes_close(h) != RS_OK) return RS_EHIP;
     PolicyIo* p = h->pio;
     if (!p || !p->h_viol) {
         h->err = "rs_report_extend: no report history (rs_report_begin)";
@@ -382,6 +388,7 @@
 
 extern "C" int rs_report_fetch(rs_handle* h, int16_t* violation, double* reward, int16_t* resources, int32_t* n_recorded) {
     if (!h) return RS_EINVAL;
+    if (lanes_close(h) != RS_OK) return RS_EHIP;
     PolicyIo* p = h->pio;
     if (!p || !p->h_viol) {
         h->err = "rs_report_fetch: no report history (rs_report_begin)";
@@ -401,6 +408,7 @@
 
 extern "C" int rs_device_copy(rs_handle* h, void* dst, const void* src, uint64_t bytes, int to_device) {
     if (!h || (bytes && (!dst || !src))) return RS_EINVAL;
+    if (lanes_close(h) != RS_OK) return RS_EHIP;
     HIPCHK(h, hipSetDevice(h->device));
     if (bytes == 0) return RS_OK;
     HIPCHK(h, hipMemcpyAsync(dst, src, (size_t)bytes, to_device ? hipMemcpyHostToDevice : hipMemcpyDeviceToHost, h->stream));
diff --git a/network-slicing_amd/ranslice/_lib.py b/network-slicing_amd/ranslice/_lib.py
--- a/network-slicing_amd/ranslice/_lib.py
+++ b/network-slicing_amd/ranslice/_lib.py
@@ -40,6 +40,7 @@
     'rs_fork', 'rs_set_lookahead', 'rs_step_clairvoyant', 'rs_set_clairvoyant_fallback',
     'rs_get_device_view', 'rs_step_device', 'rs_stream_join', 'rs_set_action_table', 'rs_report_begin', 'rs_report_extend',
     'rs_report_fetch', 'rs_device_copy',
+    'rs_set_lanes', 'rs_get_lane_info',
 ) + KB_EXPORTS
 
 RS_ACT_PRBS, RS_ACT_SHARES, RS_ACT_INDEX = 0, 1, 2
@@ -114,6 +115,8 @@
     L.rs_get_task_profile.argtypes = [vp, up]
     L.rs_set_group_size.argtypes = [vp, C.c_int]
     L.rs_set_schedule_hint.argtypes = [vp, C.c_int]
+    L.rs_set_lanes.argtypes = [vp, C.c_int]
+    L.rs_get_lane_info.argtypes = [vp, dp]
     L.rs_kernel_time_ms.argtypes = [vp, dp, C.POINTER(C.c_int64)]
     L.rs_kernel_time_stats_ms.argtypes = [vp, dp, C.POINTER(C.c_int64)]
     L.rs_set_kernel_timing.argtypes = [vp, C.c_int]
diff --git a/network-slicing_amd/ranslice/vec_env.py b/network-slicing_amd/ranslice/vec_env.py
--- a/network-slicing_amd/ranslice/vec_env.py
+++ b/network-slicing_amd/ranslice/vec_env.py
@@ -199,6 +199,14 @@
     def set_group_size(self, lanes):
         self._check(self.L.rs_set_group_size(self.h, int(lanes)))
 
+    def set_lanes(self, n):
+        self._check(self.L.rs_set_lanes(self.h, int(n)))
+
+    def lane_info(self):
+        out = (C.c_double * 4)()
+        self._check(self.L.rs_get_lane_info(self.h, out))
+        return int(out[0]), out[1], out[2], out[3]
+
     def set_schedule_hint(self, mode):
         self._check(self.L.rs_set_schedule_hint(self.h, int(mode)))
 
```

After: 5.113 million (median of 6 runs). 1.04x the previous value.
